# li199603/easy_gaussian_splatting

Hardware: AMD Instinct MI355X
Metric: train iters/sec + forward render fps, 1M Gaussians @ 1080p (higher is better)
Workload: dtype f32

## Files before the change

### easy_gaussian_splatting_amd/csrc/gs_binning.hip

```cpp

#include "gs_common.h"

namespace gs {

#define GS_BIN_PER_GROUP 4096
#define GS_BIN_MAX_GROUPS 256
constexpr int kBinThreads = 1024;
constexpr int kCoopTiles = 32;

BinLayout bin_layout(int C, int64_t N, int tiles) {
    BinLayout L;
    int64_t g = (N + GS_BIN_PER_GROUP - 1) / GS_BIN_PER_GROUP;
    if (g < 1) g = 1;
    if (g > GS_BIN_MAX_GROUPS) g = GS_BIN_MAX_GROUPS;
    L.groups = (int)g;
    L.per_group = (N + g - 1) / g;
    auto align = [](size_t x) { return (x + 255) & ~(size_t)255; };
    size_t off = 0;
    L.hist_off = off; off = align(off + sizeof(uint32_t) * (size_t)C * L.groups * tiles);
    L.tile_cnt_off = off; off = align(off + sizeof(uint32_t) * (size_t)C * tiles);
    L.grp_tot_off = off; off = align(off + sizeof(uint32_t) * (size_t)C * L.groups);
    L.grp_base_off = off; off = align(off + sizeof(uint32_t) * (size_t)C * L.groups);
    L.items_off = off; off = align(off + sizeof(int32_t) * (64 + (size_t)10 * (size_t)C * tiles));
    L.total = off;
// ... 45 lines not shown
        }
    }
    __syncthreads();
    uint32_t* out = hist_mat + ((size_t)c * G + grp) * tiles;
    for (int t = threadIdx.x; t < tiles; t += blockDim.x) out[t] = hist[t];
    uint32_t wsum = wave_reduce_add(local);
    if (lane_id() == 0) scratch[threadIdx.x >> 6] = wsum;
    __syncthreads();
    if (threadIdx.x == 0) {
        uint32_t s = 0;
        for (int i = 0; i < (int)(blockDim.x >> 6); ++i) s += scratch[i];
        grp_tot[c * G + grp] = s;
    }
}

constexpr int kColTiles = GS_BIN_MAX_GROUPS > 256 ? 32 : 64, kColChunks = GS_BIN_MAX_GROUPS > 256 ? 32 : 16;
__global__ __launch_bounds__(kColTiles * kColChunks) void bin_colscan_kernel(int C, int G, int tiles, uint32_t* __restrict__ hist_mat,
                                                                              uint32_t* __restrict__ tile_cnt) {
    __shared__ uint32_t part[kColChunks][kColTiles + 1];
    const int tl = threadIdx.x % kColTiles, ch = threadIdx.x / kColTiles;
    const int64_t i = (int64_t)blockIdx.x * kColTiles + tl;
    const bool in = i < (int64_t)C * tiles;
    const int c = in ? (int)(i / tiles) : 0, t = in ? (int)(i % tiles) : 0;
    const int per = (G + kColChunks - 1) / kColChunks;
    const int g0 = ch * per, g1 = min(G, g0 + per);
    uint32_t* col = hist_mat + (size_t)c * G * tiles + t;
    constexpr int kMax = 16;
    uint32_t v[kMax];
    uint32_t sum = 0;
#pragma unroll
    for (int k = 0; k < kMax; ++k) {
        v[k] = (in && g0 + k < g1) ? col[(size_t)(g0 + k) * tiles] : 0u;
        sum += v[k];
    }
    uint32_t extra = 0;
    for (int g = g0 + kMax; in && g < g1; ++g) extra += col[(size_t)g * tiles];
    part[ch][tl] = sum + extra;
    __syncthreads();
    uint32_t run = 0, total = 0;
#pragma unroll
    for (int k = 0; k < kColChunks; ++k) {
        const uint32_t p = part[k][tl];
        run += k < ch ? p : 0u;
        total += p;
    }
    if (in) {
#pragma unroll
        for (int k = 0; k < kMax; ++k) {
            if (g0 + k < g1) col[(size_t)(g0 + k) * tiles] = run;
            run += v[k];
        }
        for (int g = g0 + kMax; g < g1; ++g) { const uint32_t x = col[(size_t)g * tiles]; col[(size_t)g * tiles] = run; run += x; }
        if (ch == 0) tile_cnt[i] = total;
    }
}

constexpr int kScanItems = 16;
__global__ __launch_bounds__(kBinThreads) void bin_tilescan_kernel(
    int n_tiles_total, int n_groups_total, const uint32_t* __restrict__ tile_cnt,
    const uint32_t* __restrict__ grp_tot, int32_t* __restrict__ isect_offsets,
    int32_t* __restrict__ bucket_offsets, uint32_t* __restrict__ grp_base,
    int64_t* __restrict__ info, int32_t* __restrict__ tile_order, int64_t cap_isects, int64_t cap_tile,
    int64_t keep_mask, int32_t* __restrict__ sort_counts, int64_t* __restrict__ info_mirror, int per_call,
    int64_t* __restrict__ rblk, int phase) {
    __shared__ unsigned long long scratch[17];
    const int chunk = kBinThreads * kScanItems;
    if (round_idle(rblk, phase)) return;
    if (blockIdx.x == 2) {
        if (sort_counts && threadIdx.x < 64) sort_counts[threadIdx.x] = 0;
        unsigned long long gcarry = 0;
        for (int base = 0; base < n_groups_total; base += kBinThreads) {
            const int i = base + threadIdx.x;
            unsigned long long v = i < n_groups_total ? grp_tot[i] : 0ull, total;
            unsigned long long ex = block_excl_scan_add(v, scratch, &total);
            if (i < n_groups_total) grp_base[i] = (uint32_t)(gcarry + ex);
            gcarry += total;
        }
        return;
    }
    if (blockIdx.x == 1) {
        if (!tile_order) return;
        if (n_tiles_total > chunk) {
            for (int i = threadIdx.x; i < n_tiles_total; i += kBinThreads) tile_order[i] = i;
            return;
        }
        constexpr int kW = kBinThreads / 64;
        __shared__ uint32_t cls_cnt[64][kW + 1];
        auto cls_of = [](uint32_t x) -> int {
            if (x < 2u) return 0;
            const int lg = 31 - __clz((int)x);
            return min(63, (lg << 2) | (int)((x << (31 - lg)) >> 29 & 3u));
        };
        const int wv = threadIdx.x >> 6;
        const int first = threadIdx.x * kScanItems;
        uint32_t v[kScanItems];
#pragma unroll
        for (int k = 0; k < kScanItems; ++k) v[k] = (first + k < n_tiles_total) ? tile_cnt[first + k] : 0u;
        for (int i = threadIdx.x; i < 64 * (kW + 1); i += kBinThreads) (&cls_cnt[0][0])[i] = 0u;
        __syncthreads();
#pragma unroll
        for (int k = 0; k < kScanItems; ++k)
            if (first + k < n_tiles_total) atomicAdd(&cls_cnt[cls_of(v[k])][wv], 1u);
        __syncthreads();
        if (threadIdx.x < 64) {
            const int c = 63 - (int)threadIdx.x;
            uint32_t n = 0, cw[kW];
#pragma unroll
            for (int w = 0; w < kW; ++w) { cw[w] = cls_cnt[c][w]; n += cw[w]; }
            uint32_t run = wave_incl_scan_add(n) - n;
#pragma unroll
            for (int w = 0; w < kW; ++w) { cls_cnt[c][w] = run; run += cw[w]; }
        }
        __syncthreads();
#pragma unroll
        for (int k = 0; k < kScanItems; ++k)
            if (first + k < n_tiles_total) tile_order[atomicAdd(&cls_cnt[cls_of(v[k])][wv], 1u)] = first + k;
        return;
    }
    unsigned long long carry_i = phase == 2 ? (unsigned long long)rblk[GS_ROUND_BASE] : 0ull, carry_b = 0;
    uint32_t max_cnt = 0;
    for (int base = 0; base < n_tiles_total; base += chunk) {
        const int first = base + threadIdx.x * kScanItems;
        uint32_t v[kScanItems];
        unsigned long long si = 0, sb = 0;
#pragma unroll
        for (int k = 0; k < kScanItems; ++k) {
            v[k] = (first + k < n_tiles_total) ? tile_cnt[first + k] : 0u;
            si += v[k];
            sb += (v[k] + GS_BUCKET - 1) / GS_BUCKET;
// ... 116 lines not shown
            for (int i = lane_id(); i < bcnt; i += 64) {
                const int yy = div_by_width(i, binv);
                const uint32_t pos = atomicAdd(&cursor[(by0 + yy) * tw + bx0 + (i - yy * bw)], 1u);
                keys[pos] = ((unsigned long long)bd << 32) | (slot_gid ? bslot + i : (uint32_t)bf);
                if (slot_gid) slot_gid[bslot + i] = bf;
            }
        }
    }
}

template <typename KeyPtr>
__device__ __forceinline__ void bitonic_sort_keys(KeyPtr key, int n, int P) {
    for (int k = 2; k <= P; k <<= 1) {
        const int half = k >> 1;
        for (int idx = threadIdx.x; idx < (P >> 1); idx += blockDim.x) {
            const int blk = idx / half, off = idx - blk * half;
            const int a = blk * k + off, b = blk * k + k - 1 - off;
            if (b < n) {
                const unsigned long long ka = key[a], kb = key[b];
                if (ka > kb) { key[a] = kb; key[b] = ka; }
            }
        }
        __syncthreads();
        for (int j = half >> 1; j > 0; j >>= 1) {
            for (int idx = threadIdx.x; idx < (P >> 1); idx += blockDim.x) {
                const int a = ((idx & ~(j - 1)) << 1) | (idx & (j - 1)), b = a + j;
                if (b < n) {
                    const unsigned long long ka = key[a], kb = key[b];
                    if (ka > kb) { key[a] = kb; key[b] = ka; }
                }
            }
            __syncthreads();
        }
    }
}

struct SortArgs {
    int tiles, tile_bits, lo_excl, hi_incl;
    const int32_t* isect_offsets;
    unsigned long long* keys;
    const int32_t* slot_gid;
    int64_t* isect_ids;
    int32_t* flatten_ids;
    int32_t* slots;
    const int64_t* guard;
    int coarse;
    int seg;
    unsigned long long* merged;
    const int64_t* rblk;
    int phase;
};
__device__ __forceinline__ bool sort_off(const SortArgs& a) { return guard_tripped(a.guard) || round_idle(a.rblk, a.phase); }

constexpr int kSegLen = 8192;
constexpr int kSegMax = 8;

template <bool IN_LDS>
__global__ void tile_sort_kernel(const SortArgs a) {
    extern __shared__ __attribute__((aligned(16))) unsigned long long skeys[];
    const int t = blockIdx.x;
    if (sort_off(a)) return;
    const int lo = a.isect_offsets[t], hi = a.isect_offsets[t + 1];
    const int n = hi - lo;
    if (n <= a.lo_excl || n > a.hi_incl) return;
    int P = 1;
    while (P < n) P <<= 1;
    unsigned long long* gk = a.keys + lo;
    if (IN_LDS) {
        for (int i = threadIdx.x; i < n; i += blockDim.x) skeys[i] = gk[i];
        __syncthreads();
        bitonic_sort_keys(skeys, n, P);
    } else {
        bitonic_sort_keys(gk, n, P);
    }
    if (a.coarse) {
        if (IN_LDS) for (int i = threadIdx.x; i < n; i += blockDim.x) gk[i] = skeys[i];
        return;
    }
    const int cam = t / a.tiles, tid = t - cam * a.tiles;
    const long long hi_bits = ((long long)cam << (32 + a.tile_bits)) | ((long long)tid << 32);
    for (int i = threadIdx.x; i < n; i += blockDim.x) {
        const unsigned long long k = IN_LDS ? skeys[i] : gk[i];
        const uint32_t slot = (uint32_t)k;
        if (a.slot_gid) { a.slots[lo + i] = (int32_t)slot; a.flatten_ids[lo + i] = a.slot_gid[slot]; }
        else a.flatten_ids[lo + i] = (int32_t)slot;
        if (a.isect_ids) a.isect_ids[lo + i] = hi_bits | (long long)(k >> 32);
    }
}

template <int T>
__device__ __forceinline__ void radix_sort_list(const SortArgs& a, const int vblock) {
    extern __shared__ __attribute__((aligned(16))) unsigned long long skeys[];
    constexpr int W = T / 64;
    const int tile = a.seg ? vblock / kSegMax : vblock;
    int lo = a.isect_offsets[tile], n = a.isect_offsets[tile + 1] - lo;
    if (n <= a.lo_excl || n > a.hi_incl) return;
    if (a.seg) {
        const int sg = vblock - tile * kSegMax;
        lo += sg * kSegLen;
        n = min(kSegLen, n - sg * kSegLen);
        if (n <= 0) return;
    }
    const int cap = a.seg ? kSegLen : a.hi_incl;
    unsigned long long* src = skeys;
    unsigned long long* dst = skeys + cap;
    uint32_t* cnt = reinterpret_cast<uint32_t*>(skeys + 2 * cap);
    uint32_t* nxt = cnt + W * 256;
    __shared__ int s_flag;
    const int tid = threadIdx.x, lane = tid & 63, wave = tid >> 6;
// ... 69 lines not shown
        uint32_t* tc = cnt; cnt = nxt; nxt = tc;
    }
    __syncthreads();
    if (tid == 0) s_flag = 0;
    __syncthreads();
    bool bad = false;
    for (int i = tid + 1; i < n; i += T) bad |= src[i] < src[i - 1];
    if (bad) s_flag = 1;
    __syncthreads();
    if (s_flag) {
        int P = 1;
        while (P < n) P <<= 1;
        bitonic_sort_keys(src, n, P);
    }
    if (a.coarse || a.seg) {
        unsigned long long* out = a.keys + lo;
        for (int i = tid; i < n; i += T) out[i] = src[i];
        return;
    }
    const int cam = tile / a.tiles, tix = tile - cam * a.tiles;
    const long long hi_bits = ((long long)cam << (32 + a.tile_bits)) | ((long long)tix << 32);
    for (int i = tid; i < n; i += T) {
        const unsigned long long k = src[i];
        const uint32_t slot = (uint32_t)k;
        if (a.slot_gid) { a.slots[lo + i] = (int32_t)slot; a.flatten_ids[lo + i] = a.slot_gid[slot]; }
        else a.flatten_ids[lo + i] = (int32_t)slot;
        if (a.isect_ids) a.isect_ids[lo + i] = hi_bits | (long long)(k >> 32);
    }
}

template <int T>
__global__ __launch_bounds__(T) void tile_radix_sort_kernel(const SortArgs a) {
    if (sort_off(a)) return;
    radix_sort_list<T>(a, blockIdx.x);
}

template <int T>
__global__ __launch_bounds__(T) void tile_radix_sort_items_kernel(const SortArgs a, const int32_t* __restrict__ items,
                                                                  const int32_t* __restrict__ n_items) {
    if (sort_off(a)) return;
    const int n = *n_items;
    for (int it = blockIdx.x; it < n; it += gridDim.x) {
        radix_sort_list<T>(a, items[it]);
        __syncthreads();
    }
}

__global__ __launch_bounds__(256) void class_items_kernel(int n_lists, const int32_t* __restrict__ offsets,
                                                          int32_t* __restrict__ items, int32_t* __restrict__ counts,
                                                          const int64_t* __restrict__ guard, const int64_t* __restrict__ rblk, int phase) {
    if (guard_tripped(guard) || round_idle(rblk, phase)) return;
    const int i = blockIdx.x * blockDim.x + threadIdx.x;
    if (i >= n_lists) return;
    const int n = offsets[i + 1] - offsets[i];
    if (n > 1024 && n <= 4096) items[atomicAdd(&counts[0], 1)] = i;
    else if (n > 4096 && n <= kSegLen) items[n_lists + atomicAdd(&counts[1], 1)] = i;
    else if (n > kSegLen && n <= kSegLen * kSegMax) {
        const int ns = (n + kSegLen - 1) / kSegLen;
        const int p = atomicAdd(&counts[2], ns);
        for (int sg = 0; sg < ns; ++sg) items[2 * n_lists + p + sg] = i * kSegMax + sg;
    }
}

static size_t sort_items_bytes(int64_t n_lists) {
    return sizeof(int32_t) * (64 + (size_t)(2 + kSegMax) * (size_t)n_lists);
}


struct BinsLayout {
    int groups, shift, bw, bh, nbins;
    int64_t per_group;
    size_t hist_off;
    size_t bin_cnt_off;
    size_t grp_tot_off;
    size_t grp_base_off;
    size_t coff_off;
    size_t choff_off;
    size_t tile_cnt_off;
    size_t chunk_bin_off;
    int chunk_shift;
    size_t rec_off;
    size_t staged_off;
    size_t cnt_ct_off;
    size_t items_off;
    int64_t max_chunks;
    size_t total;
};

static BinsLayout bins_layout(int C, int64_t N, int tw, int th, int bin_shift, int64_t coarse_cap) {
    BinsLayout L;
    int64_t g = (N + GS_BIN_PER_GROUP - 1) / GS_BIN_PER_GROUP;
    if (g < 1) g = 1;
    if (g > GS_BIN_MAX_GROUPS) g = GS_BIN_MAX_GROUPS;
    L.groups = (int)g;
    L.per_group = (N + g - 1) / g;
    const int64_t nb2 = (int64_t)((tw + 3) / 4) * ((th + 3) / 4);
    L.shift = bin_shift ? bin_shift : ((N / nb2 > 2500) ? 1 : 2);
    const int B = 1 << L.shift;
    L.bw = (tw + B - 1) / B; L.bh = (th + B - 1) / B; L.nbins = L.bw * L.bh;
    auto align = [](size_t x) { return (x + 255) & ~(size_t)255; };
    size_t off = 0;
    L.hist_off = off; off = align(off + sizeof(uint32_t) * (size_t)C * L.groups * L.nbins);
    L.bin_cnt_off = off; off = align(off + sizeof(uint32_t) * (size_t)C * L.nbins);
    L.grp_tot_off = off; off = align(off + sizeof(uint32_t) * (size_t)C * L.groups);
    L.grp_base_off = off; off = align(off + sizeof(uint32_t) * (size_t)C * L.groups);
    L.coff_off = off; off = align(off + sizeof(int32_t) * ((size_t)C * L.nbins + 1));
    L.choff_off = off; off = align(off + sizeof(int32_t) * ((size_t)C * L.nbins + 1));
    L.tile_cnt_off = off; off = align(off + sizeof(uint32_t) * (size_t)C * tw * th);
    L.chunk_shift = 10 + (L.shift - 1);
    L.max_chunks = (coarse_cap >> L.chunk_shift) + (int64_t)C * L.nbins;
    L.chunk_bin_off = off; off = align(off + sizeof(int4) * (size_t)L.max_chunks);
    L.rec_off = off; off = align(off + sizeof(uint4) * (size_t)C * (size_t)N);
    L.staged_off = off; off = align(off + sizeof(uint4) * (size_t)coarse_cap);
    L.cnt_ct_off = off; off = align(off + sizeof(uint32_t) * (size_t)L.max_chunks * B * B);
// ... 377 lines not shown
            int l = 0, r = min(kSegLen, n - o * kSegLen);
            while (l < r) {
                const int mid = (l + r) >> 1;
                if (seg[mid] < k) l = mid + 1; else r = mid;
            }
            pos += l;
        }
        if (a.coarse) {
            a.merged[lo + pos] = k;
        } else {
            const uint32_t slot = (uint32_t)k;
            if (a.slot_gid) { a.slots[lo + pos] = (int32_t)slot; a.flatten_ids[lo + pos] = a.slot_gid[slot]; }
            else a.flatten_ids[lo + pos] = (int32_t)slot;
            if (a.isect_ids) a.isect_ids[lo + pos] = hi_bits | (long long)(k >> 32);
        }
    }
    }
}

__global__ __launch_bounds__(1024) void seg_copy_kernel(const SortArgs a, const int32_t* __restrict__ items,
                                                        const int32_t* __restrict__ n_items) {
    if (sort_off(a)) return;
    const int n_it = *n_items;
    for (int it = blockIdx.x; it < n_it; it += gridDim.x) {
        const int vblock = items[it];
        const int list = vblock / kSegMax, sg = vblock - list * kSegMax;
        const int lo = a.isect_offsets[list], n = a.isect_offsets[list + 1] - lo;
        const int s_lo = sg * kSegLen, s_n = min(kSegLen, n - s_lo);
        for (int i = threadIdx.x; i < s_n; i += blockDim.x) a.keys[lo + s_lo + i] = a.merged[lo + s_lo + i];
    }
}

constexpr int kSortLarge = kSegLen * kSegMax;

}

using namespace gs;

extern "C" int gs_bin_groups(int64_t N) { return bin_layout(1, N, 1).groups; }

static int list_round(int64_t*& rblk) {
    const Rounds R = current_rounds();
    const int phase = (R.phase == 1 || R.phase == 4) ? 1 : (R.phase == 2 ? 2 : 0);
    rblk = phase ? R.blk : nullptr;
    return phase;
}

extern "C" size_t gs_bin_workspace_bytes(int C, int64_t N, int tile_w, int tile_h) {
    return bin_layout(C, N, tile_w * tile_h).total;
}

#define GS_SORT1K_THREADS 256
#define GS_SORT4K_THREADS 256
static int launch_list_sorts(hipStream_t st, SortArgs& a, unsigned grid, int64_t max_tile_count, int32_t* items_ws) {
    int lo_excl = 0;
    int32_t* counts = items_ws;
    int32_t* items = items_ws + 64;
    const size_t radix_lds = 2 * sizeof(uint32_t) * 256;
    a.lo_excl = 0; a.hi_incl = 1024;
    if (max_tile_count > 0) {
        const size_t lds_k = 2 * sizeof(uint64_t) * 1024 + radix_lds * (GS_SORT1K_THREADS / 64);
        hipLaunchKernelGGL(tile_radix_sort_kernel<GS_SORT1K_THREADS>, dim3(grid), dim3(GS_SORT1K_THREADS), lds_k, st, a);
        GS_LAUNCH_CHECK("tile_radix_sort_kernel");
    }
    if (max_tile_count <= 1024) return GS_OK;
    hipLaunchKernelGGL(class_items_kernel, dim3((grid + 255) / 256), dim3(256), 0, st, (int)grid, a.isect_offsets, items, counts, a.guard, a.rblk, a.phase);
    GS_LAUNCH_CHECK("class_items_kernel");
    {
        a.lo_excl = 1024; a.hi_incl = 4096;
        const size_t lds_k = 2 * sizeof(uint64_t) * 4096 + radix_lds * (GS_SORT4K_THREADS / 64);
        if (int rc = ensure_lds((const void*)tile_radix_sort_items_kernel<GS_SORT4K_THREADS>, lds_k)) return rc;
        hipLaunchKernelGGL(tile_radix_sort_items_kernel<GS_SORT4K_THREADS>, dim3(grid < 512u ? grid : 512u), dim3(GS_SORT4K_THREADS), lds_k, st, a,
                           (const int32_t*)items, (const int32_t*)counts);
        GS_LAUNCH_CHECK("tile_radix_sort_items_kernel<4096>");
    }
    if (max_tile_count > 4096) {
        a.lo_excl = 4096; a.hi_incl = kSegLen;
        const size_t lds_k = 2 * sizeof(uint64_t) * (size_t)kSegLen + radix_lds * (768 / 64);
        if (int rc = ensure_lds((const void*)tile_radix_sort_items_kernel<768>, lds_k)) return rc;
        hipLaunchKernelGGL(tile_radix_sort_items_kernel<768>, dim3(grid < 256u ? grid : 256u), dim3(768), lds_k, st, a,
                           (const int32_t*)(items + grid), (const int32_t*)(counts + 1));
        GS_LAUNCH_CHECK("tile_radix_sort_items_kernel<8192>");
    }
    if (max_tile_count > kSegLen) {
        a.lo_excl = kSegLen; a.hi_incl = kSortLarge; a.seg = 1;
        const size_t lds_k = 2 * sizeof(uint64_t) * (size_t)kSegLen + radix_lds * (768 / 64);
        if (int rc = ensure_lds((const void*)tile_radix_sort_items_kernel<768>, lds_k)) return rc;
        const int32_t* it = items + 2 * (size_t)grid;
        const int32_t* nit = counts + 2;
        hipLaunchKernelGGL(tile_radix_sort_items_kernel<768>, dim3(256), dim3(768), lds_k, st, a, it, nit);
        GS_LAUNCH_CHECK("tile_radix_sort_items_kernel<segments>");
        hipLaunchKernelGGL(seg_merge_kernel, dim3(512), dim3(1024), 0, st, a, it, nit);
        GS_LAUNCH_CHECK("seg_merge_kernel");
        if (a.coarse) {
            hipLaunchKernelGGL(seg_copy_kernel, dim3(512), dim3(1024), 0, st, a, it, nit);
            GS_LAUNCH_CHECK("seg_copy_kernel");
        }
        a.seg = 0;
    }
    if (max_tile_count > kSortLarge) {
        a.lo_excl = kSortLarge; a.hi_incl = 0x7fffffff;
        hipLaunchKernelGGL(tile_sort_kernel<false>, dim3(grid), dim3(1024), 0, st, a);
        GS_LAUNCH_CHECK("tile_sort_kernel<global>");
    }
    (void)lo_excl;
    return GS_OK;
}

extern "C" int gs_bin_count(void* stream, int C, int64_t N, int tile_w, int tile_h, const uint32_t* bbox,
                            void* workspace, size_t workspace_bytes, int32_t* isect_offsets,
                            int32_t* bucket_offsets, int32_t* tile_order, int64_t* info_dev, int64_t* info_host) {
    GS_REQUIRE(C >= 1 && N >= 0 && tile_w > 0 && tile_h > 0, "C>=1, N>=0, positive tile grid");
    const int tiles = tile_w * tile_h;
    GS_REQUIRE((size_t)tiles * 4 + 128 <= 160 * 1024, "tile grid too large for the LDS histogram (max 40928 tiles per camera)");
    GS_REQUIRE((int64_t)C * tiles < (1ll << 31), "too many tiles");
    const BinLayout L = bin_layout(C, N, tiles);
    GS_REQUIRE(workspace && workspace_bytes >= L.total, "workspace too small (see gs_bin_workspace_bytes)");
    GS_REQUIRE(isect_offsets && bucket_offsets && info_dev, "null output pointer");
    GS_REQUIRE(N == 0 || bbox, "null bbox");
    int64_t* rblk;
// ... 15 lines not shown
                       tiles, hist, tile_cnt);
    GS_LAUNCH_CHECK("bin_colscan_kernel");
    const Guard gd = current_guard();
    GS_REQUIRE(gd.info == nullptr || gd.info == info_dev, "the guard set by gs_guard_set must be this call's info_dev");
    hipLaunchKernelGGL(bin_tilescan_kernel, dim3(3), dim3(kBinThreads), 0, st, (int)ct, C * L.groups, tile_cnt,
                       grp_tot, isect_offsets, bucket_offsets, grp_base, info_dev, tile_order, gd.cap_isects, gd.cap_tile,
                       (int64_t)0, (int32_t*)(ws + L.items_off), current_info_mirror(), gd.per_call, rblk, phase);
    GS_LAUNCH_CHECK("bin_tilescan_kernel");
    if (info_host) {
        GS_HIP_CHECK(hipMemcpyAsync(info_host, info_dev, 4 * sizeof(int64_t), hipMemcpyDeviceToHost, st));
        GS_HIP_CHECK(hipStreamSynchronize(st));
    }
    return GS_OK;
}

extern "C" int gs_bin_emit_sort(void* stream, int C, int64_t N, int tile_w, int tile_h, const uint32_t* bbox,
                                const float* depths, void* workspace, size_t workspace_bytes,
                                const int32_t* isect_offsets, int64_t n_isects, int64_t max_tile_count,
                                uint64_t* keys_tmp, int32_t* slot_gid, int32_t* cum_tiles,
                                int64_t* isect_ids, int32_t* flatten_ids, int32_t* slots) {
    GS_REQUIRE(C >= 1 && N >= 0 && tile_w > 0 && tile_h > 0, "C>=1, N>=0, positive tile grid");
    const int tiles = tile_w * tile_h;
    const BinLayout L = bin_layout(C, N, tiles);
    GS_REQUIRE(workspace && workspace_bytes >= L.total, "workspace too small (see gs_bin_workspace_bytes)");
    GS_REQUIRE(n_isects >= 0 && n_isects < (1ll << 31), "intersection count must fit int32");
    if (N == 0) return GS_OK;
    GS_REQUIRE(bbox && depths && isect_offsets && cum_tiles, "null pointer");
    GS_REQUIRE(n_isects == 0 || (keys_tmp && flatten_ids), "null intersection buffer");
    GS_REQUIRE((slot_gid == nullptr) == (slots == nullptr), "slot_gid and slots: both (training lists) or neither (inference lists)");
    int64_t* rblk;
    const int phase = list_round(rblk);
    GS_REQUIRE(phase == 0 || C == 1, "depth rounds: one camera per call");
    hipStream_t st = (hipStream_t)stream;
    char* ws = (char*)workspace;
    const uint32_t* hist = (const uint32_t*)(ws + L.hist_off);
    const uint32_t* grp_base = (const uint32_t*)(ws + L.grp_base_off);
    const size_t lds = sizeof(uint32_t) * ((size_t)tiles + 32);
    if (int rc = ensure_lds((const void*)bin_emit_kernel, lds)) return rc;
    hipLaunchKernelGGL(bin_emit_kernel, dim3(L.groups, C), dim3(kBinThreads), lds, st, N, tile_w, tiles,
                       L.per_group, (const uint4*)bbox, depths, hist, isect_offsets, grp_base,
                       (unsigned long long*)keys_tmp, slot_gid, cum_tiles, current_guard().info, (const int64_t*)rblk, phase);
    GS_LAUNCH_CHECK("bin_emit_kernel");
    if (n_isects == 0) return GS_OK;
    SortArgs a;
    a.tiles = tiles;
    int tb = 0;
    for (int v = tiles; v > 0; v >>= 1) ++tb;
    a.tile_bits = tb;
    a.isect_offsets = isect_offsets; a.keys = (unsigned long long*)keys_tmp; a.slot_gid = slot_gid;
    a.isect_ids = isect_ids; a.flatten_ids = flatten_ids; a.slots = slots;
    a.guard = current_guard().info;
    a.coarse = 0; a.seg = 0; a.merged = nullptr; a.rblk = rblk; a.phase = phase;
    static_assert(2 + kSegMax == 10, "bin_layout sizes the work lists for kSegMax == 8");
    return launch_list_sorts(st, a, (unsigned)(C * tiles), max_tile_count, (int32_t*)(ws + L.items_off));
}

extern "C" size_t gs_bins_workspace_bytes(int C, int64_t N, int tile_w, int tile_h, int bin_shift, int64_t coarse_cap) {
    if (bin_shift < 0 || bin_shift > 2 || coarse_cap < 0) return 0;
    return bins_layout(C, N, tile_w, tile_h, bin_shift, coarse_cap).total;
}

template <bool WRITE>
static int launch_refine(hipStream_t st, const BinsLayout& L, const RefineArgs& a) {
    const unsigned grid = (unsigned)L.max_chunks;
    if (L.shift == 2) hipLaunchKernelGGL((bins_refine_kernel<WRITE, 2>), dim3(grid), dim3(1024), 0, st, a);
    else hipLaunchKernelGGL((bins_refine_kernel<WRITE, 1>), dim3(grid), dim3(256), 0, st, a);
    GS_LAUNCH_CHECK("bins_refine_kernel");
    return GS_OK;
}

static void fill_refine_args(RefineArgs& r, const BinsLayout& L, int C, int tile_w, int tile_h, char* ws, const uint64_t* coarse_keys,
                             const uint32_t* bbox, const int64_t* info_dev) {
    r.tw = tile_w; r.th = tile_h; r.tiles = tile_w * tile_h; r.n_bins_total = C * L.nbins;
    r.choff = (const int32_t*)(ws + L.choff_off);
    r.chunk_desc = (const int4*)(ws + L.chunk_bin_off);
    r.cnt_ct = (uint32_t*)(ws + L.cnt_ct_off);
    int tb = 0;
    for (int v = r.tiles; v > 0; v >>= 1) ++tb;
    r.tile_bits = tb; r.bw = L.bw; r.nbins = L.nbins;
    r.coff = (const int32_t*)(ws + L.coff_off);
    r.keys = (const unsigned long long*)coarse_keys;
    r.rec = (const uint4*)(ws + L.rec_off);
    r.staged = (uint4*)(ws + L.staged_off);
    r.tile_cnt = (uint32_t*)(ws + L.tile_cnt_off);
    r.isect_offsets = nullptr; r.isect_ids = nullptr; r.flatten_ids = nullptr; r.slots = nullptr;
    r.info = info_dev;
    int64_t* rblk;
    r.phase = list_round(rblk);
    r.rblk = rblk;
}

extern "C" int gs_bins_count(void* stream, int C, int64_t N, int tile_w, int tile_h, int bin_shift, const uint32_t* bbox,
                             const float* depths, void* workspace, size_t workspace_bytes, uint64_t* coarse_keys,
                             int64_t coarse_cap, int64_t coarse_list_cap,
                             int32_t* cum_tiles, int32_t* isect_offsets, int32_t* bucket_offsets, int32_t* tile_order,
                             int64_t* info_dev, int64_t* info_host) {
    GS_REQUIRE(C >= 1 && N >= 0 && tile_w > 0 && tile_h > 0, "C>=1, N>=0, positive tile grid");
    const int tiles = tile_w * tile_h;
    GS_REQUIRE((int64_t)C * tiles < (1ll << 31) && (int64_t)C * N < (1ll << 31), "too many tiles or flatten ids");
    GS_REQUIRE(bin_shift >= 0 && bin_shift <= 2, "bin_shift: 0 (library default), 1 (2x2 tiles) or 2 (4x4 tiles)");
    GS_REQUIRE(coarse_cap >= 0 && coarse_cap < (1ll << 31) && (coarse_cap == 0 || coarse_keys), "coarse key buffer");
    const BinsLayout L = bins_layout(C, N, tile_w, tile_h, bin_shift, coarse_cap);
    GS_REQUIRE((size_t)L.nbins * 4 + 128 <= 160 * 1024, "tile grid too large for the LDS bin histogram");
    GS_REQUIRE(workspace && workspace_bytes >= L.total, "workspace too small (see gs_bins_workspace_bytes)");
    GS_REQUIRE(isect_offsets && bucket_offsets && info_dev, "null output pointer");
    GS_REQUIRE(N == 0 || (bbox && depths && cum_tiles), "null bbox / depths / cum_tiles");
    hipStream_t st = (hipStream_t)stream;
    char* ws = (char*)workspace;
    uint32_t* hist = (uint32_t*)(ws + L.hist_off);
    uint32_t* bin_cnt = (uint32_t*)(ws + L.bin_cnt_off);
    uint32_t* grp_tot = (uint32_t*)(ws + L.grp_tot_off);
    uint32_t* grp_base = (uint32_t*)(ws + L.grp_base_off);
    int32_t* coff = (int32_t*)(ws + L.coff_off);
    uint32_t* tile_cnt = (uint32_t*)(ws + L.tile_cnt_off);
    const Guard gd = current_guard();
    GS_REQUIRE(gd.info == nullptr || gd.info == info_dev, "the guard set by gs_guard_set must be this call's info_dev");
    int64_t* rblk;
    const int phase = list_round(rblk);
    GS_REQUIRE(phase == 0 || C == 1, "depth rounds: one camera per call");
    int64_t list_cap = 0x7fffffff;
    if (coarse_list_cap > 0) list_cap = coarse_list_cap <= 1024 ? 1024 : coarse_list_cap <= 4096 ? 4096 : coarse_list_cap <= kSegLen ? kSegLen
                                        : coarse_list_cap <= kSortLarge ? kSortLarge : 0x7fffffff;
    const size_t lds = sizeof(uint32_t) * ((size_t)L.nbins + 32);
    if (int rc = ensure_lds((const void*)bins_hist_kernel, lds)) return rc;
    hipLaunchKernelGGL(bins_hist_kernel, dim3(L.groups, C), dim3(kBinThreads), lds, st, N, L.shift, L.bw, L.nbins, L.per_group,
                       (const uint4*)bbox, hist, grp_tot, (const int64_t*)rblk, phase);
    GS_LAUNCH_CHECK("bins_hist_kernel");
    const int64_t cb = (int64_t)C * L.nbins;
    hipLaunchKernelGGL(bins_colscan_kernel, dim3((unsigned)((cb + 3) / 4)), dim3(256), 0, st, C, L.groups, L.nbins, hist, bin_cnt);
    GS_LAUNCH_CHECK("bins_colscan_kernel");
    hipLaunchKernelGGL(bins_scan_kernel, dim3(2), dim3(kBinThreads), 0, st, (int)cb, C * L.groups, bin_cnt, grp_tot, coff,
                       (int32_t*)(ws + L.choff_off), (int4*)(ws + L.chunk_bin_off), L.max_chunks, L.chunk_shift, grp_base,
                       info_dev, coarse_cap, list_cap,
                       (gd.info != nullptr && !gd.per_call) ? 1 : 0, (int32_t*)(ws + L.items_off), (const int64_t*)rblk, phase);
    GS_LAUNCH_CHECK("bins_scan_kernel");
    if (N > 0) {
        if (int rc = ensure_lds((const void*)bins_emit_kernel, lds)) return rc;
        hipLaunchKernelGGL(bins_emit_kernel, dim3(L.groups, C), dim3(kBinThreads), lds, st, N, L.shift, L.bw, L.nbins, L.per_group,
                           (const uint4*)bbox, depths, hist, coff, grp_base, (unsigned long long*)coarse_keys, cum_tiles,
                           (uint4*)(ws + L.rec_off), (const int64_t*)info_dev, (const int64_t*)rblk, phase);
        GS_LAUNCH_CHECK("bins_emit_kernel");
        SortArgs a;
        a.tiles = L.nbins; a.tile_bits = 0;
        a.isect_offsets = coff; a.keys = (unsigned long long*)coarse_keys; a.slot_gid = nullptr;
        a.isect_ids = nullptr; a.flatten_ids = nullptr; a.slots = nullptr;
        a.guard = info_dev; a.coarse = 1; a.seg = 0; a.rblk = rblk; a.phase = phase;
        a.merged = (unsigned long long*)(ws + L.staged_off);
        if (int rc = launch_list_sorts(st, a, (unsigned)cb, list_cap < coarse_cap ? list_cap : coarse_cap, (int32_t*)(ws + L.items_off))) return rc;
    }
    RefineArgs r;
    fill_refine_args(r, L, C, tile_w, tile_h, ws, coarse_keys, bbox, info_dev);
    if (int rc = launch_refine<false>(st, L, r)) return rc;
    {
        const unsigned g = (unsigned)(((int64_t)C * tiles + 255) / 256);
        if (L.shift == 2) hipLaunchKernelGGL(bins_chunkscan_kernel<2>, dim3(g), dim3(256), 0, st, r, C);
        else hipLaunchKernelGGL(bins_chunkscan_kernel<1>, dim3(g), dim3(256), 0, st, r, C);
        GS_LAUNCH_CHECK("bins_chunkscan_kernel");
    }
    hipLaunchKernelGGL(bin_tilescan_kernel, dim3(2), dim3(kBinThreads), 0, st, C * tiles, 0, tile_cnt, (const uint32_t*)nullptr,
                       isect_offsets, bucket_offsets, (uint32_t*)nullptr, info_dev, tile_order, gd.cap_isects,
                       (int64_t)0x7fffffffffffffffll, (int64_t)12, (int32_t*)nullptr, current_info_mirror(), gd.per_call, rblk, phase);
    GS_LAUNCH_CHECK("bin_tilescan_kernel");
    if (info_host) {
        GS_HIP_CHECK(hipMemcpyAsync(info_host, info_dev, 8 * sizeof(int64_t), hipMemcpyDeviceToHost, st));
        GS_HIP_CHECK(hipStreamSynchronize(st));
    }
    return GS_OK;
}

extern "C" int gs_bins_lists(void* stream, int C, int64_t N, int tile_w, int tile_h, int bin_shift, const uint32_t* bbox, void* workspace,
                             size_t workspace_bytes, const uint64_t* coarse_keys, int64_t coarse_cap, const int32_t* cum_tiles,
                             const int32_t* isect_offsets, int64_t* isect_ids, int32_t* flatten_ids, int32_t* slots,
                             const int64_t* info_dev) {
    GS_REQUIRE(C >= 1 && N >= 0 && tile_w > 0 && tile_h > 0, "C>=1, N>=0, positive tile grid");
    GS_REQUIRE(bin_shift >= 0 && bin_shift <= 2 && coarse_cap >= 0, "bin_shift: 0, 1 or 2; coarse_cap as given to gs_bins_count");
    const BinsLayout L = bins_layout(C, N, tile_w, tile_h, bin_shift, coarse_cap);
    GS_REQUIRE(workspace && workspace_bytes >= L.total, "workspace too small (see gs_bins_workspace_bytes)");
    GS_REQUIRE(info_dev && isect_offsets, "null pointer");
    if (N == 0) return GS_OK;
    GS_REQUIRE(cum_tiles && bbox && flatten_ids, "null list buffer");
    RefineArgs r;
    fill_refine_args(r, L, C, tile_w, tile_h, (char*)workspace, coarse_keys, bbox, info_dev);
    r.isect_offsets = isect_offsets; r.isect_ids = isect_ids; r.flatten_ids = flatten_ids; r.slots = slots;
    return launch_refine<true>((hipStream_t)stream, L, r);
}
```

### easy_gaussian_splatting_amd/csrc/gs_blend.hip

```cpp
#include <algorithm>

#include "gs_common.h"
#include "gs_math.h"

namespace gs {

#ifdef GS_BWD_CHECK
struct BwdCheck {
    float* fwd_T;
    int32_t* fwd_cnt;
    float2* unit_out;
    int2* unit_hdr;
};
static BwdCheck g_bwd_check = {nullptr, nullptr, nullptr, nullptr};
#define GS_IF_CHECK(...) __VA_ARGS__
#else
#define GS_IF_CHECK(...)
#endif

constexpr int kUnit = GS_UNIT;
constexpr int kChunk = 8;
constexpr int kUnitLog = 128;
constexpr int kWalkUnits = GS_WALK_UNITS, kWalkStorage = GS_WALK_STORAGE, kWalkRows = GS_WALK_ROWS,
              kWalkFlags = GS_WALK_FLAGS, kWalkSkip = GS_WALK_SKIP;
constexpr int kScanThreads = 256, kScanPerThread = 32, kScanChunk = kScanThreads * kScanPerThread;

struct BlendFwdArgs {
    const int32_t* tile_order;
    int C, W, H, tw, tiles;
    const float4* rec;
    const float* bg;
    const int32_t *isect_offsets, *flatten_ids, *slots;
    float *out_colors, *out_alphas;
    float4* ckpt;
    int2* qlist;
    int32_t* qcnt;
    uint8_t* qmask;
    int4* unit_desc;
    int32_t* walk;
    int cap_units;
    unsigned long long* flags;
    const int64_t* guard;
    int64_t* rblk;
    uint8_t* live;
    float4* tstate;
    int4* trec;
    int solo;
    GS_IF_CHECK(BwdCheck chk;)
};

#ifdef GS_CLOCK_PROBE
__device__ unsigned long long gs_clk_acc[4];
struct ClockProbe {
    long long c0, w0; int slot;
    __device__ ClockProbe(int s) : c0(clock64()), w0(wall_clock64()), slot(s) {}
    __device__ ~ClockProbe() {
        if ((threadIdx.x & 63) == 0) {
            atomicAdd(&gs_clk_acc[slot], (unsigned long long)(clock64() - c0));
            atomicAdd(&gs_clk_acc[slot + 1], (unsigned long long)(wall_clock64() - w0));
        }
    }
};
#define GS_CLOCK_PROBE_SCOPE(slot) ClockProbe clock_probe_(slot)
#else
#define GS_CLOCK_PROBE_SCOPE(slot)
#endif

#ifdef GS_EXACT_MATH
__device__ __forceinline__ float fast_exp2(float x) { return (float)exp2((double)x); }
__device__ __forceinline__ float fast_rcp(float x) { return (float)(1.0 / (double)x); }
#else
__device__ __forceinline__ float fast_exp2(float x) { return __builtin_amdgcn_exp2f(x); }
__device__ __forceinline__ float fast_rcp(float x) { return __builtin_amdgcn_rcpf(x); }
#endif

constexpr float kDoneScale = 18446744073709551616.f;
constexpr float kDoneInv = 5.421010862427522e-20f;
// ... 258 lines not shown
        }
        if (lv && !a.solo) {
#pragma unroll
            for (int k = 0; k < 4; ++k) a.tstate[((size_t)t * 4 + k) * 64 + lane] = make_float4(T[k], cr[k], cg[k], cb[k]);
            if (CKPT && lane == 0) {
                a.trec[2 * (size_t)t] = make_int4(cnt[0], cnt[1], cnt[2], cnt[3]);
                int ru[4];
#pragma unroll
                for (int k = 0; k < 4; ++k) ru[k] = cnt[k] > 0 ? uring[4 * k + (((cnt[k] - 1) / kUnit) & 3)] : 0;
                a.trec[2 * (size_t)t + 1] = make_int4(ru[0], ru[1], ru[2], ru[3]);
            }
        }
    }
    float bgr = 0.f, bgg = 0.f, bgb = 0.f, bga = 0.f;
    if (a.bg) {
        bgr = a.bg[NC * cam];
        if (NC > 1) bgg = a.bg[NC * cam + 1];
        if (NC > 2) bgb = a.bg[NC * cam + 2];
        if (NC > 3) bga = a.bg[NC * cam + 3];
    }
#pragma unroll
    for (int k = 0; k < 4; ++k) {
        const int px = px0 + 8 * (k & 1), py = py0 + 8 * (k >> 1);
        if (px < a.W && py < a.H) {
            const size_t o = ((size_t)cam * a.H + py) * a.W + px;
            const float Tf = px_final_T(T[k]);
            a.out_colors[NC * o] = cr[k] + Tf * bgr;
            if (NC > 1) a.out_colors[NC * o + 1] = cg[k] + Tf * bgg;
            if (NC > 2) a.out_colors[NC * o + 2] = cb[k] + Tf * bgb;
            if (NC > 3) a.out_colors[NC * o + 3] = ca[k] + Tf * bga;
            a.out_alphas[o] = 1.f - Tf;
            GS_IF_CHECK(if (CKPT && a.chk.fwd_T) { a.chk.fwd_T[o] = Tf; a.chk.fwd_cnt[o] = taken[k]; })
        }
    }
}

template <bool CKPT, int WAVES, int ROUND>
__global__ __launch_bounds__(64 * WAVES) GS_FWD_ATTR void blend_fwd_kernel(const BlendFwdArgs a) {
    blend_fwd_body<CKPT, WAVES, ROUND, 3>(a, nullptr);
}
template <bool CKPT, int WAVES, int NC>
__global__ __launch_bounds__(64 * WAVES) __attribute__((amdgpu_waves_per_eu(CKPT ? (NC == 4 ? 4 : 5) : 1, 8))) void chan_fwd_kernel(const BlendFwdArgs a, float* ckpt_ext) {
    blend_fwd_body<CKPT, WAVES, 0, NC>(a, ckpt_ext);
}

struct RowScanArgs {
    const uint8_t* qmask;
    int32_t* row_base;
    int32_t* walk;
    int64_t n_cap, cap_rows;
    unsigned long long* flags;
    const int64_t* guard;
    volatile int64_t* mirror;
};

__device__ __forceinline__ int32_t row_counts32(const uint8_t* __restrict__ qmask, int64_t i0, int64_t n, uint32_t (&w)[8]) {
#pragma unroll
    for (int j = 0; j < 8; ++j) w[j] = 0u;
    if (i0 + kScanPerThread <= n) {
        const uint4 x = reinterpret_cast<const uint4*>(qmask + i0)[0], y = reinterpret_cast<const uint4*>(qmask + i0)[1];
        w[0] = x.x; w[1] = x.y; w[2] = x.z; w[3] = x.w; w[4] = y.x; w[5] = y.y; w[6] = y.z; w[7] = y.w;
    } else {
        for (int j = 0; j < kScanPerThread; ++j)
            if (i0 + j < n) w[j >> 2] |= (uint32_t)qmask[i0 + j] << (8 * (j & 3));
    }
    int32_t tot = 0;
#pragma unroll
    for (int j = 0; j < 8; ++j) {
        uint32_t v = w[j] & 0x0f0f0f0fu;
        v = v - ((v >> 1) & 0x55555555u);
        v = (v & 0x33333333u) + ((v >> 2) & 0x33333333u);
        w[j] = v;
        tot += (int32_t)((v * 0x01010101u) >> 24);
    }
    return tot;
}

__global__ __launch_bounds__(kScanThreads) void row_count_kernel(const RowScanArgs a) {
    __shared__ int32_t scratch[20];
    if (a.walk[kWalkSkip] != 0) return;
    const int64_t n = slots_in_use(a.n_cap, a.guard);
    const int64_t c0 = (int64_t)blockIdx.x * kScanChunk;
    if (c0 > n) return;
    uint32_t w[8];
    const int32_t tot = row_counts32(a.qmask, c0 + (int64_t)threadIdx.x * kScanPerThread, n, w);
    int32_t block_tot;
    block_excl_scan_add<int32_t>(tot, scratch, &block_tot);
    if (threadIdx.x == 0) a.walk[GS_WALK_WORDS + blockIdx.x] = block_tot;
}

__global__ __launch_bounds__(1024) void row_chunk_scan_kernel(const RowScanArgs a) {
    __shared__ int32_t scratch[20];
    if (a.walk[kWalkSkip] != 0) return;
    const int64_t n = slots_in_use(a.n_cap, a.guard);
    const int nb = (int)(n / kScanChunk) + 1;
    int32_t* part = a.walk + GS_WALK_WORDS;
    const int per = (nb + 1023) / 1024;
    const int j0 = (int)threadIdx.x * per, j1 = min(nb, j0 + per);
    int32_t mine = 0;
    for (int j = j0; j < j1; ++j) mine += part[j];
    int32_t total;
    int32_t run = block_excl_scan_add<int32_t>(mine, scratch, &total);
    for (int j = j0; j < j1; ++j) { const int32_t c = part[j]; part[j] = run; run += c; }
    if (threadIdx.x == 0) {
        int32_t fullest = 0;
        for (int r = 0; r < GS_WALK_RANGES; ++r) fullest = max(fullest, a.walk[GS_WALK_RANGE0 + 32 * r]);
        a.walk[kWalkStorage] = GS_WALK_RANGES * fullest;
        a.walk[kWalkRows] = total;
        int fl = a.walk[kWalkFlags];
        if (a.flags && (fl & GS_FLAG_UNITS)) atomicOr(a.flags, (unsigned long long)GS_FLAG_UNITS);
        if ((int64_t)total > a.cap_rows) {
            fl |= GS_FLAG_ROWS;
            a.walk[kWalkFlags] = fl;
            if (a.flags) atomicOr(a.flags, (unsigned long long)GS_FLAG_ROWS);
        }
        if (a.mirror) {
            a.mirror[0] = a.walk[kWalkUnits]; a.mirror[1] = a.walk[kWalkStorage]; a.mirror[2] = total; a.mirror[3] = fl;
            __threadfence_system();
        }
    }
}

__global__ __launch_bounds__(kScanThreads) void row_base_kernel(const RowScanArgs a) {
    __shared__ int32_t scratch[20];
    if (a.walk[kWalkSkip] != 0) return;
    const int64_t n = slots_in_use(a.n_cap, a.guard);
    const int64_t c0 = (int64_t)blockIdx.x * kScanChunk;
    if (c0 > n) return;
    const int64_t i0 = c0 + (int64_t)threadIdx.x * kScanPerThread;
    uint32_t w[8];
    const int32_t tot = row_counts32(a.qmask, i0, n, w);
    int32_t block_tot;
    const int32_t run = block_excl_scan_add<int32_t>(tot, scratch, &block_tot) + a.walk[GS_WALK_WORDS + blockIdx.x];
    int32_t first16 = 0;
#pragma unroll
    for (int j = 0; j < 4; ++j) first16 += (int32_t)((w[j] * 0x01010101u) >> 24);
    if (i0 <= n) a.row_base[i0 >> 4] = run;
    if (i0 + 16 <= n) a.row_base[(i0 >> 4) + 1] = run + first16;
}

struct BlendBwdArgs {
    int C, W, H, tw, tiles;
    const float4* rec;
    const int32_t* walk;
    const int2* qlist;
    const int32_t* qcnt;
    const int4* unit_desc;
    const float4* ckpt;
    const uint8_t* qmask;
    const int32_t* row_base;
    int cap_units;
    const int32_t* cls_hdr;
    const int4* cls_desc;
    int cls_cap;
    const float *out_colors, *out_alphas, *v_colors, *v_alphas;
    float4* rows;
    const int64_t* guard;
    GS_IF_CHECK(BwdCheck chk;)
};

constexpr int kBwdWaves = 4;
constexpr int kPipeLanes = 8;
constexpr int kPerLane = kUnit / kPipeLanes;
static_assert(kPerLane == 4, "bwd_wave is instantiated for 1 .. 4 entries per lane");
constexpr int kUnitsPerWave = 64 / kPipeLanes;
constexpr int kUnitPixels = 64;
constexpr int kBwdSteps = kUnitPixels + kPipeLanes - 1;

__device__ __forceinline__ float dpp_row_shr1(float v) {
    return __builtin_bit_cast(float, __builtin_amdgcn_update_dpp(__builtin_bit_cast(int, v), __builtin_bit_cast(int, v), 0x111, 0xf, 0xf, false));
}


// ... 169 lines not shown
        row[i] += __popc((unsigned)m & ((1u << q) - 1u));
    }
#pragma unroll
    for (int i = 0; i < E; ++i) {
        if (e[i].has) {
            float4* rp = a.rows + (GS_ROW_FLOATS / 4) * (size_t)row[i];
            const float v_op = e[i].op > 0.f ? (float)(-e[i].s_vs / (acc_t)e[i].op) : 0.f;
            rp[0] = make_float4((float)e[i].s_mx, (float)e[i].s_my, (float)e[i].s_ax, (float)e[i].s_ay);
            rp[1] = make_float4((float)((acc_t)0.5f * e[i].s_A), (float)e[i].s_B, (float)((acc_t)0.5f * e[i].s_C), v_op);
            rp[2] = make_float4((float)e[i].s_r, (float)e[i].s_g, (float)e[i].s_b, NC == 4 ? (float)e[i].s_3 : 0.f);
        }
    }
}

constexpr int kClsHdrInts = 16, kClsThreads = 1024;
__global__ __launch_bounds__(64) void unit_classes_clear_kernel(int32_t* __restrict__ hdr) {
    if (threadIdx.x < kClsHdrInts) hdr[threadIdx.x] = 0;
}
__global__ __launch_bounds__(kClsThreads) void unit_classes_kernel(const int32_t* __restrict__ walk, const int4* __restrict__ unit_desc,
                                                                   const int32_t* __restrict__ qcnt, int cap_units, int cls_cap,
                                                                   int32_t* __restrict__ hdr, int4* __restrict__ cls, const int64_t* __restrict__ guard) {
    __shared__ int s_cnt[kClsThreads / 64][4], s_base[kClsThreads / 64][4];
    if (guard_tripped(guard)) return;
    const int n_units = min(walk[kWalkUnits], cap_units);
    if ((int)blockIdx.x * kClsThreads >= n_units) return;
    const int u = (int)blockIdx.x * kClsThreads + (int)threadIdx.x, wave = threadIdx.x >> 6, lane = threadIdx.x & 63;
    int c = 0;
    int4 ud = make_int4(0, 0, 0, 0);
    if (u < n_units) {
        ud = unit_desc[u];
        const int n_in = min(kUnit, qcnt[ud.x] - ud.y * kUnit);
        c = min(max((n_in + kPipeLanes - 1) / kPipeLanes, 1), 4);
        ud.w = u;
    }
    unsigned long long m[4];
#pragma unroll
    for (int k = 0; k < 4; ++k) m[k] = __ballot(c == k + 1);
    if (lane < 4) s_cnt[wave][lane] = (int)__popcll(lane == 0 ? m[0] : (lane == 1 ? m[1] : (lane == 2 ? m[2] : m[3])));
    __syncthreads();
    if (threadIdx.x < 4) {
        int tot = 0;
        for (int w = 0; w < kClsThreads / 64; ++w) { s_base[w][threadIdx.x] = tot; tot += s_cnt[w][threadIdx.x]; }
        const int base = tot ? atomicAdd(hdr + 1 + threadIdx.x, tot) : 0;
        for (int w = 0; w < kClsThreads / 64; ++w) s_base[w][threadIdx.x] += base;
    }
    __syncthreads();
    if (c) {
        const unsigned long long mine = c == 1 ? m[0] : (c == 2 ? m[1] : (c == 3 ? m[2] : m[3]));
        const int i = s_base[wave][c - 1] + (int)__popcll(mine & ((1ull << lane) - 1ull));
        if (i < (c == 4 ? cap_units : cls_cap)) cls[(c == 4 ? 0 : cap_units + (3 - c) * cls_cap) + i] = ud;
    }
}

template <int NC>
__device__ __forceinline__ void blend_bwd_body(const BlendBwdArgs& a, const float* __restrict__ ckpt_ext) {
    __shared__ float4 sd0_all[kBwdWaves][kUnitsPerWave][64];
    __shared__ float2 sck_all[kBwdWaves][kUnitsPerWave][64];
    const int wave = threadIdx.x >> 6, lane = threadIdx.x & 63;
    const int pipe = lane / kPipeLanes, r = lane & (kPipeLanes - 1);
    if (guard_tripped(a.guard)) return;
    constexpr int kPerBlock = kBwdWaves * kUnitsPerWave;
    int cls = 4, blk = (int)blockIdx.x, n_units, first = 0;
    if (a.cls_hdr == nullptr) {
        n_units = min(a.walk[kWalkUnits], a.cap_units);
    } else {
        const int b4 = (a.cap_units + kPerBlock - 1) / kPerBlock, bt = (a.cls_cap + kPerBlock - 1) / kPerBlock;
        if (blk >= b4) {
            const int k = (blk - b4) / bt;
            cls = 3 - k; blk -= b4 + k * bt; first = a.cap_units + k * a.cls_cap;
        }
        n_units = min(a.cls_hdr[cls], cls == 4 ? a.cap_units : a.cls_cap);
    }
    const int in_class = (blk * kBwdWaves + wave) * kUnitsPerWave + pipe;
    if ((blk * kBwdWaves + wave) * kUnitsPerWave >= n_units) return;
    GS_CLOCK_PROBE_SCOPE(2);
    const bool valid = in_class < n_units;
    float4* sd0 = sd0_all[wave][pipe];
    float2* sck = sck_all[wave][pipe];
    float* sd1 = nullptr;
    if constexpr (NC == 4) {
        __shared__ float sd1_all[kBwdWaves][kUnitsPerWave][64];
        sd1 = sd1_all[wave][pipe];
    }

    int4 ud = make_int4(0, 0, 0, 0);
    if (valid) ud = a.cls_hdr ? a.cls_desc[first + in_class] : a.unit_desc[in_class];
    const int unit = a.cls_hdr ? ud.w : in_class;
    if (cls == 4) bwd_wave<4, NC>(a, ud, valid, unit, sd0, sd1, sck, r, ckpt_ext);
    else if (cls == 3) bwd_wave<3, NC>(a, ud, valid, unit, sd0, sd1, sck, r, ckpt_ext);
    else if (cls == 2) bwd_wave<2, NC>(a, ud, valid, unit, sd0, sd1, sck, r, ckpt_ext);
    else bwd_wave<1, NC>(a, ud, valid, unit, sd0, sd1, sck, r, ckpt_ext);
}

__global__ __launch_bounds__(kBwdWaves * 64) void blend_bwd_kernel(const BlendBwdArgs a) {
    blend_bwd_body<3>(a, nullptr);
}
template <int NC>
__global__ __launch_bounds__(kBwdWaves * 64) void chan_bwd_kernel(const BlendBwdArgs a, const float* ckpt_ext) {
    blend_bwd_body<NC>(a, ckpt_ext);
}

}

using namespace gs;

#ifdef GS_BWD_CHECK
extern "C" int gs_debug_bwd_check_set(float* fwd_T, int32_t* fwd_cnt, float* unit_out, int32_t* unit_hdr) {
    g_bwd_check.fwd_T = fwd_T; g_bwd_check.fwd_cnt = fwd_cnt;
    g_bwd_check.unit_out = reinterpret_cast<float2*>(unit_out); g_bwd_check.unit_hdr = reinterpret_cast<int2*>(unit_hdr);
    return GS_OK;
}
#endif

#ifdef GS_CLOCK_PROBE
extern "C" int gs_debug_clock_probe(int64_t* out4, int reset) {
    unsigned long long h[4] = {0, 0, 0, 0};
    if (out4) { GS_HIP_CHECK(hipMemcpyFromSymbol(h, HIP_SYMBOL(gs_clk_acc), sizeof(h))); for (int i = 0; i < 4; ++i) out4[i] = (int64_t)h[i]; }
    if (reset) { unsigned long long z[4] = {0, 0, 0, 0}; GS_HIP_CHECK(hipMemcpyToSymbol(HIP_SYMBOL(gs_clk_acc), z, sizeof(z))); }
    return GS_OK;
}
#endif

extern "C" size_t gs_walk_state_ints(int64_t n_isects) {
    if (n_isects < 0) return 0;
    return (size_t)GS_WALK_WORDS + (size_t)(n_isects / kScanChunk + 1);
}

template <int NC>
static int blend_fwd_launch(void* stream, int C, int width, int height, const float* rec,
                            const float* backgrounds, const int32_t* isect_offsets, const int32_t* tile_order,
                            const int32_t* flatten_ids, const int32_t* slots, int64_t n_isects, float* render_colors,
                            float* render_alphas, float* ckpt, int32_t* qlist, int32_t* qcnt, uint8_t* qmask,
                            int32_t* unit_desc, int64_t cap_units, int32_t* row_base, int64_t cap_rows, int32_t* walk_state,
                            float* ckpt_ext) {
    GS_REQUIRE(C >= 1 && width > 0 && height > 0 && n_isects >= 0, "C>=1, positive image size, n_isects>=0");
    GS_REQUIRE(isect_offsets && render_colors && render_alphas, "null pointer");
    const bool train = ckpt != nullptr;
    GS_REQUIRE(!train || (qlist && qcnt && qmask && unit_desc && row_base && walk_state && slots), "training mode needs every list output");
    GS_REQUIRE(!train || (cap_units >= kChunk * GS_WALK_RANGES && cap_units < (1ll << 26) && cap_rows >= 0 && cap_rows < (1ll << 31)),
               "training mode: 256 <= cap_units < 2^26 work units, cap_rows < 2^31 gradient rows");
    GS_REQUIRE(!train || n_isects < (1ll << 31) - kScanChunk, "training mode: the slots of a call are indexed by int32");
    static_assert(kScanPerThread == 32, "row_base_kernel writes two groups of 16 slots per thread");
    GS_REQUIRE(!train || (((uintptr_t)qmask & 15) == 0 && ((uintptr_t)row_base & 15) == 0 && ((uintptr_t)walk_state & 7) == 0),
               "training mode: qmask / row_base 16-byte aligned, walk_state 8-byte aligned");
    BlendFwdArgs a;
    a.C = C; a.W = width; a.H = height;
    a.tw = (width + GS_TILE - 1) / GS_TILE;
    a.tiles = a.tw * ((height + GS_TILE - 1) / GS_TILE);
    a.rec = reinterpret_cast<const float4*>(rec); a.bg = backgrounds; a.isect_offsets = isect_offsets;
    a.flatten_ids = flatten_ids; a.slots = slots;
    a.out_colors = render_colors; a.out_alphas = render_alphas;
    a.ckpt = reinterpret_cast<float4*>(ckpt); a.qlist = reinterpret_cast<int2*>(qlist); a.qcnt = qcnt; a.qmask = qmask;
    a.unit_desc = reinterpret_cast<int4*>(unit_desc); a.walk = walk_state; a.cap_units = (int)cap_units;
    a.tile_order = tile_order;
    a.guard = current_guard().info;
    a.flags = a.guard ? reinterpret_cast<unsigned long long*>(const_cast<int64_t*>(a.guard) + 3) : nullptr;
    const Rounds R = current_rounds();
    const int phase = (R.phase == 1 || R.phase == 4) ? 1 : (R.phase == 2 ? 2 : 0);
    a.solo = R.phase == 4 ? 1 : 0;
    GS_REQUIRE(R.phase != 4 || a.flags != nullptr, "depth rounds, front round alone: needs a step guard (gs_guard_set)");
    GS_REQUIRE(phase == 0 || C == 1, "depth rounds: one camera per call");
    GS_REQUIRE(phase == 0 || !train || R.tile_rec, "depth rounds, training mode: gs_rounds_set needs tile_rec");
    GS_REQUIRE(NC == 3 || phase == 0, "depth rounds render 3 channels only (tile_state holds T, r, g, b): clear gs_rounds_set");
    GS_REQUIRE(NC != 4 || !train || ckpt_ext, "channels = 4, training mode: ckpt_ext (cap_units * 64 floats) is required");
    a.rblk = R.blk; a.live = R.live; a.tstate = R.state; a.trec = reinterpret_cast<int4*>(R.tile_rec);
    GS_IF_CHECK(a.chk = g_bwd_check;)
    const unsigned n_tiles = (unsigned)(C * a.tiles);
    hipStream_t st = (hipStream_t)stream;
    constexpr int kFwdWaves = 4;
    const dim3 grid((n_tiles + kFwdWaves - 1) / kFwdWaves), block(64 * kFwdWaves);
    if (train) {
        const int walk_ints = (int)gs_walk_state_ints(n_isects);
        const unsigned cg = (unsigned)std::min<int64_t>(1024, std::max<int64_t>(1, (n_isects / 16 + 255) / 256));
        hipLaunchKernelGGL(qmask_clear_kernel, dim3(cg), dim3(256), 0, st, qmask, n_isects, walk_state, walk_ints, a.guard,
                           (const int64_t*)R.blk, phase);
        GS_LAUNCH_CHECK("qmask_clear_kernel");
        if constexpr (NC != 3) hipLaunchKernelGGL((chan_fwd_kernel<true, kFwdWaves, NC>), grid, block, 0, st, a, ckpt_ext);
        else if (phase == 1) hipLaunchKernelGGL((blend_fwd_kernel<true, kFwdWaves, 1>), grid, block, 0, st, a);
        else if (phase == 2) hipLaunchKernelGGL((blend_fwd_kernel<true, kFwdWaves, 2>), grid, block, 0, st, a);
        else hipLaunchKernelGGL((blend_fwd_kernel<true, kFwdWaves, 0>), grid, block, 0, st, a);
        GS_LAUNCH_CHECK("blend_fwd_kernel");
        if (phase == 1 && !a.solo) return GS_OK;
        RowScanArgs s;
        s.qmask = qmask; s.row_base = row_base; s.walk = walk_state; s.n_cap = n_isects; s.cap_rows = cap_rows;
        s.flags = a.flags; s.guard = a.guard; s.mirror = current_walk_mirror();
        const unsigned chunks = (unsigned)(n_isects / kScanChunk + 1);
        hipLaunchKernelGGL(row_count_kernel, dim3(chunks), dim3(kScanThreads), 0, st, s);
        hipLaunchKernelGGL(row_chunk_scan_kernel, dim3(1), dim3(1024), 0, st, s);
        hipLaunchKernelGGL(row_base_kernel, dim3(chunks), dim3(kScanThreads), 0, st, s);
        GS_LAUNCH_CHECK("row_base_kernel");
    } else {
        if constexpr (NC != 3) hipLaunchKernelGGL((chan_fwd_kernel<false, kFwdWaves, NC>), grid, block, 0, st, a, nullptr);
        else if (phase == 1) hipLaunchKernelGGL((blend_fwd_kernel<false, kFwdWaves, 1>), grid, block, 0, st, a);
        else if (phase == 2) hipLaunchKernelGGL((blend_fwd_kernel<false, kFwdWaves, 2>), grid, block, 0, st, a);
        else hipLaunchKernelGGL((blend_fwd_kernel<false, kFwdWaves, 0>), grid, block, 0, st, a);
        GS_LAUNCH_CHECK("blend_fwd_kernel");
    }
    return GS_OK;
}

extern "C" int gs_blend_fwd(void* stream, int C, int width, int height, const float* rec,
                            const float* backgrounds, const int32_t* isect_offsets, const int32_t* tile_order,
                            const int32_t* flatten_ids, const int32_t* slots, int64_t n_isects, float* render_colors,
                            float* render_alphas, float* ckpt, int32_t* qlist, int32_t* qcnt, uint8_t* qmask,
                            int32_t* unit_desc, int64_t cap_units, int32_t* row_base, int64_t cap_rows, int32_t* walk_state) {
    return blend_fwd_launch<3>(stream, C, width, height, rec, backgrounds, isect_offsets, tile_order, flatten_ids, slots, n_isects,
                               render_colors, render_alphas, ckpt, qlist, qcnt, qmask, unit_desc, cap_units, row_base, cap_rows,
                               walk_state, nullptr);
}

extern "C" int gs_blend_fwd_ch(void* stream, int C, int width, int height, int channels, const float* rec,
                               const float* backgrounds, const int32_t* isect_offsets, const int32_t* tile_order,
                               const int32_t* flatten_ids, const int32_t* slots, int64_t n_isects, float* render_colors,
                               float* render_alphas, float* ckpt, int32_t* qlist, int32_t* qcnt, uint8_t* qmask,
                               int32_t* unit_desc, int64_t cap_units, int32_t* row_base, int64_t cap_rows, int32_t* walk_state,
                               float* ckpt_ext) {
    GS_REQUIRE(channels >= 1 && channels <= 4, "channels must be 1, 2, 3 or 4");
#define GS_FWD_CH(NC) blend_fwd_launch<NC>(stream, C, width, height, rec, backgrounds, isect_offsets, tile_order, flatten_ids, slots, \
                                           n_isects, render_colors, render_alphas, ckpt, qlist, qcnt, qmask, unit_desc, cap_units,   \
                                           row_base, cap_rows, walk_state, ckpt_ext)
    switch (channels) {
        case 1: return GS_FWD_CH(1);
        case 2: return GS_FWD_CH(2);
        case 3: return GS_FWD_CH(3);
        default: return GS_FWD_CH(4);
    }
#undef GS_FWD_CH
}

static int64_t cls_region(int C, int width, int height) {
    const int64_t tiles = (int64_t)((width + GS_TILE - 1) / GS_TILE) * ((height + GS_TILE - 1) / GS_TILE);
    const int64_t per_block = kBwdWaves * kUnitsPerWave;
    return (4 * (int64_t)C * tiles + per_block - 1) / per_block * per_block;
}

extern "C" size_t gs_unit_classes_ints(int64_t cap_units, int C, int width, int height) {
    if (cap_units < 0 || C < 1 || width <= 0 || height <= 0) return 0;
    return (size_t)kClsHdrInts + 4 * ((size_t)cap_units + 3 * (size_t)cls_region(C, width, height));
}

template <int NC>
static int blend_bwd_launch(void* stream, int C, int width, int height, const float* rec,
                            const int32_t* qlist, const int32_t* qcnt, const int32_t* unit_desc, int64_t cap_units,
                            const float* ckpt, const uint8_t* qmask, const int32_t* row_base, const int32_t* walk_state,
                            const float* render_colors, const float* render_alphas, const float* v_render_colors,
                            const float* v_render_alphas, float* rows, int32_t* unit_classes, const float* ckpt_ext) {
    GS_REQUIRE(C >= 1 && width > 0 && height > 0 && cap_units >= 0 && cap_units < (1ll << 26), "C>=1, positive image size, 0 <= cap_units < 2^26");
    if (cap_units == 0) return GS_OK;
    GS_REQUIRE(rec && qlist && qcnt && unit_desc && ckpt && qmask && row_base && walk_state, "null list pointer");
    GS_REQUIRE(render_colors && render_alphas && v_render_colors && rows, "null image pointer");
    GS_REQUIRE(NC != 4 || ckpt_ext, "channels = 4: ckpt_ext (gs_blend_fwd_ch's fourth-channel checkpoints) is required");
    BlendBwdArgs a;
    a.C = C; a.W = width; a.H = height;
    a.tw = (width + GS_TILE - 1) / GS_TILE;
    a.tiles = a.tw * ((height + GS_TILE - 1) / GS_TILE);
    a.rec = reinterpret_cast<const float4*>(rec);
    a.qlist = reinterpret_cast<const int2*>(qlist); a.qcnt = qcnt; a.walk = walk_state;
    a.unit_desc = reinterpret_cast<const int4*>(unit_desc); a.cap_units = (int)cap_units;
    a.ckpt = reinterpret_cast<const float4*>(ckpt); a.qmask = qmask; a.row_base = row_base;
    a.out_colors = render_colors;
    a.out_alphas = render_alphas; a.v_colors = v_render_colors; a.v_alphas = v_render_alphas;
    a.rows = reinterpret_cast<float4*>(rows);
    a.guard = current_guard().info;
    GS_IF_CHECK(a.chk = g_bwd_check;)
    unsigned grid = (unsigned)((cap_units + kUnitsPerWave * kBwdWaves - 1) / (kUnitsPerWave * kBwdWaves));
    a.cls_hdr = nullptr; a.cls_desc = nullptr; a.cls_cap = 0;
    if (unit_classes) {
        GS_REQUIRE(((uintptr_t)unit_classes & 15) == 0, "unit_classes must be 16-byte aligned");
        a.cls_hdr = unit_classes; a.cls_desc = reinterpret_cast<const int4*>(unit_classes + kClsHdrInts);
        a.cls_cap = (int)cls_region(C, width, height);
        hipLaunchKernelGGL(unit_classes_clear_kernel, dim3(1), dim3(64), 0, (hipStream_t)stream, unit_classes);
        hipLaunchKernelGGL(unit_classes_kernel, dim3((unsigned)((cap_units + kClsThreads - 1) / kClsThreads)), dim3(kClsThreads), 0, (hipStream_t)stream,
                           walk_state, a.unit_desc, qcnt, (int)cap_units, a.cls_cap, unit_classes, reinterpret_cast<int4*>(unit_classes + kClsHdrInts),
                           a.guard);
        GS_LAUNCH_CHECK("unit_classes_kernel");
        grid += 3u * (unsigned)(a.cls_cap / (kUnitsPerWave * kBwdWaves));
    }
    if constexpr (NC == 3) hipLaunchKernelGGL(blend_bwd_kernel, dim3(grid), dim3(kBwdWaves * 64), 0, (hipStream_t)stream, a);
    else hipLaunchKernelGGL((chan_bwd_kernel<NC>), dim3(grid), dim3(kBwdWaves * 64), 0, (hipStream_t)stream, a, ckpt_ext);
    GS_LAUNCH_CHECK("blend_bwd_kernel");
    return GS_OK;
}

extern "C" int gs_blend_bwd(void* stream, int C, int width, int height, const float* rec,
                            const int32_t* qlist, const int32_t* qcnt, const int32_t* unit_desc, int64_t cap_units,
                            const float* ckpt, const uint8_t* qmask, const int32_t* row_base, const int32_t* walk_state,
                            const float* render_colors, const float* render_alphas, const float* v_render_colors,
                            const float* v_render_alphas, float* rows, int32_t* unit_classes) {
    return blend_bwd_launch<3>(stream, C, width, height, rec, qlist, qcnt, unit_desc, cap_units, ckpt, qmask, row_base, walk_state,
                               render_colors, render_alphas, v_render_colors, v_render_alphas, rows, unit_classes, nullptr);
}

extern "C" int gs_blend_bwd_ch(void* stream, int C, int width, int height, int channels, const float* rec,
                               const int32_t* qlist, const int32_t* qcnt, const int32_t* unit_desc, int64_t cap_units,
                               const float* ckpt, const uint8_t* qmask, const int32_t* row_base, const int32_t* walk_state,
                               const float* render_colors, const float* render_alphas, const float* v_render_colors,
                               const float* v_render_alphas, float* rows, int32_t* unit_classes, const float* ckpt_ext) {
    GS_REQUIRE(channels >= 1 && channels <= 4, "channels must be 1, 2, 3 or 4");
#define GS_BWD_CH(NC) blend_bwd_launch<NC>(stream, C, width, height, rec, qlist, qcnt, unit_desc, cap_units, ckpt, qmask, row_base, \
                                           walk_state, render_colors, render_alphas, v_render_colors, v_render_alphas, rows,         \
                                           unit_classes, ckpt_ext)
    switch (channels) {
        case 1: return GS_BWD_CH(1);
        case 2: return GS_BWD_CH(2);
        case 3: return GS_BWD_CH(3);
        default: return GS_BWD_CH(4);
    }
#undef GS_BWD_CH
}
```

### easy_gaussian_splatting_amd/csrc/gs_capi.hip

```cpp
#include <stdarg.h>

#include "gs_common.h"

namespace gs {
static thread_local char g_err[512] = "";
void set_error(const char* fmt, ...) {
    va_list ap;
    va_start(ap, fmt);
    vsnprintf(g_err, sizeof(g_err), fmt, ap);
    va_end(ap);
}
static thread_local Guard g_guard = {nullptr, 0, 0, 0};
Guard current_guard() { return g_guard; }
static thread_local int64_t* g_info_mirror = nullptr;
int64_t* current_info_mirror() { return g_info_mirror; }
static thread_local int64_t* g_walk_mirror = nullptr;
int64_t* current_walk_mirror() { return g_walk_mirror; }
static thread_local Rounds g_rounds = {nullptr, nullptr, nullptr, nullptr, 0};
Rounds current_rounds() { return g_rounds; }
}

extern "C" int gs_rounds_set(int64_t* rounds_dev, uint8_t* tile_live, float* tile_state, int32_t* tile_rec, int phase) {
    if (phase < 0 || phase > 4 || (phase != 0 && !rounds_dev) || ((phase == 1 || phase == 2 || phase == 4) && (!tile_live || !tile_state))) {
        gs::set_error("invalid argument: phase 0 (off), 1 (front round), 2 (back round), 3 (behind both) or 4 (front round alone); a round needs its buffers");
        return GS_ERR_ARG;
    }
    if ((((uintptr_t)tile_state) & 15) != 0 || (((uintptr_t)tile_rec) & 15) != 0) {
        gs::set_error("invalid argument: tile_state / tile_rec 16-byte aligned");
        return GS_ERR_ARG;
    }
    gs::g_rounds.blk = phase ? rounds_dev : nullptr;
    gs::g_rounds.live = phase ? tile_live : nullptr;
    gs::g_rounds.state = phase ? reinterpret_cast<float4*>(tile_state) : nullptr;
    gs::g_rounds.tile_rec = phase ? tile_rec : nullptr;
    gs::g_rounds.phase = phase;
    return GS_OK;
}

extern "C" int gs_info_mirror_set(int64_t* info_host_mapped) {
    gs::g_info_mirror = info_host_mapped;
    return GS_OK;
}

extern "C" int gs_walk_mirror_set(int64_t* walk_host_mapped) {
    gs::g_walk_mirror = walk_host_mapped;
    return GS_OK;
}

extern "C" int gs_guard_set(const int64_t* info_dev, int64_t cap_isects, int64_t cap_tile) {
    if (info_dev != nullptr && (cap_isects <= 0 || cap_tile <= 0)) {
        gs::set_error("invalid argument: a guard needs positive capacities");
        return GS_ERR_ARG;
    }
    gs::g_guard.info = info_dev;
    gs::g_guard.cap_isects = info_dev ? cap_isects : 0;
    gs::g_guard.cap_tile = info_dev ? cap_tile : 0;
    gs::g_guard.per_call = 0;
    return GS_OK;
}

extern "C" int gs_guard_set_call(const int64_t* info_dev, int64_t cap_isects, int64_t cap_tile) {
    if (int rc = gs_guard_set(info_dev, cap_isects, cap_tile)) return rc;
    gs::g_guard.per_call = info_dev != nullptr;
    return GS_OK;
}

namespace gs {
__global__ void step_status_kernel(const int64_t* __restrict__ info, const int64_t* __restrict__ applied,
                                   volatile int64_t* __restrict__ status, const float* __restrict__ loss3,
                                   float* __restrict__ loss_ring, int ring_len, const int32_t* __restrict__ walk,
                                   const int64_t* __restrict__ rblk) {
    if (threadIdx.x < 4) status[threadIdx.x] = info[threadIdx.x];
    if (threadIdx.x == 7) status[7] = rblk ? rblk[GS_ROUND_LIVE] : -1;
    if (threadIdx.x == 4) status[4] = applied ? applied[0] : 0;
    if (threadIdx.x == 5) status[5] = walk ? walk[GS_WALK_STORAGE] : 0;
    if (threadIdx.x == 6) status[6] = walk ? walk[GS_WALK_ROWS] : 0;
    if (loss_ring != nullptr && applied != nullptr && info[3] == 0 && threadIdx.x < 3 && applied[0] > 0)
        loss_ring[3 * ((applied[0] - 1) % ring_len) + threadIdx.x] = loss3[threadIdx.x];
    __threadfence_system();
}
}

extern "C" int gs_step_status(void* stream, const int64_t* info_dev, const int64_t* applied_dev, int64_t* status,
                              const float* loss3_dev, float* loss_ring_dev, int ring_len, const int32_t* walk_state) {
    if (!info_dev || !status || (loss_ring_dev && (!loss3_dev || ring_len <= 0))) {
        gs::set_error("invalid argument: null pointer / empty ring");
        return GS_ERR_ARG;
    }
    const gs::Rounds R = gs::current_rounds();
    hipLaunchKernelGGL(gs::step_status_kernel, dim3(1), dim3(64), 0, (hipStream_t)stream, info_dev, applied_dev, status, loss3_dev,
                       loss_ring_dev, ring_len, walk_state, (const int64_t*)(R.phase == 3 ? R.blk : nullptr));
    GS_LAUNCH_CHECK("step_status_kernel");
    return GS_OK;
}

namespace gs {
__global__ void guard_flag_out_kernel(const int64_t* __restrict__ info, float* __restrict__ dst0, float* __restrict__ dst1) {
    const float f = info[3] != 0 ? 1.f : 0.f;
// ... 42 lines not shown
```

### easy_gaussian_splatting_amd/csrc/gs_common.h

```cpp
#pragma once
#include <hip/hip_runtime.h>
#include <stdint.h>
#include <stdio.h>
#include <string.h>

#include <map>
#include <mutex>
#include <utility>

#include "../../include/gs_raster.h"

namespace gs {

void set_error(const char* fmt, ...);

#define GS_HIP_CHECK(expr)                                                                   \
    do {                                                                                     \
        hipError_t _e = (expr);                                                              \
        if (_e != hipSuccess) {                                                              \
            gs::set_error("%s failed: %s (%s:%d)", #expr, hipGetErrorString(_e), __FILE__,   \
                          __LINE__);                                                         \
            return GS_ERR_HIP;                                                               \
        }                                                                                    \
    } while (0)

#define GS_LAUNCH_CHECK(name)                                                                \
    do {                                                                                     \
        hipError_t _e = hipGetLastError();                                                   \
        if (_e != hipSuccess) {                                                              \
            gs::set_error("launch of %s failed: %s", name, hipGetErrorString(_e));           \
            return GS_ERR_HIP;                                                               \
        }                                                                                    \
    } while (0)

inline int ensure_lds(const void* fn, size_t bytes) {
    if (bytes > 64 * 1024) {
        static std::mutex mu;
        static std::map<std::pair<int, const void*>, size_t> done;
        int dev = 0;
        GS_HIP_CHECK(hipGetDevice(&dev));
        std::lock_guard<std::mutex> lock(mu);
        size_t& have = done[{dev, fn}];
        if (have < bytes) {
            GS_HIP_CHECK(hipFuncSetAttribute(fn, hipFuncAttributeMaxDynamicSharedMemorySize, (int)bytes));
            have = bytes;
        }
    }
    return GS_OK;
}

#define GS_REQUIRE(cond, msg)                                                                \
    do {                                                                                     \
        if (!(cond)) {                                                                       \
            gs::set_error("invalid argument: %s (%s)", msg, #cond);                          \
            return GS_ERR_ARG;                                                               \
        }                                                                                    \
    } while (0)

constexpr int kWave = 64;

struct Guard {
    const int64_t* info;
    int64_t cap_isects;
    int64_t cap_tile;
    int per_call;
};
Guard current_guard();
int64_t* current_info_mirror();
int64_t* current_walk_mirror();
__device__ __forceinline__ bool guard_tripped(const int64_t* info) { return info != nullptr && info[3] != 0; }

struct Rounds {
    int64_t* blk;
    uint8_t* live;
    float4* state;
    int32_t* tile_rec;
    int phase;
};
Rounds current_rounds();
__device__ __forceinline__ bool round_idle(const int64_t* blk, int phase) { return phase == 2 && blk[GS_ROUND_LIVE] == 0; }

__device__ __forceinline__ int rows_before(const int32_t* __restrict__ row_base16, const uint8_t* __restrict__ qmask, int s, int* slot_mask = nullptr) {
    const int g = s >> 4, k = s & 15;
    const uint4 q = reinterpret_cast<const uint4*>(qmask)[g];
    const uint32_t w[4] = {q.x, q.y, q.z, q.w};
    int n = row_base16[g];
#pragma unroll
    for (int j = 0; j < 4; ++j) {
        const int b = min(max(k - 4 * j, 0), 4);
        const uint32_t m = b >= 4 ? 0xffffffffu : ((1u << (8 * b)) - 1u);
        n += __popc(w[j] & m & 0x0f0f0f0fu);
    }
    if (slot_mask) *slot_mask = (int)((w[k >> 2] >> (8 * (k & 3))) & 0xfu);
    return n;
}

struct BinLayout {
    int groups;
    int64_t per_group;
    size_t hist_off;
    size_t tile_cnt_off;
    size_t grp_tot_off;
    size_t grp_base_off;
    size_t items_off;
    size_t total;
};
BinLayout bin_layout(int C, int64_t N, int tiles);

__device__ __forceinline__ int div_by_width(int i, float inv_w) { return (int)(((float)i + 0.5f) * inv_w); }

__device__ __forceinline__ int lane_id() { return threadIdx.x & 63; }

template <typename T>
__device__ __forceinline__ T wave_incl_scan_add(T v) {
#pragma unroll
    for (int d = 1; d < 64; d <<= 1) {
        T o = __shfl_up(v, d, 64);
        if (lane_id() >= d) v += o;
    }
    return v;
}

// ... 144 lines not shown
```

### easy_gaussian_splatting_amd/csrc/gs_loss.hip

```cpp
#include "gs_loss_tile.h"

namespace gs {

constexpr float kC1 = 0.01f * 0.01f, kC2 = 0.03f * 0.03f;

struct LossArgs {
    int H, W;
    int clamp_input;
    float lambda_ssim;
    const float *render, *gt, *mask;
    const float* const* slots;
    float* maps;
    float* partial;
    const float* gout;
    float* v_render;
};

__device__ __forceinline__ void st_off(float* base, unsigned byte_off, float v) {
    *reinterpret_cast<float*>(reinterpret_cast<char*>(base) + byte_off) = v;
}

__device__ __forceinline__ void st3_off(float* base, unsigned byte_off, float x, float y, float z) {
    *reinterpret_cast<F3*>(reinterpret_cast<char*>(base) + byte_off) = F3{x, y, z};
}

__device__ __forceinline__ bool loss_tile_channel(const LossArgs& a, int& x0, int& y0, int& ch) {
    const int ntx = (a.W + kLT - 1) / kLT, nt = ntx * ((a.H + kLT - 1) / kLT), per = (nt + 7) >> 3;
    const int id = blockIdx.x, k = id >> 3, local = k / 3, t = (id & 7) * per + local;
    ch = k - 3 * local;
    if (t >= nt) return false;
    const int ty = t / ntx;
    x0 = (t - ty * ntx) * kLT; y0 = ty * kLT;
    return true;
}

template <bool MASK>
__global__ __launch_bounds__(256) void l1_ssim_fwd_kernel(const LossArgs a) {
    constexpr float kWin[11] = GS_WIN_TAPS;
    extern __shared__ __attribute__((aligned(16))) float lds[];
    float* sx = lds;
    float* sy = sx + kLR * kLRP;
    float* hp = sy + kLR * kLRP;
    __shared__ float red[2][4];
    int x0, y0;
    if (!loss_tile(a, x0, y0)) {
        if (threadIdx.x == 0) { a.partial[2 * blockIdx.x] = 0.f; a.partial[2 * blockIdx.x + 1] = 0.f; }
        return;
    }
    const int tid = threadIdx.x;
    const unsigned row_bytes = 12u * (unsigned)a.W;
    const float* gt_img = a.slots ? a.slots[0] : a.gt;
    const float* mask_img = a.slots ? a.slots[1] : a.mask;
    constexpr int kPer = kLR / 6;
    float rv[kPer][3], gv[kPer][3], mv[MASK ? kPer : 1];
    if (tid < kLR * 6) {
        const int rg = tid / kLR, col = tid - rg * kLR;
        const int cx = clampi(x0 - kHalo + col, 0, a.W - 1), ytop = y0 - kHalo + rg;
#pragma unroll
        for (int i = 0; i < kPer; ++i) {
            const unsigned cy = (unsigned)clampi(ytop + 6 * i, 0, a.H - 1);
            const unsigned o = __umul24(cy, row_bytes) + 12u * (unsigned)cx;
            const F3 g3 = ld3_off(gt_img, o), r3 = ld3_off(a.render, o);
            gv[i][0] = g3.x; gv[i][1] = g3.y; gv[i][2] = g3.z;
            rv[i][0] = r3.x; rv[i][1] = r3.y; rv[i][2] = r3.z;
            if (MASK) mv[i] = ld_off(mask_img, __umul24(cy, 4u * (unsigned)a.W) + 4u * (unsigned)cx);
        }
    }
    float l1 = 0.f, ssim_sum = 0.f;
#pragma unroll 1
    for (int ch = 0; ch < 3; ++ch) {
        int t = tid;
        asm volatile("" : "+v"(t));
        const bool st_on = t < kLR * 6;
        const int rg = t / kLR, col = t - rg * kLR;
        if (st_on) {
            const int gx = x0 - kHalo + col;
            const bool col_own = col >= kHalo && col < kHalo + kLT && gx < a.W;
            float* dx = sx + rg * kLRP + col;
            float* dy = sy + rg * kLRP + col;
#pragma unroll
            for (int i = 0; i < kPer; ++i) {
                const int row = rg + 6 * i, gy = y0 - kHalo + row;
                const float g = gv[i][0];
                float r = rv[i][0];
                if (a.clamp_input) r = fminf(fmaxf(r, 0.f), 1.f);
                if (MASK) r = mv[i] * g + (1.f - mv[i]) * r;
                dx[6 * i * kLRP] = r;
                dy[6 * i * kLRP] = g;
                if (col_own && row >= kHalo && row < kHalo + kLT && gy < a.H) l1 += fabsf(r - g);
                gv[i][0] = gv[i][1]; gv[i][1] = gv[i][2];
                rv[i][0] = rv[i][1]; rv[i][1] = rv[i][2];
            }
        }
        __syncthreads();
        float* maps_c = a.maps + (size_t)ch * a.H * a.W * 3;
        {
            const bool h_on = st_on;
            const int row = col, c0 = min(kHOut * rg, kLT - kHOut);
            if (h_on) {
// ... 14 lines not shown
                }
            }
        }
        __syncthreads();
        {
            const int q = t / kLT, vcol = t - q * kLT, r0 = 4 * q;
            float mom[4][4];
#pragma unroll
            for (int mi = 0; mi < 4; ++mi) {
                float hv[14];
#pragma unroll
                for (int i = 0; i < 14; ++i) hv[i] = hp[mi * kLR * kHP + (r0 + i) * kHP + vcol];
#pragma unroll
                for (int j = 0; j < 4; ++j) {
                    float acc = kWin[0] * hv[j];
#pragma unroll
                    for (int kk = 1; kk < 11; ++kk) acc = fmaf(kWin[kk], hv[j + kk], acc);
                    mom[mi][j] = acc;
                }
            }
            const int gx = x0 + vcol;
#pragma unroll
            for (int j = 0; j < 4; ++j) {
                const int gy = y0 + r0 + j;
                const float mu_x = mom[0][j], mu_y = mom[1][j], ess = mom[2][j], exy = mom[3][j];
                const bool interior = gy >= kHalo && gy < a.H - kHalo && gx >= kHalo && gx < a.W - kHalo;
                if (gy < a.H && gx < a.W) {
                    float dmu = 0.f, dxx = 0.f, dxy = 0.f;
                    if (interior) {
                        const float mm = mu_x * mu_x + mu_y * mu_y, sxy = exy - mu_x * mu_y;
                        const float n1 = 2.f * mu_x * mu_y + kC1, n2 = 2.f * sxy + kC2;
                        const float d1 = mm + kC1, d2 = (ess - mm) + kC2;
                        const float i1 = __builtin_amdgcn_rcpf(d1), i2 = __builtin_amdgcn_rcpf(d2), inv = i1 * i2;
                        const float sv = n1 * n2 * inv;
                        ssim_sum += sv;
                        dxx = -sv * i2;
                        dxy = 2.f * n1 * inv;
                        dmu = 2.f * mu_y * (n2 - n1) * inv + 2.f * mu_x * sv * (i2 - i1);
                    }
                    st3_off(maps_c, __umul24((unsigned)gy, row_bytes) + 12u * (unsigned)gx, dmu, dxx, dxy);
                }
            }
        }
        if (ch < 2) __syncthreads();
    }
    l1 = wave_reduce_add(l1);
    ssim_sum = wave_reduce_add(ssim_sum);
    if (lane_id() == 0) { red[0][tid >> 6] = l1; red[1][tid >> 6] = ssim_sum; }
    __syncthreads();
    if (tid == 0) {
        a.partial[2 * blockIdx.x] = red[0][0] + red[0][1] + red[0][2] + red[0][3];
        a.partial[2 * blockIdx.x + 1] = red[1][0] + red[1][1] + red[1][2] + red[1][3];
    }
}

__global__ __launch_bounds__(256) void loss_reduce_kernel(int nblocks, const float* __restrict__ partial, int H, int W,
                                                          float lambda_ssim, float* __restrict__ out) {
    __shared__ double red[2][4];
    double s0 = 0.0, s1 = 0.0;
    for (int i = threadIdx.x; i < nblocks; i += 256) { s0 += partial[2 * i]; s1 += partial[2 * i + 1]; }
#pragma unroll
    for (int d = 32; d > 0; d >>= 1) { s0 += __shfl_xor(s0, d, 64); s1 += __shfl_xor(s1, d, 64); }
    if (lane_id() == 0) { red[0][threadIdx.x >> 6] = s0; red[1][threadIdx.x >> 6] = s1; }
    __syncthreads();
    if (threadIdx.x == 0) {
        const double l1 = (red[0][0] + red[0][1] + red[0][2] + red[0][3]) / ((double)H * W * 3.0);
        const double cnt = (double)(H - 2 * kHalo) * (double)(W - 2 * kHalo) * 3.0;
        const double ssim = (red[1][0] + red[1][1] + red[1][2] + red[1][3]) / cnt;
        out[0] = (float)l1; out[1] = (float)(1.0 - ssim);
        out[2] = (float)((1.0 - lambda_ssim) * l1 + lambda_ssim * (1.0 - ssim));
    }
}

__global__ __launch_bounds__(256) void l1_ssim_bwd_kernel(const LossArgs a) {
    constexpr float kWin[11] = GS_WIN_TAPS;
    extern __shared__ __attribute__((aligned(16))) float lds[];
    float* sm = lds;
    float* hp = lds;
    int x0, y0, ch;
    if (!loss_tile_channel(a, x0, y0, ch)) return;
    const int tid = threadIdx.x;
    const size_t plane = (size_t)a.H * a.W;
    const float g = a.gout[0];
    const float cnt = (float)(a.H - 2 * kHalo) * (float)(a.W - 2 * kHalo) * 3.f;
    const float k_ssim = -g * a.lambda_ssim / cnt;
    const float k_l1 = g * (1.f - a.lambda_ssim) / ((float)a.H * (float)a.W * 3.f);
    const unsigned row_bytes = 12u * (unsigned)a.W;
    const int q = tid / kLT, ocol = tid - q * kLT, r0 = 4 * q, ogx = x0 + ocol;
    const bool col_in = ogx < a.W;
    const unsigned o0 = __umul24((unsigned)min(y0 + r0, a.H - 1), row_bytes) + 12u * (unsigned)min(ogx, a.W - 1);
    const float* mask_img = a.slots ? a.slots[1] : a.mask;
    const float* gt_c = (a.slots ? a.slots[0] : a.gt) + ch;
    const float* render_c = a.render + ch;
    float gtv[4], rr[4], mk[4];
#pragma unroll
    for (int j = 0; j < 4; ++j) {
        const unsigned o = o0 + (y0 + r0 + j < a.H ? j * row_bytes : 0u);
        gtv[j] = ld_off(gt_c, o); rr[j] = ld_off(render_c, o);
        if (mask_img) mk[j] = ld_off(mask_img, o / 3u);
    }
    {
        constexpr int kRowsPer = kLR / 2;
        const int half = __builtin_amdgcn_readfirstlane(tid >> 7), jj = tid & 127;
        const int scol = jj / 3, smi = jj - scol * 3;
        const int sgx = x0 - kHalo + scol;
        const float* maps_c = a.maps + (size_t)ch * plane * 3;
        if (jj < kLR * 3) {
            const bool col_ok = sgx >= 0 && sgx < a.W;
            const unsigned lane_off = 4u * (unsigned)(clampi(sgx, 0, a.W - 1) * 3 + smi);
            float v[kRowsPer];
            const int gy0 = y0 - kHalo + half;
            const char* rowp = reinterpret_cast<const char*>(maps_c) + (int64_t)gy0 * row_bytes;
#pragma unroll
            for (int i = 0; i < kRowsPer; ++i) {
                const int gy = gy0 + 2 * i;
                v[i] = 0.f;
                if (gy >= 0 && gy < a.H) v[i] = ld_off(reinterpret_cast<const float*>(rowp), lane_off);
                rowp += 2 * row_bytes;
            }
            float* d = sm + (smi * kLR + half) * kLRP + scol;
#pragma unroll
            for (int i = 0; i < kRowsPer; ++i) d[2 * i * kLRP] = col_ok ? v[i] : 0.f;
        }
    }
// ... 48 lines not shown
            float r = rr[j], keep = 1.f;
            if (a.clamp_input) { keep = (r >= 0.f && r <= 1.f) ? 1.f : 0.f; r = fminf(fmaxf(r, 0.f), 1.f); }
            if (mask_img) { r = mk[j] * gtv[j] + (1.f - mk[j]) * r; keep *= 1.f - mk[j]; }
            const float d = r - gtv[j];
            const float sgn = d > 0.f ? 1.f : (d < 0.f ? -1.f : 0.f);
            st_off(out_c, o0 + j * row_bytes, keep * (k_ssim * (c[0][j] + 2.f * r * c[1][j] + gtv[j] * c[2][j]) + k_l1 * sgn));
        }
    }
}

__global__ __launch_bounds__(256) void clamp01_kernel(int64_t n4, int64_t n, const float* __restrict__ x,
                                                      const float* __restrict__ v_out, float* __restrict__ out) {
    const int64_t i = (int64_t)blockIdx.x * blockDim.x + threadIdx.x;
    if (i < n4) {
        const float4 a = reinterpret_cast<const float4*>(x)[i];
        float4 r;
        if (v_out) {
            const float4 g = reinterpret_cast<const float4*>(v_out)[i];
            r.x = (a.x >= 0.f && a.x <= 1.f) ? g.x : 0.f; r.y = (a.y >= 0.f && a.y <= 1.f) ? g.y : 0.f;
            r.z = (a.z >= 0.f && a.z <= 1.f) ? g.z : 0.f; r.w = (a.w >= 0.f && a.w <= 1.f) ? g.w : 0.f;
        } else {
            r.x = fminf(fmaxf(a.x, 0.f), 1.f); r.y = fminf(fmaxf(a.y, 0.f), 1.f);
            r.z = fminf(fmaxf(a.z, 0.f), 1.f); r.w = fminf(fmaxf(a.w, 0.f), 1.f);
        }
        reinterpret_cast<float4*>(out)[i] = r;
    }
    if (i == 0)
        for (int64_t k = n4 * 4; k < n; ++k) {
            const float a = x[k];
            out[k] = v_out ? ((a >= 0.f && a <= 1.f) ? v_out[k] : 0.f) : fminf(fmaxf(a, 0.f), 1.f);
        }
}

}

using namespace gs;

extern "C" int gs_clamp01(void* stream, int64_t n, const float* x, const float* v_out, float* out) {
    GS_REQUIRE(n >= 0, "n >= 0");
    if (n == 0) return GS_OK;
    GS_REQUIRE(x && out, "null pointer");
    GS_REQUIRE((((uintptr_t)x | (uintptr_t)out | (uintptr_t)v_out) & 15) == 0, "buffers must be 16-byte aligned");
    const int64_t n4 = n >> 2, blocks = (n4 + 255) / 256;
    hipLaunchKernelGGL(clamp01_kernel, dim3((unsigned)(blocks > 0 ? blocks : 1)), dim3(256), 0, (hipStream_t)stream, n4, n, x, v_out, out);
    GS_LAUNCH_CHECK("clamp01_kernel");
    return GS_OK;
}

extern "C" size_t gs_loss_workspace_floats(int height, int width) {
    const size_t nb = (size_t)((width + kLT - 1) / kLT) * ((height + kLT - 1) / kLT);
    return 9 * (size_t)height * width + 2 * (nb + 8);
}

static int loss_fwd_launch(void* stream, int height, int width, float lambda_ssim, const float* render, const float* gt,
                           const float* mask, const float* const* slots, bool has_mask, int clamp_input, float* workspace, float* out3) {
    GS_REQUIRE(height > 2 * kHalo && width > 2 * kHalo, "image must be larger than the 11x11 window");
    GS_REQUIRE((int64_t)height * width <= kLossMaxPixels && width <= kLossMaxWidth && height <= (1 << 24),
               "image too large for the loss kernels' 32-bit byte offsets (H * W <= 2^28, W <= 2^20, H <= 2^24: row indices go through 24-bit multiplies)");
    GS_REQUIRE(render && (gt || slots) && workspace && out3, "null pointer");
    LossArgs a;
    a.H = height; a.W = width; a.lambda_ssim = lambda_ssim; a.render = render; a.gt = gt; a.mask = mask; a.slots = slots;
    a.clamp_input = clamp_input != 0;
    a.maps = workspace; a.partial = workspace + 9 * (size_t)height * width; a.gout = nullptr; a.v_render = nullptr;
    const int blocks = (int)loss_grid(loss_tile_count(height, width)).x;
    const size_t lds = sizeof(float) * (2 * kLR * kLRP + 4 * kLR * kHP);
    hipStream_t st = (hipStream_t)stream;
    if (has_mask) hipLaunchKernelGGL(l1_ssim_fwd_kernel<true>, dim3((unsigned)blocks), dim3(256), lds, st, a);
    else hipLaunchKernelGGL(l1_ssim_fwd_kernel<false>, dim3((unsigned)blocks), dim3(256), lds, st, a);
    GS_LAUNCH_CHECK("l1_ssim_fwd_kernel");
    hipLaunchKernelGGL(loss_reduce_kernel, dim3(1), dim3(256), 0, st, blocks, a.partial, height, width, lambda_ssim, out3);
    GS_LAUNCH_CHECK("loss_reduce_kernel");
    return GS_OK;
}

static int loss_bwd_launch(void* stream, int height, int width, float lambda_ssim, const float* render, const float* gt,
                           const float* mask, const float* const* slots, int clamp_input, const float* workspace,
                           const float* v_total, float* v_render) {
    GS_REQUIRE(height > 2 * kHalo && width > 2 * kHalo, "image must be larger than the 11x11 window");
    GS_REQUIRE((int64_t)height * width <= kLossMaxPixels && width <= kLossMaxWidth && height <= (1 << 24),
               "image too large for the loss kernels' 32-bit byte offsets (H * W <= 2^28, W <= 2^20, H <= 2^24: row indices go through 24-bit multiplies)");
    GS_REQUIRE(render && (gt || slots) && workspace && v_total && v_render, "null pointer");
    LossArgs a;
    a.H = height; a.W = width; a.lambda_ssim = lambda_ssim; a.render = render; a.gt = gt; a.mask = mask; a.slots = slots;
    a.clamp_input = clamp_input != 0;
    a.maps = const_cast<float*>(workspace); a.partial = nullptr; a.gout = v_total; a.v_render = v_render;
    const size_t lds = sizeof(float) * (3 * kLR * kLRP);
    hipLaunchKernelGGL(l1_ssim_bwd_kernel, dim3(3 * loss_grid(loss_tile_count(height, width)).x), dim3(256), lds, (hipStream_t)stream, a);
    GS_LAUNCH_CHECK("l1_ssim_bwd_kernel");
    return GS_OK;
}

extern "C" int gs_l1_ssim_fwd(void* stream, int height, int width, float lambda_ssim, const float* render,
                              const float* gt, const float* mask, int clamp_input, float* workspace, float* out3) {
    return loss_fwd_launch(stream, height, width, lambda_ssim, render, gt, mask, nullptr, mask != nullptr, clamp_input, workspace, out3);
}

extern "C" int gs_l1_ssim_bwd(void* stream, int height, int width, float lambda_ssim, const float* render,
                              const float* gt, const float* mask, int clamp_input, const float* workspace,
                              const float* v_total, float* v_render) {
    return loss_bwd_launch(stream, height, width, lambda_ssim, render, gt, mask, nullptr, clamp_input, workspace, v_total, v_render);
}

extern "C" int gs_l1_ssim_fwd_slots(void* stream, int height, int width, float lambda_ssim, const float* render,
                                    const float* const* slots_dev, int has_mask, int clamp_input, float* workspace, float* out3) {
    GS_REQUIRE(slots_dev != nullptr, "slots_dev is required");
    return loss_fwd_launch(stream, height, width, lambda_ssim, render, nullptr, nullptr, slots_dev, has_mask != 0, clamp_input, workspace, out3);
}

extern "C" int gs_l1_ssim_bwd_slots(void* stream, int height, int width, float lambda_ssim, const float* render,
                                    const float* const* slots_dev, int clamp_input, const float* workspace,
                                    const float* v_total, float* v_render) {
    GS_REQUIRE(slots_dev != nullptr, "slots_dev is required");
    return loss_bwd_launch(stream, height, width, lambda_ssim, render, nullptr, nullptr, slots_dev, clamp_input, workspace, v_total, v_render);
}
```

### easy_gaussian_splatting_amd/rendering.py

```python
from __future__ import annotations

import ctypes as _ct
import math
import os
import threading
import time
import weakref
from typing import Dict, Optional, Tuple

import torch
from torch import Tensor

from . import _native as nat
from . import workspace as WS

_TILE = nat.GS_TILE
_BWD_CLASSES = os.environ.get("GS_BWD_CLASSES", "1") != "0"


def _ptr(t: Optional[Tensor]) -> Optional[int]:
    return None if t is None else t.data_ptr()


def _stream(device: torch.device) -> int:
# ... 91 lines not shown

ROUNDS_MIN_LISTED = 4_000_000
ROUNDS_MAX_LIVE = 0.05
ROUND_FRACTION = float(os.environ.get("GS_ROUND_FRACTION", "0.125"))
_round_bufs: Dict[tuple, dict] = {}


def rounds_mode() -> str:
    mode = os.environ.get("GS_ROUNDS", "auto")
    if mode not in ("auto", "on", "off"):
        raise ValueError(f"GS_ROUNDS must be 'auto', 'on' or 'off', got {mode!r}")
    return mode


def _round_buffers(dev: torch.device, st: int, N: int, tiles: int) -> dict:
    key = (dev.index if dev.index is not None else torch.cuda.current_device(), st)
    with _state_lock:
        b = _round_bufs.get(key)
    if b is None or b["N"] != N or b["tiles"] != tiles:
        b = {"N": N, "tiles": tiles,
             "blk": torch.zeros((nat.GS_ROUND_WORDS,), dtype=torch.int64, device=dev),
             "hist": torch.zeros((4096,), dtype=torch.int32, device=dev),
             "live": torch.zeros((tiles,), dtype=torch.uint8, device=dev),
             "state": torch.empty((tiles, 4, 64, 4), dtype=torch.float32, device=dev),
             "bbox": torch.empty((N, 4), dtype=torch.int32, device=dev),
             "tpg": torch.empty((N,), dtype=torch.int32, device=dev),
             "host": torch.zeros((nat.GS_ROUND_WORDS,), dtype=torch.int64, pin_memory=True)}
        with _state_lock:
            _round_bufs[key] = b
    return b


def _quantize_up(x: int) -> int:
    g = 1 << max(12, int(x).bit_length() - 5)
    return (int(x) + g - 1) // g * g


_INFO_RING = 8


def _pinned_info(device: torch.device) -> Tensor:
    cache = getattr(_tls, "pinned", None)
    if cache is None:
        cache = _tls.pinned = {}
    key = device.index if device.index is not None else torch.cuda.current_device()
    ring = cache.get(key)
    if ring is None:
        ring = cache[key] = [torch.empty((_INFO_RING, nat.GS_INFO_WORDS), dtype=torch.int64, pin_memory=True), 0]
    ring[1] = (ring[1] + 1) % _INFO_RING
    return ring[0][ring[1]]


class _WalkRecord:
    __slots__ = ("host", "event", "_pool")

    def __init__(self):
        pool = getattr(_tls, "walk_pool", None)
        if pool is None:
            pool = _tls.walk_pool = []
        self._pool = pool
        self.host = pool.pop() if pool else torch.zeros((4,), dtype=torch.int64, pin_memory=True)
        self.host.fill_(-1)
        self.event = None

    def __del__(self):
        try:
            self._pool.append(self.host)
        except Exception:
            pass


def _pending_checks() -> list:
    q = getattr(_tls, "pending_checks", None)
    if q is None:
        q = _tls.pending_checks = []
    return q


def flush_size_checks() -> int:
    q = _pending_checks()
    late = 0
    while q:
        late += int(q.pop(0).resolve())
    return late


class _PendingCheck:

    def __init__(self, resolve_fn):
        self._fn, self.done, self.late = resolve_fn, False, False
        self._lock = threading.Lock()

    def resolve(self) -> bool:
        with self._lock:
            if not self.done:
                self.late = bool(self._fn())
                self.done = True
                self._fn = None
                self.lease_ref = None
        return self.late


class _LazyMeta(dict):
    PENDING = object()

    class Lazy:
        __slots__ = ("fn",)

        def __init__(self, fn):
            self.fn = fn

    _lease = None

    def _isect_ids(self) -> Tensor:
        C, tiles = self["n_cameras"], self["tile_width"] * self["tile_height"]
        fid = self["flatten_ids"]
# ... 224 lines not shown
    flags = (WS.F_TRAIN if need_grad else 0) | (WS.F_TWO_LEVEL if two_level else 0) | (WS.F_ISECT_IDS if eager_ids else 0)
    cap = max(int(hint.get("cap", 0)), 2 * C * N + 4096 if not hint else 0, 4096)
    cap_tile = int(hint.get("cap_tile", 1024)) if not two_level else (1 << 30)
    coarse_cap = max(int(hint.get("entries", 0)), 2 * C * N + 1024) if two_level else 0
    coarse_list_cap = int(hint.get("longest", 0)) if two_level else 0
    cap, coarse_cap = _quantize_up(cap), (_quantize_up(coarse_cap) if two_level else 0)
    cap_units = cap_rows = 0
    if need_grad:
        cap_units = _quantize_up(max(int(hint.get("cap_units", 0)), (cap // 16 + 12 * C * tiles) if "cap_units" not in hint else 0, 256))
        cap_rows = _quantize_up(max(int(hint.get("cap_rows", 0)), cap if "cap_rows" not in hint else 0, 4096))
    walk = _WalkRecord() if need_grad else None

    lease = WS.pool.acquire(dev, st)
    lease.bind(WS.Layout(C, N, W, H, cap, coarse_cap, shift, flags, max(cap_units, 256), cap_rows), st)
    P = lease.ptr
    info_dev = lease.view(WS.INFO, nat.GS_INFO_WORDS)
    info_host = _pinned_info(dev)
    bin_bytes = lambda: int(L.gs_bins_workspace_bytes(C, N, tw, th, shift, coarse_cap) if two_level else L.gs_bin_workspace_bytes(C, N, tw, th))

    use_jac = bool(need_grad and _SH_JAC and deg >= 1)

    def project(stage: int, tag: str):
        _stage(tag, dev, lambda: nat.check(L.gs_project_fwd(
            st, C, N, K, deg, _ptr(means), _ptr(quats), _ptr(scales), _ptr(opacities), _ptr(colors), _ptr(colors_rest),
            per_cam, _ptr(viewmats), _ptr(Ks), W, H, cfg["eps2d"], cfg["near_plane"], cfg["far_plane"],
            cfg["radius_clip"], cfg["tile_culling"], stage, cfg.get("activations", 0), _ptr(radii), _ptr(means2d), _ptr(depths), _ptr(conics),
            P(WS.COLORS_POST), P(WS.REC), P(WS.BBOX), P(WS.TILES_PER_GAUSS), _ptr(rect_ref),
            P(WS.SH_JAC) if use_jac else None), "gs_project_fwd"))

    def bbox_ptr():
        return rb["bbox"].data_ptr() if rounds else P(WS.BBOX)

    def count():
        if two_level:
            nat.check(L.gs_bins_count(st, C, N, tw, th, shift, bbox_ptr(), _ptr(depths), P(WS.BIN), bin_bytes(),
                                      P(WS.COARSE_KEYS), coarse_cap, coarse_list_cap, P(WS.CUM_TILES), P(WS.ISECT_OFFSETS),
                                      P(WS.BUCKET_OFFSETS), P(WS.TILE_ORDER), P(WS.INFO), None), "gs_bins_count")
        else:
            nat.check(L.gs_bin_count(st, C, N, tw, th, bbox_ptr(), P(WS.BIN), bin_bytes(), P(WS.ISECT_OFFSETS),
                                     P(WS.BUCKET_OFFSETS), P(WS.TILE_ORDER), P(WS.INFO), None), "gs_bin_count")

    def lists_and_blend():
        if two_level:
            _stage("gs_bin_emit_sort", dev, lambda: nat.check(L.gs_bins_lists(
                st, C, N, tw, th, shift, bbox_ptr(), P(WS.BIN), bin_bytes(), P(WS.COARSE_KEYS), coarse_cap,
                P(WS.CUM_TILES), P(WS.ISECT_OFFSETS), P(WS.ISECT_IDS), P(WS.FLATTEN_IDS), P(WS.SLOTS), P(WS.INFO)), "gs_bins_lists"))
        else:
            _stage("gs_bin_emit_sort", dev, lambda: nat.check(L.gs_bin_emit_sort(
                st, C, N, tw, th, bbox_ptr(), _ptr(depths), P(WS.BIN), bin_bytes(), P(WS.ISECT_OFFSETS), cap,
                min(cap_tile, cap), P(WS.KEYS_TMP), P(WS.SLOT_GID), P(WS.CUM_TILES), P(WS.ISECT_IDS), P(WS.FLATTEN_IDS),
                P(WS.SLOTS)), "gs_bin_emit_sort"))
        if walk is not None:
            nat.check(L.gs_walk_mirror_set(walk.host.data_ptr()), "gs_walk_mirror_set")
        try:
            if ch == 3:
                _stage("gs_blend_fwd", dev, lambda: nat.check(L.gs_blend_fwd(
                    st, C, W, H, P(WS.REC), _ptr(backgrounds), P(WS.ISECT_OFFSETS), P(WS.TILE_ORDER),
                    P(WS.FLATTEN_IDS), P(WS.SLOTS), cap, _ptr(render_colors), _ptr(render_alphas), P(WS.CKPT), P(WS.QLIST), P(WS.QCNT),
                    P(WS.QMASK), P(WS.UNIT_DESC), lease.layout.cap_units, P(WS.ROW_BASE), lease.layout.cap_rows, P(WS.WALK_STATE)),
                    "gs_blend_fwd"))
            else:
                _stage("gs_blend_fwd", dev, lambda: nat.check(L.gs_blend_fwd_ch(
                    st, C, W, H, ch, P(WS.REC), _ptr(backgrounds), P(WS.ISECT_OFFSETS), P(WS.TILE_ORDER),
                    P(WS.FLATTEN_IDS), P(WS.SLOTS), cap, _ptr(render_colors), _ptr(render_alphas), P(WS.CKPT), P(WS.QLIST), P(WS.QCNT),
                    P(WS.QMASK), P(WS.UNIT_DESC), lease.layout.cap_units, P(WS.ROW_BASE), lease.layout.cap_rows, P(WS.WALK_STATE),
                    lease.ckpt_ext() if (need_grad and ch == 4) else None), "gs_blend_fwd_ch"))
        finally:
            if walk is not None:
                L.gs_walk_mirror_set(None)
                walk.event = torch.cuda.Event()
                walk.event.record(tstream)

    if dc == 3:
        project(1 if split_project else 0, "gs_project_fwd")
    else:
        project(1, "gs_project_fwd")
        if dc > 0:
            _stage("gs_rec_colors", dev, lambda: nat.check(L.gs_rec_colors(st, C, N, dc, _ptr(colors), per_cam, _ptr(radii), P(WS.REC)),
                                                           "gs_rec_colors"))
    if dmode:
        _stage("gs_rec_depth", dev, lambda: nat.check(L.gs_rec_depth(st, C, N, dc, _ptr(depths), _ptr(radii), P(WS.REC)), "gs_rec_depth"))
    sizes = {"attempt": 0, "waited": 0, "info": None}
    tstream = torch.cuda.current_stream(dev)

    def enqueue_attempt():
        nat.check(L.gs_guard_set_call(P(WS.INFO), cap, min(cap_tile, cap)), "gs_guard_set_call")
        nat.check(L.gs_info_mirror_set(info_host.data_ptr()), "gs_info_mirror_set")
        try:
            if rounds:
                if sizes["attempt"] == 0 and split_project:
                    project(2, "gs_project_fwd_color")
                nat.check(L.gs_round_split(st, N, _ptr(depths), P(WS.TILES_PER_GAUSS), ROUND_FRACTION, rb["hist"].data_ptr(), rb["blk"].data_ptr()),
                          "gs_round_split")
                ev = None
                for phase in (1, 2):
                    nat.check(L.gs_rounds_set(rb["blk"].data_ptr(), rb["live"].data_ptr(), rb["state"].data_ptr(), None, phase), "gs_rounds_set")
                    nat.check(L.gs_info_mirror_set(info_host.data_ptr()), "gs_info_mirror_set")
                    _stage("gs_round_footprints", dev, lambda: nat.check(L.gs_round_footprints(
                        st, N, tw, th, P(WS.BBOX), _ptr(depths), rb["bbox"].data_ptr(), rb["tpg"].data_ptr()), "gs_round_footprints"))
                    _stage("gs_bin_count", dev, count)
                    nat.check(L.gs_info_mirror_set(None), "gs_info_mirror_set")
                    if phase == 2:
                        ev = torch.cuda.Event()
                        ev.record(tstream)
                    lists_and_blend()
                    if phase == 1 and not deferred:
                        nat.check(L.gs_round_status(st, rb["blk"].data_ptr(), rb["host"].data_ptr()), "gs_round_status")
                        ev = torch.cuda.Event()
                        ev.record(tstream)
                        t_wait = time.perf_counter_ns()
                        ev.synchronize()
                        sizes["waited"] += time.perf_counter_ns() - t_wait
                        if int(info_host[nat.GS_INFO_FLAGS]) != 0 or int(rb["host"][nat.GS_ROUND_LIVE]) == 0:
                            break
                return ev
            _stage("gs_bin_count", dev, count)
            nat.check(L.gs_info_mirror_set(None), "gs_info_mirror_set")
            ev = torch.cuda.Event()
            ev.record(tstream)
            if sizes["attempt"] == 0 and split_project and ch == 3:
                project(2, "gs_project_fwd_color")
            lists_and_blend()
# ... 86 lines not shown
            stats["deferred_calls"] += 1
        n_isects, n_buckets, max_tile = None, n_buckets_bound, None
    else:
        pending = None
        ev, whole = ev0, False
        while not settle(ev, whole):
            ev, whole = enqueue_attempt(), True
        learn()
        n_isects, n_buckets, max_tile = (sizes["info"][w] for w in (nat.GS_INFO_ISECTS, nat.GS_INFO_BUCKETS, nat.GS_INFO_MAX_TILE))

    def isects() -> int:
        if pending is not None:
            pending.resolve()
            return state_late["n_isects"]
        return n_isects

    ref = WS.LeaseRef(lease)
    lazy = _LazyMeta.Lazy
    if lazy_ref:
        ref_lists = _ReferenceLists(rect_ref, depths, C, N, tw, th, eager_ids)
        list_entries = {"tiles_per_gauss": lazy(lambda: ref_lists.get("tiles_per_gauss")),
                        "isect_ids": lazy(lambda: ref_lists.get("isect_ids")) if eager_ids else _LazyMeta.PENDING,
                        "flatten_ids": lazy(lambda: ref_lists.get("flatten_ids")),
                        "isect_offsets": lazy(lambda: ref_lists.get("isect_offsets"))}
    elif rounds:
        one = _OneRoundLists(lease, depths, C, N, tw, th)
        list_entries = {"tiles_per_gauss": lazy(lambda: lease.view(WS.TILES_PER_GAUSS, C * N).clone().view(C, N)),
                        "isect_ids": _LazyMeta.PENDING, "flatten_ids": lazy(lambda: one.get("flatten_ids")),
                        "isect_offsets": lazy(lambda: one.get("isect_offsets"))}
    else:
        list_entries = {
            "tiles_per_gauss": lazy(lambda: (isects(), lease.view(WS.TILES_PER_GAUSS, C * N).clone().view(C, N))[1]),
            "isect_ids": lazy(lambda: lease.view(WS.ISECT_IDS, isects()).clone()) if eager_ids else _LazyMeta.PENDING,
            "flatten_ids": lazy(lambda: lease.view(WS.FLATTEN_IDS, isects()).clone()),
            "isect_offsets": lazy(lambda: (isects(), lease.view(WS.ISECT_OFFSETS, C * tiles).clone().view(C, th, tw))[1])}
    meta = _LazyMeta({
        "camera_ids": None, "gaussian_ids": None,
        "radii": radii, "means2d": means2d, "depths": depths, "conics": conics,
        "opacities": opacities[None, :].expand(C, N),
        "tile_width": tw, "tile_height": th, **list_entries,
        "width": W, "height": H, "tile_size": _TILE, "n_cameras": C,
    })
    if not lazy_ref:
        meta._lease = ref
    state = dict(C=C, N=N, K=K, deg=deg, per_cam=per_cam, ch=ch, dc=dc, dmode=dmode, sh_jac=use_jac, n_isects=n_isects, n_buckets=n_buckets, radii=radii, lease=lease,
                 lease_ref=WS.LeaseRef(lease) if need_grad else None, factorised=factorised, pending=pending, late=state_late,
                 walk=walk, hint_key=hint_key, backgrounds=backgrounds)
    if pending is not None:
        pending.lease_ref = WS.LeaseRef(lease)
    del ref
    return render_colors, render_alphas, meta, state


def _settle_walk(s: dict, cfg: dict, render_colors: Tensor, render_alphas: Tensor) -> int:
    walk, lease = s.get("walk"), s["lease"]
    if walk is None:
        return 0
    L = nat.lib()
    dev = render_colors.device
    walk.event.synchronize()
    units, storage, rows, fl = (int(v) for v in walk.host.tolist())
    if fl < 0:
        raise nat.NativeLibraryError("rasterization: the forward of this call left no walk record (was it skipped by a step guard?)")
    tries = 0
    while fl & (WS.FLAG_UNITS | WS.FLAG_ROWS):
        tries += 1
        if tries > 3:
            raise nat.NativeLibraryError(f"rasterization: the walk capacities did not settle (units {storage}, rows {rows}, flags {fl})")
        lay = lease.layout
        cu = _quantize_up(storage + (storage >> 2) + 512) if fl & WS.FLAG_UNITS else lay.cap_units
        cr = _quantize_up(rows + (rows >> 2) + 4096) if fl & WS.FLAG_ROWS else lay.cap_rows
        C, N, W, H, cap, coarse_cap, shift, flags = lay.key[:8]
        lease.grow_walk(WS.Layout(C, N, W, H, cap, coarse_cap, shift, flags, cu, cr))
        P = lease.ptr
        with _state_lock:
            stats["walk_reruns"] += 1
        with torch.cuda.device(dev):
            st = _stream(dev)
            sc, sa = torch.empty_like(render_colors), torch.empty_like(render_alphas)
            nat.check(L.gs_walk_mirror_set(walk.host.data_ptr()), "gs_walk_mirror_set")
            try:
                if s["ch"] == 3:
                    nat.check(L.gs_blend_fwd(st, C, W, H, P(WS.REC), _ptr(s["backgrounds"]), P(WS.ISECT_OFFSETS), P(WS.TILE_ORDER),
                                             P(WS.FLATTEN_IDS), P(WS.SLOTS), s["n_isects"], _ptr(sc), _ptr(sa), P(WS.CKPT), P(WS.QLIST),
                                             P(WS.QCNT), P(WS.QMASK), P(WS.UNIT_DESC), cu, P(WS.ROW_BASE), cr, P(WS.WALK_STATE)), "gs_blend_fwd")
                else:
                    nat.check(L.gs_blend_fwd_ch(st, C, W, H, s["ch"], P(WS.REC), _ptr(s["backgrounds"]), P(WS.ISECT_OFFSETS),
                                                P(WS.TILE_ORDER), P(WS.FLATTEN_IDS), P(WS.SLOTS), s["n_isects"], _ptr(sc), _ptr(sa), P(WS.CKPT),
                                                P(WS.QLIST), P(WS.QCNT), P(WS.QMASK), P(WS.UNIT_DESC), cu, P(WS.ROW_BASE), cr, P(WS.WALK_STATE),
                                                lease.ckpt_ext() if s["ch"] == 4 else None), "gs_blend_fwd_ch")
            finally:
                L.gs_walk_mirror_set(None)
            torch.cuda.current_stream(dev).synchronize()
        units, storage, rows, fl = (int(v) for v in walk.host.tolist())
    with _state_lock:
        old = _hints.get(s["hint_key"])
        if old is not None:
            old["cap_units"] = max(storage + (storage >> 2) + 512, int(old.get("cap_units", 0) * 0.995))
            old["cap_rows"] = max(rows + (rows >> 2) + 4096, int(old.get("cap_rows", 0) * 0.995))
    return rows


class _Rasterize(torch.autograd.Function):

    @staticmethod
    def forward(ctx, means, quats, scales, opacities, colors, colors_rest, viewmats, Ks, backgrounds, cfg, holder, campos=None):
        ctx.camera_grads = bool(cfg.get("camera_grads")) and ctx.needs_input_grad[6]
        need_grad = bool(cfg.get("grad_enabled", True)) and (any(ctx.needs_input_grad[:6]) or ctx.camera_grads)
        ctx.set_materialize_grads(False)
        render_colors, render_alphas, meta, state = _forward_stages(
            means, quats, scales, opacities, colors, colors_rest, viewmats, Ks, backgrounds, cfg, need_grad)
        holder.meta = meta
        if holder.debug is not None and need_grad:
            lease, tiles = state["lease"], meta["tile_width"] * meta["tile_height"]
            wstate = lease.view(WS.WALK_STATE, 8).clone()
            holder.debug.update(unit_counter=wstate[WS.WALK_UNITS:WS.WALK_UNITS + 1], walk_state=wstate,
                                qcnt=lease.view(WS.QCNT, state["C"] * tiles * 4).clone(), unit_entries=nat.GS_UNIT)
            if state["n_isects"] is not None:
                holder.debug["walked_isects"] = lease.view(WS.QMASK, max(state["n_isects"], 1))[: state["n_isects"]].count_nonzero()
        holder.lease_ref = state.pop("lease_ref")
        out_colors = render_colors
        if cfg.get("expected_depth"):
            out_colors = torch.empty_like(render_colors)
            _stage("gs_expected_depth_fwd", means.device, lambda: nat.check(nat.lib().gs_expected_depth_fwd(
                _stream(means.device), render_alphas.numel(), state["ch"], _ptr(render_colors), _ptr(render_alphas), _ptr(out_colors)),
                "gs_expected_depth_fwd"))
        holder.out_ptrs = (out_colors.data_ptr(), render_alphas.data_ptr())
        ctx.cfg, ctx.holder, ctx.state = cfg, holder, state
        ctx.split = colors_rest is not None
        if need_grad:
            extra = (colors_rest,) if ctx.split else ()
            ctx.save_for_backward(means, quats, scales, colors, viewmats, Ks, render_colors, render_alphas, opacities, *extra)
        return out_colors, render_alphas

    @staticmethod
    def backward(ctx, v_render_colors, v_render_alphas):
        L = nat.lib()
        means, quats, scales, colors, viewmats, Ks, render_colors, render_alphas, opacities = ctx.saved_tensors[:9]
        colors_rest = ctx.saved_tensors[9] if ctx.split else None
        s, cfg, holder = ctx.state, ctx.cfg, ctx.holder
        dev = means.device
        st = _stream(dev)
        C, N, K = s["C"], s["N"], s["K"]
        W, H = cfg["width"], cfg["height"]
        f32 = dict(dtype=torch.float32, device=dev)
        v_rc = torch.zeros_like(render_colors) if v_render_colors is None else v_render_colors.contiguous()
        v_ra = None if v_render_alphas is None else v_render_alphas.contiguous()
        lease, factorised = s["lease"], s["factorised"]
        if s.get("pending") is not None:
            if s["pending"].resolve():
                raise RuntimeError("rasterization(_size_check='deferred'): the forward of this call outgrew its list capacities and was "
                                   "repaired only now -- the loss and the upstream gradient of this backward were computed from unwritten "
                                   "memory.  Re-run the step (the capacities have been raised), or use the default immediate size check.")
            s["n_isects"], s["n_buckets"] = s["late"]["n_isects"], s["late"]["n_buckets"]
        P = lease.ptr
        n_rows = _settle_walk(s, cfg, render_colors, render_alphas)
        ucls = torch.empty((int(L.gs_unit_classes_ints(lease.layout.cap_units, C, W, H)),), dtype=torch.int32, device=dev) if _BWD_CLASSES else None
        ch, dc, dmode = s["ch"], s["dc"], s["dmode"]
        if cfg.get("expected_depth"):
            v_out, v_ra_in = v_rc, v_ra
            v_rc, v_ra = torch.empty_like(render_colors), torch.empty_like(render_alphas)
            _stage("gs_expected_depth_bwd", dev, lambda: nat.check(L.gs_expected_depth_bwd(
                st, render_alphas.numel(), ch, _ptr(render_colors), _ptr(render_alphas), _ptr(v_out), _ptr(v_ra_in), _ptr(v_rc), _ptr(v_ra)),
                "gs_expected_depth_bwd"))
        if ch == 3:
            _stage("gs_blend_bwd", dev, lambda: nat.check(L.gs_blend_bwd(st, C, W, H, P(WS.REC), P(WS.QLIST), P(WS.QCNT),
                                     P(WS.UNIT_DESC), lease.layout.cap_units, P(WS.CKPT), P(WS.QMASK), P(WS.ROW_BASE), P(WS.WALK_STATE),
                                     _ptr(render_colors), _ptr(render_alphas), _ptr(v_rc), _ptr(v_ra), P(WS.ROWS), _ptr(ucls)), "gs_blend_bwd"))
        else:
            _stage("gs_blend_bwd", dev, lambda: nat.check(L.gs_blend_bwd_ch(st, C, W, H, ch, P(WS.REC), P(WS.QLIST), P(WS.QCNT),
                                     P(WS.UNIT_DESC), lease.layout.cap_units, P(WS.CKPT), P(WS.QMASK), P(WS.ROW_BASE), P(WS.WALK_STATE),
                                     _ptr(render_colors), _ptr(render_alphas), _ptr(v_rc), _ptr(v_ra), P(WS.ROWS), _ptr(ucls),
                                     lease.ckpt_ext() if ch == 4 else None), "gs_blend_bwd_ch"))
        go = holder.grad_out or {}
        for k_, shp in (("means", (N, 3)), ("quats", (N, 4)), ("scales", (N, 3)), ("opacities", (N,)), ("grad_norm", (N,)), ("count", (N,))):
            if k_ in go and not (go[k_].shape == shp and go[k_].is_contiguous() and go[k_].dtype == torch.float32 and go[k_].device == dev):
                raise ValueError(f"_grad_out['{k_}'] must be a contiguous float32 tensor of shape {shp} on {dev}")
        if ("grad_norm" in go) != ("count" in go) or ("count" in go and not (factorised and C == 1)):
            raise ValueError("_grad_out['grad_norm'] / ['count'] come together, with _sh_grads='colors_pre' and a single camera")
        v_means = go["means"] if "means" in go else torch.empty((N, 3), **f32)
        v_quats = go["quats"] if "quats" in go else torch.empty((N, 4), **f32)
        v_scales = go["scales"] if "scales" in go else torch.empty((N, 3), **f32)
        v_opac = go["opacities"] if "opacities" in go else torch.empty((N,), **f32)
        v_colors = None if (factorised or dmode == "only") else torch.empty(colors.shape, **f32)
        v_pc, pc_cam = (v_colors, s["per_cam"]) if dc == 3 else (torch.empty((C, N, 3), **f32), 1)
        v_rest = torch.empty(colors_rest.shape, **f32) if (ctx.split and not factorised and dmode != "only") else None
        v_pre = row_sums = None
        if factorised:
            row_sums = torch.empty((C * N, 12), **f32)
            pay = holder.view_payload
            if pay is not None:
                if not (C == 1 and pay.dim() == 1 and pay.numel() >= 4 * N + 16 and pay.is_contiguous() and pay.dtype == torch.float32 and pay.device == dev):
                    raise ValueError(f"_view_payload must be a contiguous 1-D float32 tensor of >= 4 N + 16 elements on {dev} (single camera)")
                v_pre, rad_out, cam_out = pay[:3 * N].view(1, N, 3), pay[3 * N:4 * N], pay[4 * N:4 * N + 16]
            else:
                v_pre, rad_out, cam_out = torch.empty((C, N, 3), **f32), None, None
            _stage("gs_row_sums", dev, lambda: nat.check(L.gs_row_sums(
                st, C, N, _ptr(s["radii"]), P(WS.COLORS_POST), P(WS.TILES_PER_GAUSS), P(WS.CUM_TILES), P(WS.ROWS), P(WS.ROW_BASE), P(WS.QMASK),
                _ptr(row_sums), _ptr(v_pre), _ptr(rad_out), float(max(W, H)), _ptr(viewmats), _ptr(cam_out)), "gs_row_sums"))
            if holder.means2d_ref is not None and holder.means2d_ref() is not None:
                holder.means2d_ref().colors_pre_grad = v_pre
            if holder.on_colors_pre is not None:
                holder.on_colors_pre(v_pre)
        v_abs = torch.empty((C, N, 2), **f32)
        dbg = holder.debug
        v_m2 = v_cn = v_cp = None
        m2_out = holder.means2d_ref() if holder.means2d_ref is not None else None
        if dbg is not None or (m2_out is not None and m2_out.requires_grad):
            v_m2 = torch.empty((C, N, 2), **f32)
        if dbg is not None:
            v_cn = torch.empty((C, N, 3), **f32)
            v_cp = torch.empty((C, N, 3), **f32)
        v_viewmats = v_campos = None
        bwd_args = lambda: (st, C, N, K, s["deg"], _ptr(means), _ptr(quats), _ptr(scales), _ptr(colors),
                            _ptr(colors_rest), pc_cam, _ptr(viewmats), _ptr(Ks), W, H, cfg["eps2d"],
                            cfg["near_plane"], cfg["far_plane"], _ptr(s["radii"]),
                            P(WS.COLORS_POST), P(WS.TILES_PER_GAUSS), P(WS.CUM_TILES),
                            P(WS.ROWS), P(WS.ROW_BASE), P(WS.QMASK), _ptr(v_means), _ptr(v_quats), _ptr(v_scales), _ptr(v_opac),
                            _ptr(v_pc), _ptr(v_rest), _ptr(v_abs), _ptr(v_m2), _ptr(v_cn), _ptr(v_cp), None,
                            _ptr(opacities), cfg.get("activations", 0), P(WS.SH_JAC) if s.get("sh_jac") else None,
                            _ptr(row_sums), _ptr(go.get("grad_norm")), _ptr(go.get("count")))
        if ctx.camera_grads:
            v_m2 = torch.empty((C, N, 2), **f32) if v_m2 is None else v_m2
            v_cn = torch.empty((C, N, 3), **f32) if v_cn is None else v_cn
            v_cp = torch.empty((C, N, 3), **f32) if v_cp is None else v_cp
            partials = torch.empty((int(L.gs_cam_partials_doubles(C, N)),), dtype=torch.float64, device=dev)
# ... 220 lines not shown
```

### easy_gaussian_splatting_amd/train_graph.py

```python
from __future__ import annotations

import ctypes as ct
import math
import time
from collections import deque
from collections.abc import Mapping
from typing import Any, Dict, Optional

import torch
from torch import Tensor

from . import _native as nat
from .optim import FusedAdam
from . import rendering
from .rendering import _SH_JAC


_TILE = nat.GS_TILE
_SORT_CLASSES = (1024, 4096, 8192, 16384)


def _p(t: Optional[Tensor]):
    return None if t is None else t.data_ptr()

# ... 433 lines not shown
                self._alloc_binning()
                with torch.cuda.device(dev), self._on_stream():
                    self._count()
                info = b["info"].tolist()
                if not int(info[nat.GS_INFO_FLAGS]) & (nat.GS_FLAG_COARSE | nat.GS_FLAG_COARSE_LIST):
                    break
                self.cap_coarse = int(int(info[nat.GS_INFO_COARSE]) * self.margin) + 4096
            self.cap_coarse = int(int(info[nat.GS_INFO_COARSE]) * self.margin) + 4096
            self.cap_coarse_list = int(int(info[nat.GS_INFO_MAX_BIN]) * 1.5) + 64
            self.probed_coarse = (int(info[nat.GS_INFO_COARSE]), int(info[nat.GS_INFO_MAX_BIN]))
            n_isects, max_tile = int(info[nat.GS_INFO_ISECTS]), int(info[nat.GS_INFO_MAX_TILE])
        b["info"].zero_()
        return n_isects, max_tile

    def _enqueue_forward(self):
        L, b = nat.lib(), self.buf
        self._project()
        if not self.rounds_on:
            self._lists_and_blend("bbox")
            return
        self._ck(L.gs_round_split(self._st(), self.N, _p(b["depths"]), _p(b["tiles_per_gauss"]), self.round_fraction, _p(b["depth_hist"]),
                                   _p(b["rounds"])), "gs_round_split")
        for phase in ((4,) if self.front_only else (1, 2)):
            self._rounds_phase(phase)
            self._ck(L.gs_round_footprints(self._st(), self.N, self.tw, self.th, _p(b["bbox"]), _p(b["depths"]), _p(b["bbox_round"]),
                                            _p(b["tpg_round"])), "gs_round_footprints")
            self._lists_and_blend("bbox_round")
        self._rounds_phase(3)

    def _lists_and_blend(self, bbox: str):
        L, b = nat.lib(), self.buf
        st = self._st()
        N, W, H = self.N, self.W, self.H
        self._count(bbox)
        if self.binning == "bins":
            self._ck(L.gs_bins_lists(st, 1, N, self.tw, self.th, self.bin_shift, _p(b[bbox]), _p(b["ws"]), self.ws_bytes,
                                      _p(b["coarse_keys"]), self.cap_coarse, _p(b["cum_tiles"]), _p(b["isect_offsets"]),
                                      None, _p(b["flatten_ids"]), _p(b["slots"]), _p(b["info"])), "gs_bins_lists")
        else:
            self._ck(L.gs_bin_emit_sort(st, 1, N, self.tw, self.th, _p(b[bbox]), _p(b["depths"]), _p(b["ws"]), self.ws_bytes,
                                         _p(b["isect_offsets"]), self.cap, self.cap_tile, _p(b["keys_tmp"]), _p(b["slot_gid"]),
                                         _p(b["cum_tiles"]), None, _p(b["flatten_ids"]), _p(b["slots"])), "gs_bin_emit_sort")
        self._ck(L.gs_blend_fwd(st, 1, W, H, _p(b["rec"]), _p(b["bg"]), _p(b["isect_offsets"]),
                                 _p(b["tile_order"]), _p(b["flatten_ids"]), _p(b["slots"]), self.cap, _p(b["render_colors"]),
                                 _p(b["render_alphas"]), _p(b["ckpt"]), _p(b["qlist"]), _p(b["qcnt"]), _p(b["qmask"]),
                                 _p(b["unit_desc"]), self.cap_units, _p(b["row_base"]), self.cap_rows, _p(b["walk_state"])),
                 "gs_blend_fwd")

    def _enqueue_step(self):
        L, b, m, opt = nat.lib(), self.buf, self.model, self.opt
        st = self._st()
        N, W, H = self.N, self.W, self.H
        nat.check(L.gs_guard_set(_p(b["info"]), self.cap, self.cap_tile), "gs_guard_set")
        self._stage_no = 0
        try:
            self._enqueue_forward()
            lam = float(self.lc.lambda_ssim)
            self._ck(L.gs_l1_ssim_fwd_slots(st, H, W, lam, _p(b["render_colors"]), _p(b["img_slots"]), int(self.has_mask), 1, _p(b["loss_ws"]),
                                             _p(b["loss3"])), "gs_l1_ssim_fwd_slots")
            self._ck(L.gs_l1_ssim_bwd_slots(st, H, W, lam, _p(b["render_colors"]), _p(b["img_slots"]), 1, _p(b["loss_ws"]),
                                             _p(b["one"]), _p(b["v_render"])), "gs_l1_ssim_bwd_slots")
            if self.scale_reg and self.fuse_adam:
                self._scale_reg(None)
            self._ck(L.gs_blend_bwd(st, 1, W, H, _p(b["rec"]), _p(b["qlist"]), _p(b["qcnt"]), _p(b["unit_desc"]), self.cap_units,
                                     _p(b["ckpt"]), _p(b["qmask"]), _p(b["row_base"]), _p(b["walk_state"]),
                                     _p(b["render_colors"]), _p(b["render_alphas"]), _p(b["v_render"]), None, _p(b["rows"]), _p(b["unit_cls"])),
                      "gs_blend_bwd")
            b1, b2 = opt.defaults["betas"]
            if self.fuse_adam:
                offs = (ct.c_int64 * 6)(*opt._offs)
                args = (st, N, self.K, int(m.active_sh_degree), _p(opt.flat_param), _p(opt.exp_avg),
                        _p(opt.exp_avg_sq), offs, _p(b["viewmats"]), _p(b["Ks"]), W, H, 0.3, 0.01, 1e10,
                        _p(b["radii"]), _p(b["colors_post"]), self._tpg(), _p(b["cum_tiles"]),
                        _p(b["rows"]), _p(b["row_base"]), _p(b["qmask"]), _p(b["v_abs"]), float(b1), float(b2),
                        float(opt.defaults["eps"]), _p(b["hyper"]), _p(b["applied"]), _p(m.max_radii),
                        _p(m.grad_norm_accum), _p(m.collecting_counts), _p(b["sh_jac"]))
                if self.scale_reg:
                    self._ck(L.gs_project_bwd_adam_reg(*args, self.max_scale_ratio, self.lambda_scale), "gs_project_bwd_adam_reg")
                else:
                    self._ck(L.gs_project_bwd_adam(*args), "gs_project_bwd_adam")
            else:
                g = self.grads
                self._ck(L.gs_project_bwd(st, 1, N, self.K, int(m.active_sh_degree), _p(m.means), _p(m.quats), _p(m.log_scales),
                                          _p(m.sh_0), _p(m.sh_rest) if self.K > 1 else None, 0, _p(b["viewmats"]), _p(b["Ks"]), W, H,
                                          0.3, 0.01, 1e10, _p(b["radii"]), _p(b["colors_post"]), self._tpg(),
                                          _p(b["cum_tiles"]), _p(b["rows"]), _p(b["row_base"]), _p(b["qmask"]), _p(g["means"]), _p(g["quats"]),
                                          _p(g["log_scales"]), _p(g["logit_opacities"]), _p(g["sh_0"]), _p(g["sh_rest"]), _p(b["v_abs"]),
                                          None, None, None, None, _p(m.logit_opacities), 1, _p(b["sh_jac"]), None, None, None), "gs_project_bwd")
                if self.scale_reg:
                    self._scale_reg(g["log_scales"])
                self._ck(L.gs_update_statistics(st, N, float(max(H, W)), _p(b["radii"]), _p(b["v_abs"]), _p(m.max_radii),
                                                _p(m.grad_norm_accum), _p(m.collecting_counts)), "gs_update_statistics")
                ns = len(opt._plist)
                ends = (ct.c_int64 * ns)(*opt._ends)
                lens = (ct.c_int64 * ns)(*opt._lens)
                gptr = (ct.c_void_p * ns)(*[_p(g[grp["name"]]) for grp, _ in opt._plist])
                self._ck(L.gs_adam_step_dev(st, opt.flat_param.numel(), _p(opt.flat_param), _p(opt.exp_avg), _p(opt.exp_avg_sq), ns,
                                            ends, lens, gptr, float(b1), float(b2), float(opt.defaults["eps"]), 1.0, _p(b["hyper"]),
                                            _p(b["applied"])), "gs_adam_step_dev")
            self._ck(L.gs_step_status(st, _p(b["info"]), _p(b["applied"]), self.status.data_ptr(), _p(b["loss3"]), _p(b["loss_ring"]),
                                      self.LOSS_RING, _p(b["walk_state"])), "gs_step_status")
        except TrainStepGraph._Stop:
            pass
        finally:
            L.gs_guard_set(None, 0, 0)
            L.gs_rounds_set(None, None, None, None, 0)

    def _scale_reg(self, v_log_scales: Optional[Any], check=None):
        b, m = self.buf, self.model
        v = v_log_scales if (v_log_scales is None or isinstance(v_log_scales, int)) else v_log_scales.data_ptr()
        (check or self._ck)(nat.lib().gs_scale_reg(self._st(), self.N, _p(m.log_scales), self.max_scale_ratio, self.lambda_scale, _p(b["loss3"]),
                                        _p(b["scale_reg"]), v), "gs_scale_reg")

    def _tail(self, t: int, lrs):
        """What a step enqueues behind its graph (nothing: the single-GPU step is the graph)."""

    def _hyper(self, t: int, lrs):
        L, opt = nat.lib(), self.opt
        ns = len(opt._plist)
        b1, b2 = opt.defaults["betas"]
        nat.check(L.gs_adam_hyper(self._st(), ns, (ct.c_float * ns)(*lrs), float(b1), float(b2), int(t), _p(self.buf["hyper"])),
                  "gs_adam_hyper")

    def _capture(self, warm_up: bool = True):
        opt, m = self.opt, self.model
        names = ("max_radii", "grad_norm_accum", "collecting_counts")
        with torch.cuda.device(self.dev), self._on_stream():
            if warm_up:
                self._warm.add((self.binning, self.cap_tile))
                saved = [opt.flat_param.clone(), opt.exp_avg.clone(), opt.exp_avg_sq.clone()] + [getattr(m, n).clone() for n in names]
                self._hyper(max(opt._step, 0) + 1, [float(grp["lr"]) for grp, _ in opt._plist])
                self._enqueue_step()
                self.stream.synchronize()
                info = self.buf["info"].tolist()
                with torch.no_grad():
                    opt.flat_param.copy_(saved[0]); opt.exp_avg.copy_(saved[1]); opt.exp_avg_sq.copy_(saved[2])
                    for n, s in zip(names, saved[3:]):
                        getattr(m, n).copy_(s)
                self.buf["applied"].zero_()
                if info[nat.GS_INFO_FLAGS] != 0:
                    self.buf["info"].zero_()
                    raise RuntimeError(f"TrainStepGraph: warm-up step overflowed its own capacities {info}")
            self.graph = None
            if self.use_graph:
                g = torch.cuda.CUDAGraph()
                with torch.cuda.graph(g, stream=self.stream):
                    self._enqueue_step()
                self.graph = g
                self.stats["captures"] += 1
            if warm_up:
                self.stream.synchronize()
        self.status.zero_()
        self.confirmed_at_build = self.confirmed

    def _issue(self, entry):
        t, lrs, w2c, K, gt, mask, ready = entry[:7]
        conv = entry[7] if len(entry) > 7 else None
        after = entry[8] if len(entry) > 8 else None
# ... 122 lines not shown
                e[4] = HostFeed.to_target(src["image"], self.dev)
                e[5] = src["mask"].to(self.dev, torch.float32) if (self.has_mask and src.get("mask") is not None) else e[5]
        first = redo[0]
        self._build({"w2c": first[2], "K": first[3]}, first[4], first[5], min_cap=max(n_isects, 1), min_cap_tile=max_tile, min_walk=walk)
        for e in redo:
            self._issue(e)

    def finish(self):
        while self.pending:
            self._poll(block=True)

    LOSS_RING = 4096

    def loss_history(self, last_n: int) -> Tensor:
        applied = int(self.buf["applied"].item())
        n = max(0, min(int(last_n), applied, self.LOSS_RING))
        idx = (torch.arange(applied - n, applied, device=self.dev)) % self.LOSS_RING
        return self.buf["loss_ring"][idx]

    def report(self) -> Dict[str, Any]:
        extra = dict(scale_reg=True, max_scale_ratio=self.max_scale_ratio, lambda_scale=self.lambda_scale) if self.scale_reg else {}
        return dict(self.stats, **extra, binning=self.binning, probed_isects=self.probed[0], probed_longest_list=self.probed[1],
                    probed_coarse_entries=getattr(self, "probed_coarse", (0, 0))[0] if self.binning == "bins" else 0,
                    capacity_isects=self.cap, capacity_tile_list=self.cap_tile, capacity_work_units=self.cap_units,
                    capacity_rows=self.cap_rows, probed_work_units=self.probed_walk[0], probed_rows=self.probed_walk[1],
                    seen_work_units=self.seen_units, seen_rows=self.seen_rows, steps=self.confirmed,
                    graph=self.graph is not None, rounds=bool(self.rounds_on), round_fraction=self.round_fraction if self.rounds_on else None,
                    front_round_alone=bool(self.rounds_on and self.front_only))


class ViewParallelGraphStep(TrainStepGraph):

    def __init__(self, model, optimizer, loss_computer, data, gt_img, mask=None, vp=None, **kw):
        if vp is None or not vp.exchange or not vp.native or not vp.guard_words:
            raise ValueError("ViewParallelGraphStep needs a native ViewParallelStep(..., guard_words=True) with the exchange on")
        if not vp._raw_parameters():
            raise ValueError("ViewParallelGraphStep: the model must pass its raw parameters (fuse_activations)")
        self.vp = vp
        kw["fuse_adam"] = False
        super().__init__(model, optimizer, loss_computer, data, gt_img, mask, **kw)

    def _alloc_lists(self):
        super()._alloc_lists()
        self.buf["row_sums"] = self._take("row_sums", (self.N, 12), torch.float32)
        self.vp._records(); self.vp._bucket()

    def _enqueue_step(self):
        L, b, m, vp = nat.lib(), self.buf, self.model, self.vp
        st = self._st()
        N, W, H = self.N, self.W, self.H
        send, _ = vp._records()
        _, offs, flat = vp._bucket()
        nat.check(L.gs_guard_set(_p(b["info"]), self.cap, self.cap_tile), "gs_guard_set")
        self._stage_no = 0
        try:
            self._enqueue_forward()
            lam = float(self.lc.lambda_ssim)
            self._ck(L.gs_l1_ssim_fwd_slots(st, H, W, lam, _p(b["render_colors"]), _p(b["img_slots"]), int(self.has_mask), 1, _p(b["loss_ws"]),
                                             _p(b["loss3"])), "gs_l1_ssim_fwd_slots")
            self._ck(L.gs_l1_ssim_bwd_slots(st, H, W, lam, _p(b["render_colors"]), _p(b["img_slots"]), 1, _p(b["loss_ws"]),
                                             _p(b["one"]), _p(b["v_render"])), "gs_l1_ssim_bwd_slots")
            self._ck(L.gs_blend_bwd(st, 1, W, H, _p(b["rec"]), _p(b["qlist"]), _p(b["qcnt"]), _p(b["unit_desc"]), self.cap_units,
                                     _p(b["ckpt"]), _p(b["qmask"]), _p(b["row_base"]), _p(b["walk_state"]),
                                     _p(b["render_colors"]), _p(b["render_alphas"]), _p(b["v_render"]), None, _p(b["rows"]), _p(b["unit_cls"])), "gs_blend_bwd")
            sp = send.data_ptr()
            self._ck(L.gs_row_sums(st, 1, N, _p(b["radii"]), _p(b["colors_post"]), self._tpg(), _p(b["cum_tiles"]), _p(b["rows"]),
                                    _p(b["row_base"]), _p(b["qmask"]), _p(b["row_sums"]), sp, sp + 4 * 3 * N, float(max(H, W)), _p(b["viewmats"]),
                                    sp + 4 * 4 * N), "gs_row_sums")
            self._ck(L.gs_guard_flag_out(st, _p(b["info"]), sp + 4 * (4 * N + 16), flat.data_ptr() + 4 * vp._flag_off), "gs_guard_flag_out")
        except TrainStepGraph._Stop:
            pass
        finally:
            L.gs_guard_set(None, 0, 0)
            L.gs_rounds_set(None, None, None, None, 0)

    def _tail(self, t: int, lrs):
        import torch.distributed as dist
        L, b, m, vp, opt = nat.lib(), self.buf, self.model, self.vp, self.opt
        st = self._st()
        N, W, H, world = self.N, self.W, self.H, vp.world
        P = vp.record_len()
        send, recv = vp._records()
        _, offs, flat = vp._bucket()
        seg = lambda i, n: flat.data_ptr() + 4 * offs[i]
        w_gather = dist.all_gather_into_tensor(recv, send, group=vp.group, async_op=True)
        vp.collectives += 1
        nat.check(L.gs_guard_set(_p(b["info"]), self.cap, self.cap_tile), "gs_guard_set")
        try:
            nat.check(L.gs_project_bwd(st, 1, N, self.K, int(m.active_sh_degree), _p(m.means), _p(m.quats), _p(m.log_scales), _p(m.sh_0),
                                       _p(m.sh_rest) if self.K > 1 else None, 0, _p(b["viewmats"]), _p(b["Ks"]), W, H, 0.3, 0.01, 1e10, _p(b["radii"]),
                                       _p(b["colors_post"]), self._tpg(), _p(b["cum_tiles"]), _p(b["rows"]), _p(b["row_base"]), _p(b["qmask"]),
                                       seg(0, 3 * N), seg(2, 4 * N), seg(1, 3 * N), seg(3, N), None, None, _p(b["v_abs"]), None, None, None, None,
                                       _p(m.logit_opacities), 1, _p(b["sh_jac"]), _p(b["row_sums"]), seg(4, N), seg(5, N)), "gs_project_bwd")
            if self.scale_reg:
                self._scale_reg(seg(1, 3 * N), nat.check)
            w_sum = dist.all_reduce(flat, op=dist.ReduceOp.SUM, group=vp.group, async_op=True)
            vp.collectives += 1
            w_gather.wait()
            nat.check(L.gs_guard_merge(st, _p(b["info"]), recv.data_ptr() + 4 * (4 * N + 16), world, P), "gs_guard_merge")
            lr = dict(zip([g["name"] for g, _ in opt._plist], lrs))
            m0, v0 = opt.moments_of(m.sh_0)
            mr, vr = opt.moments_of(m.sh_rest) if self.K > 1 else (None, None)
            b1, b2 = opt.defaults["betas"]
            nat.check(L.gs_sh_adam_views(st, world, N, self.K, int(m.active_sh_degree), _p(m.means), recv.data_ptr(), P, _p(m.sh_0), _p(m0), _p(v0),
                                         _p(m.sh_rest) if self.K > 1 else None, _p(mr), _p(vr), float(lr["sh_0"]), float(lr["sh_rest"]), float(b1),
                                         float(b2), float(opt.defaults["eps"]), int(t), 1.0 / world, _p(m.max_radii)), "gs_sh_adam_views")
            w_sum.wait()
            nat.check(L.gs_guard_merge(st, _p(b["info"]), flat.data_ptr() + 4 * vp._flag_off, 1, 0), "gs_guard_merge")
            ns = len(opt._plist)
            grads = {"means": seg(0, 3 * N), "log_scales": seg(1, 3 * N), "quats": seg(2, 4 * N), "logit_opacities": seg(3, N)}
            gptr = (ct.c_void_p * ns)(*[grads.get(g["name"]) for g, _ in opt._plist])
            nat.check(L.gs_adam_step_stats(st, opt.flat_param.numel(), _p(opt.flat_param), _p(opt.exp_avg), _p(opt.exp_avg_sq), ns,
                                           (ct.c_int64 * ns)(*opt._ends), (ct.c_int64 * ns)(*opt._lens), gptr, (ct.c_float * ns)(*lrs), float(b1),
                                           float(b2), float(opt.defaults["eps"]), int(t), 1.0 / world, N, seg(4, N), seg(5, N),
                                           _p(m.grad_norm_accum), _p(m.collecting_counts)), "gs_adam_step_stats")
            nat.check(L.gs_step_applied(st, _p(b["info"]), _p(b["applied"])), "gs_step_applied")
            nat.check(L.gs_step_status(st, _p(b["info"]), _p(b["applied"]), self.status.data_ptr(), _p(b["loss3"]), _p(b["loss_ring"]),
                                       self.LOSS_RING, _p(b["walk_state"])), "gs_step_status")
        finally:
            L.gs_guard_set(None, 0, 0)
            L.gs_rounds_set(None, None, None, None, 0)

    def _poll(self, block: bool):
        super()._poll(block=True)


# ... 55 lines not shown
```

### include/gs_raster.h

```cpp
#ifndef GS_RASTER_H_
#define GS_RASTER_H_

#include <stddef.h>
#include <stdint.h>

#ifdef __cplusplus
extern "C" {
#endif

#define GS_TILE 16
#define GS_BUCKET 64
#define GS_UNIT 32
#define GS_REC_FLOATS 12
#ifndef GS_ROW_FLOATS
#define GS_ROW_FLOATS 12
#endif

#define GS_WALK_UNITS 0
#define GS_WALK_STORAGE 1
#define GS_WALK_ROWS 3
#define GS_WALK_FLAGS 4
#define GS_WALK_SKIP 5
#define GS_WALK_RANGES 32
#define GS_WALK_RANGE0 32
#define GS_WALK_WORDS (GS_WALK_RANGE0 + 32 * GS_WALK_RANGES)
#define GS_INFO_ISECTS 0
#define GS_INFO_BUCKETS 1
#define GS_INFO_MAX_TILE 2
#define GS_INFO_FLAGS 3
#define GS_INFO_COARSE 4
#define GS_INFO_MAX_BIN 5
#define GS_INFO_LIVE 6
#define GS_INFO_ONE_ROUND 7
#define GS_INFO_WORDS 8
#define GS_FLAG_ISECTS 1
#define GS_FLAG_TILE 2
#define GS_FLAG_COARSE 4
#define GS_FLAG_COARSE_LIST 8
#define GS_FLAG_UNITS 16
#define GS_FLAG_ROWS 32
#define GS_FLAG_BACK 64
#define GS_FLAG_PEER 128

#define GS_OK 0
#define GS_ERR_ARG (-1)
#define GS_ERR_HIP (-2)
#define GS_ERR_UNSUPPORTED (-3)

int gs_version(void);
const char* gs_build_flags(void);
const char* gs_last_error(void);
const char* gs_arch(void);

int gs_guard_set(const int64_t* info_dev, int64_t cap_isects, int64_t cap_tile);
int gs_guard_set_call(const int64_t* info_dev, int64_t cap_isects, int64_t cap_tile);

int gs_info_mirror_set(int64_t* info_host_mapped);
int gs_walk_mirror_set(int64_t* walk_host_mapped);

int gs_guard_flag_out(void* stream, const int64_t* info_dev, float* dst0, float* dst1);
int gs_guard_merge(void* stream, int64_t* info_dev, const float* flags, int n, int64_t stride);
int gs_step_applied(void* stream, const int64_t* info_dev, int64_t* applied_dev);

#define GS_ROUND_BASE 0
#define GS_ROUND_SPLIT 1
#define GS_ROUND_LIVE 2
#define GS_ROUND_FRONT_N 3
#define GS_ROUND_LISTED_ALL 4
#define GS_ROUND_WORDS 8
int gs_rounds_set(int64_t* rounds_dev, uint8_t* tile_live, float* tile_state, int32_t* tile_rec, int phase);
int gs_round_split(void* stream, int64_t N, const float* depths, const int32_t* tiles_per_gauss, float fraction,
                   uint32_t* hist_ws, int64_t* rounds_dev);
int gs_round_footprints(void* stream, int64_t N, int tile_w, int tile_h, const uint32_t* bbox, const float* depths,
                        uint32_t* bbox_round, int32_t* tiles_per_gauss_round);

// ... 33 lines not shown
#define GS_WS_TRAIN 1
#define GS_WS_TWO_LEVEL 2
#define GS_WS_ISECT_IDS 4
int gs_workspace_query(int C, int64_t N, int width, int height, int64_t cap_isects, int64_t coarse_cap, int64_t cap_units,
                       int64_t cap_rows, int bin_shift, int flags, int64_t* offsets, int64_t* arena_bytes);
int gs_workspace_bind(void* stream, void* fixed_base, int64_t fixed_bytes, void* list_base, int64_t list_bytes,
                      void* walk_base, int64_t walk_bytes, const int64_t* offsets, const int64_t* arena_bytes);

int gs_bin_groups(int64_t N);
size_t gs_bin_workspace_bytes(int C, int64_t N, int tile_w, int tile_h);

int gs_project_fwd(void* stream, int C, int64_t N, int K, int sh_degree, const float* means,
                   const float* quats, const float* scales, const float* opacities,
                   const float* colors_in, const float* sh_rest, int colors_per_camera,
                   const float* viewmats, const float* Ks, int width, int height, float eps2d,
                   float near_plane, float far_plane, float radius_clip, int tile_culling, int stage, int activations,
                   int32_t* radii,
                   float* means2d, float* depths, float* conics, float* colors_out, float* rec, uint32_t* bbox,
                   int32_t* tiles_per_gauss, uint32_t* rect_ref, float* sh_jac);

int gs_bin_count(void* stream, int C, int64_t N, int tile_w, int tile_h, const uint32_t* bbox,
                 void* workspace, size_t workspace_bytes, int32_t* isect_offsets,
                 int32_t* bucket_offsets, int32_t* tile_order, int64_t* info_dev, int64_t* info_host);

int gs_bin_emit_sort(void* stream, int C, int64_t N, int tile_w, int tile_h, const uint32_t* bbox,
                     const float* depths, void* workspace, size_t workspace_bytes,
                     const int32_t* isect_offsets, int64_t n_isects, int64_t max_tile_count,
                     uint64_t* keys_tmp, int32_t* slot_gid, int32_t* cum_tiles, int64_t* isect_ids,
                     int32_t* flatten_ids, int32_t* slots);

size_t gs_bins_workspace_bytes(int C, int64_t N, int tile_w, int tile_h, int bin_shift, int64_t coarse_cap);
int gs_bins_count(void* stream, int C, int64_t N, int tile_w, int tile_h, int bin_shift, const uint32_t* bbox,
                  const float* depths, void* workspace, size_t workspace_bytes, uint64_t* coarse_keys,
                  int64_t coarse_cap, int64_t coarse_list_cap, int32_t* cum_tiles, int32_t* isect_offsets,
                  int32_t* bucket_offsets, int32_t* tile_order, int64_t* info_dev, int64_t* info_host);
int gs_bins_lists(void* stream, int C, int64_t N, int tile_w, int tile_h, int bin_shift, const uint32_t* bbox,
                  void* workspace, size_t workspace_bytes, const uint64_t* coarse_keys, int64_t coarse_cap,
                  const int32_t* cum_tiles, const int32_t* isect_offsets, int64_t* isect_ids, int32_t* flatten_ids,
                  int32_t* slots, const int64_t* info_dev);

size_t gs_walk_state_ints(int64_t n_isects);
int gs_blend_fwd(void* stream, int C, int width, int height, const float* rec,
                 const float* backgrounds, const int32_t* isect_offsets, const int32_t* tile_order,
                 const int32_t* flatten_ids, const int32_t* slots, int64_t n_isects, float* render_colors,
                 float* render_alphas, float* ckpt, int32_t* qlist, int32_t* qcnt, uint8_t* qmask,
                 int32_t* unit_desc, int64_t cap_units, int32_t* row_base, int64_t cap_rows, int32_t* walk_state);

size_t gs_unit_classes_ints(int64_t cap_units, int C, int width, int height);
int gs_blend_bwd(void* stream, int C, int width, int height, const float* rec,
                 const int32_t* qlist, const int32_t* qcnt, const int32_t* unit_desc, int64_t cap_units,
                 const float* ckpt, const uint8_t* qmask, const int32_t* row_base, const int32_t* walk_state,
                 const float* render_colors, const float* render_alphas, const float* v_render_colors,
                 const float* v_render_alphas, float* rows, int32_t* unit_classes);

int gs_rec_colors(void* stream, int C, int64_t N, int channels, const float* colors, int colors_per_camera, const int32_t* radii,
                  float* rec);
int gs_blend_fwd_ch(void* stream, int C, int width, int height, int channels, const float* rec,
                    const float* backgrounds, const int32_t* isect_offsets, const int32_t* tile_order,
                    const int32_t* flatten_ids, const int32_t* slots, int64_t n_isects, float* render_colors,
                    float* render_alphas, float* ckpt, int32_t* qlist, int32_t* qcnt, uint8_t* qmask,
                    int32_t* unit_desc, int64_t cap_units, int32_t* row_base, int64_t cap_rows, int32_t* walk_state,
                    float* ckpt_ext);
int gs_blend_bwd_ch(void* stream, int C, int width, int height, int channels, const float* rec,
                    const int32_t* qlist, const int32_t* qcnt, const int32_t* unit_desc, int64_t cap_units,
                    const float* ckpt, const uint8_t* qmask, const int32_t* row_base, const int32_t* walk_state,
                    const float* render_colors, const float* render_alphas, const float* v_render_colors,
                    const float* v_render_alphas, float* rows, int32_t* unit_classes, const float* ckpt_ext);
int gs_channel_grads(void* stream, int C, int64_t N, int channels, int colors_per_camera, const int32_t* radii,
                     const int32_t* tiles_per_gauss, const int32_t* cum_tiles, const float* rows, const int32_t* row_base,
                     const uint8_t* qmask, float* v_colors);

int gs_project_bwd(void* stream, int C, int64_t N, int K, int sh_degree, const float* means,
                   const float* quats, const float* scales, const float* colors_in,
                   const float* sh_rest, int colors_per_camera, const float* viewmats,
                   const float* Ks, int width, int height, float eps2d, float near_plane, float far_plane,
                   const int32_t* radii, const float* colors_post, const int32_t* tiles_per_gauss,
                   const int32_t* cum_tiles, const float* rows, const int32_t* row_base, const uint8_t* qmask,
                   float* v_means, float* v_quats, float* v_scales, float* v_opacities,
                   float* v_colors, float* v_sh_rest, float* v_means2d_abs, float* v_means2d,
                   float* v_conics, float* v_colors_post, float* v_colors_pre,
                   const float* opacities, int activations, const float* sh_jac, const float* row_sums,
                   float* stat_grad_norm, float* stat_count);

size_t gs_cam_partials_doubles(int C, int64_t N);
int gs_project_bwd_cam(void* stream, int C, int64_t N, int K, int sh_degree, const float* means,
                       const float* quats, const float* scales, const float* colors_in,
                       const float* sh_rest, int colors_per_camera, const float* viewmats,
                       const float* Ks, int width, int height, float eps2d, float near_plane, float far_plane,
                       const int32_t* radii, const float* colors_post, const int32_t* tiles_per_gauss,
                       const int32_t* cum_tiles, const float* rows, const int32_t* row_base, const uint8_t* qmask,
                       float* v_means, float* v_quats, float* v_scales, float* v_opacities,
                       float* v_colors, float* v_sh_rest, float* v_means2d_abs, float* v_means2d,
                       float* v_conics, float* v_colors_post, float* v_colors_pre,
                       const float* opacities, int activations, const float* sh_jac, const float* row_sums,
                       float* stat_grad_norm, float* stat_count, double* cam_partials, float* v_viewmats,
                       float* v_campos);

int gs_rec_depth(void* stream, int C, int64_t N, int lane, const float* depths, const int32_t* radii, float* rec);
size_t gs_depth_partials_doubles(int C, int64_t N);
int gs_depth_grads(void* stream, int C, int64_t N, int lane, const float* means, const float* viewmats, const int32_t* radii,
                   const int32_t* tiles_per_gauss, const int32_t* cum_tiles, const float* rows, const int32_t* row_base,
                   const uint8_t* qmask, float* v_means, float* v_depths, double* cam_partials, float* v_viewmats);
int gs_expected_depth_fwd(void* stream, int64_t n_pixels, int channels, const float* acc_colors, const float* alphas,
                          float* out_colors);
int gs_expected_depth_bwd(void* stream, int64_t n_pixels, int channels, const float* acc_colors, const float* alphas,
                          const float* v_out, const float* v_alphas_in, float* v_colors, float* v_alphas);
// ... 113 lines not shown
```

Measured before the change: 742.4.

## Fold list classification, row chunk scan and unit classes into earlier kernels

Tile-list classification for sorting moves into the tilescan kernel, so class_items_kernel is skipped on the tile path. The single-block row_chunk_scan_kernel becomes a last-block-ticket step inside row_count_kernel. Backward unit classification is computed during the forward row count and handed to backward through a new thread-local class buffer, so the clear and classify launches are dropped. This cuts kernel launches and serial single-block stages, at the cost of more global atomics, a ticket protocol that depends on memory fences, and extra host-side state plumbing.

```diff
diff --git a/easy_gaussian_splatting_amd/csrc/gs_binning.hip b/easy_gaussian_splatting_amd/csrc/gs_binning.hip
--- a/easy_gaussian_splatting_amd/csrc/gs_binning.hip
+++ b/easy_gaussian_splatting_amd/csrc/gs_binning.hip
@@ -121,6 +121,19 @@
         }
         for (int g = g0 + kMax; g < g1; ++g) { const uint32_t x = col[(size_t)g * tiles]; col[(size_t)g * tiles] = run; run += x; }
         if (ch == 0) tile_cnt[i] = total;
+    }
+}
+
+constexpr int kSegLen = 8192;
+constexpr int kSegMax = 8;
+
+__device__ __forceinline__ void class_item(int i, int n, int n_lists, int32_t* __restrict__ items, int32_t* __restrict__ counts) {
+    if (n > 1024 && n <= 4096) items[atomicAdd(&counts[0], 1)] = i;
+    else if (n > 4096 && n <= kSegLen) items[n_lists + atomicAdd(&counts[1], 1)] = i;
+    else if (n > kSegLen && n <= kSegLen * kSegMax) {
+        const int ns = (n + kSegLen - 1) / kSegLen;
+        const int p = atomicAdd(&counts[2], ns);
+        for (int sg = 0; sg < ns; ++sg) items[2 * n_lists + p + sg] = i * kSegMax + sg;
     }
 }
 
@@ -144,6 +157,10 @@
             unsigned long long ex = block_excl_scan_add(v, scratch, &total);
             if (i < n_groups_total) grp_base[i] = (uint32_t)(gcarry + ex);
             gcarry += total;
+        }
+        if (sort_counts) {
+            __syncthreads();
+            for (int i = threadIdx.x; i < n_tiles_total; i += kBinThreads) class_item(i, (int)tile_cnt[i], n_tiles_total, sort_counts + 64, sort_counts);
         }
         return;
     }
@@ -366,9 +383,6 @@
 };
 __device__ __forceinline__ bool sort_off(const SortArgs& a) { return guard_tripped(a.guard) || round_idle(a.rblk, a.phase); }
 
-constexpr int kSegLen = 8192;
-constexpr int kSegMax = 8;
-
 template <bool IN_LDS>
 __global__ void tile_sort_kernel(const SortArgs a) {
     extern __shared__ __attribute__((aligned(16))) unsigned long long skeys[];
@@ -544,14 +558,7 @@
     if (guard_tripped(guard) || round_idle(rblk, phase)) return;
     const int i = blockIdx.x * blockDim.x + threadIdx.x;
     if (i >= n_lists) return;
-    const int n = offsets[i + 1] - offsets[i];
-    if (n > 1024 && n <= 4096) items[atomicAdd(&counts[0], 1)] = i;
-    else if (n > 4096 && n <= kSegLen) items[n_lists + atomicAdd(&counts[1], 1)] = i;
-    else if (n > kSegLen && n <= kSegLen * kSegMax) {
-        const int ns = (n + kSegLen - 1) / kSegLen;
-        const int p = atomicAdd(&counts[2], ns);
-        for (int sg = 0; sg < ns; ++sg) items[2 * n_lists + p + sg] = i * kSegMax + sg;
-    }
+    class_item(i, offsets[i + 1] - offsets[i], n_lists, items, counts);
 }
 
 static size_t sort_items_bytes(int64_t n_lists) {
@@ -1035,7 +1042,7 @@
 
 #define GS_SORT1K_THREADS 256
 #define GS_SORT4K_THREADS 256
-static int launch_list_sorts(hipStream_t st, SortArgs& a, unsigned grid, int64_t max_tile_count, int32_t* items_ws) {
+static int launch_list_sorts(hipStream_t st, SortArgs& a, unsigned grid, int64_t max_tile_count, int32_t* items_ws, bool items_ready) {
     int lo_excl = 0;
     int32_t* counts = items_ws;
     int32_t* items = items_ws + 64;
@@ -1047,8 +1054,10 @@
         GS_LAUNCH_CHECK("tile_radix_sort_kernel");
     }
     if (max_tile_count <= 1024) return GS_OK;
-    hipLaunchKernelGGL(class_items_kernel, dim3((grid + 255) / 256), dim3(256), 0, st, (int)grid, a.isect_offsets, items, counts, a.guard, a.rblk, a.phase);
-    GS_LAUNCH_CHECK("class_items_kernel");
+    if (!items_ready) {
+        hipLaunchKernelGGL(class_items_kernel, dim3((grid + 255) / 256), dim3(256), 0, st, (int)grid, a.isect_offsets, items, counts, a.guard, a.rblk, a.phase);
+        GS_LAUNCH_CHECK("class_items_kernel");
+    }
     {
         a.lo_excl = 1024; a.hi_incl = 4096;
         const size_t lds_k = 2 * sizeof(uint64_t) * 4096 + radix_lds * (GS_SORT4K_THREADS / 64);
@@ -1170,7 +1179,7 @@
     a.guard = current_guard().info;
     a.coarse = 0; a.seg = 0; a.merged = nullptr; a.rblk = rblk; a.phase = phase;
     static_assert(2 + kSegMax == 10, "bin_layout sizes the work lists for kSegMax == 8");
-    return launch_list_sorts(st, a, (unsigned)(C * tiles), max_tile_count, (int32_t*)(ws + L.items_off));
+    return launch_list_sorts(st, a, (unsigned)(C * tiles), max_tile_count, (int32_t*)(ws + L.items_off), true);
 }
 
 extern "C" size_t gs_bins_workspace_bytes(int C, int64_t N, int tile_w, int tile_h, int bin_shift, int64_t coarse_cap) {
@@ -1264,7 +1273,7 @@
         a.isect_ids = nullptr; a.flatten_ids = nullptr; a.slots = nullptr;
         a.guard = info_dev; a.coarse = 1; a.seg = 0; a.rblk = rblk; a.phase = phase;
         a.merged = (unsigned long long*)(ws + L.staged_off);
-        if (int rc = launch_list_sorts(st, a, (unsigned)cb, list_cap < coarse_cap ? list_cap : coarse_cap, (int32_t*)(ws + L.items_off))) return rc;
+        if (int rc = launch_list_sorts(st, a, (unsigned)cb, list_cap < coarse_cap ? list_cap : coarse_cap, (int32_t*)(ws + L.items_off), false)) return rc;
     }
     RefineArgs r;
     fill_refine_args(r, L, C, tile_w, tile_h, ws, coarse_keys, bbox, info_dev);
diff --git a/easy_gaussian_splatting_amd/csrc/gs_blend.hip b/easy_gaussian_splatting_amd/csrc/gs_blend.hip
--- a/easy_gaussian_splatting_amd/csrc/gs_blend.hip
+++ b/easy_gaussian_splatting_amd/csrc/gs_blend.hip
@@ -22,7 +22,7 @@
 constexpr int kChunk = 8;
 constexpr int kUnitLog = 128;
 constexpr int kWalkUnits = GS_WALK_UNITS, kWalkStorage = GS_WALK_STORAGE, kWalkRows = GS_WALK_ROWS,
-              kWalkFlags = GS_WALK_FLAGS, kWalkSkip = GS_WALK_SKIP;
+              kWalkFlags = GS_WALK_FLAGS, kWalkSkip = GS_WALK_SKIP, kWalkTicket = GS_WALK_TICKET, kWalkClasses = GS_WALK_CLASSES;
 constexpr int kScanThreads = 256, kScanPerThread = 32, kScanChunk = kScanThreads * kScanPerThread;
 
 struct BlendFwdArgs {
@@ -387,7 +387,12 @@
     unsigned long long* flags;
     const int64_t* guard;
     volatile int64_t* mirror;
+    const int4* unit_desc;
+    const int32_t* qcnt;
+    int4* cls;
+    int cap_units, cls_cap;
 };
+__device__ __forceinline__ void walk_unit_classes(const RowScanArgs& a, int nb);
 
 __device__ __forceinline__ int32_t row_counts32(const uint8_t* __restrict__ qmask, int64_t i0, int64_t n, uint32_t (&w)[8]) {
 #pragma unroll
@@ -411,26 +416,9 @@
     return tot;
 }
 
-__global__ __launch_bounds__(kScanThreads) void row_count_kernel(const RowScanArgs a) {
-    __shared__ int32_t scratch[20];
-    if (a.walk[kWalkSkip] != 0) return;
-    const int64_t n = slots_in_use(a.n_cap, a.guard);
-    const int64_t c0 = (int64_t)blockIdx.x * kScanChunk;
-    if (c0 > n) return;
-    uint32_t w[8];
-    const int32_t tot = row_counts32(a.qmask, c0 + (int64_t)threadIdx.x * kScanPerThread, n, w);
-    int32_t block_tot;
-    block_excl_scan_add<int32_t>(tot, scratch, &block_tot);
-    if (threadIdx.x == 0) a.walk[GS_WALK_WORDS + blockIdx.x] = block_tot;
-}
-
-__global__ __launch_bounds__(1024) void row_chunk_scan_kernel(const RowScanArgs a) {
-    __shared__ int32_t scratch[20];
-    if (a.walk[kWalkSkip] != 0) return;
-    const int64_t n = slots_in_use(a.n_cap, a.guard);
-    const int nb = (int)(n / kScanChunk) + 1;
+__device__ __forceinline__ void row_chunk_scan(const RowScanArgs& a, int nb, int32_t* scratch) {
     int32_t* part = a.walk + GS_WALK_WORDS;
-    const int per = (nb + 1023) / 1024;
+    const int per = (nb + kScanThreads - 1) / kScanThreads;
     const int j0 = (int)threadIdx.x * per, j1 = min(nb, j0 + per);
     int32_t mine = 0;
     for (int j = j0; j < j1; ++j) mine += part[j];
@@ -438,6 +426,7 @@
     int32_t run = block_excl_scan_add<int32_t>(mine, scratch, &total);
     for (int j = j0; j < j1; ++j) { const int32_t c = part[j]; part[j] = run; run += c; }
     if (threadIdx.x == 0) {
+        a.walk[kWalkTicket] = 0;
         int32_t fullest = 0;
         for (int r = 0; r < GS_WALK_RANGES; ++r) fullest = max(fullest, a.walk[GS_WALK_RANGE0 + 32 * r]);
         a.walk[kWalkStorage] = GS_WALK_RANGES * fullest;
@@ -454,6 +443,30 @@
             __threadfence_system();
         }
     }
+}
+
+__global__ __launch_bounds__(kScanThreads) void row_count_kernel(const RowScanArgs a) {
+    __shared__ int32_t scratch[20];
+    __shared__ int s_last;
+    if (a.walk[kWalkSkip] != 0) return;
+    const int64_t n = slots_in_use(a.n_cap, a.guard);
+    const int64_t c0 = (int64_t)blockIdx.x * kScanChunk;
+    if (c0 > n) return;
+    const int nb = (int)(n / kScanChunk) + 1;
+    uint32_t w[8];
+    const int32_t tot = row_counts32(a.qmask, c0 + (int64_t)threadIdx.x * kScanPerThread, n, w);
+    int32_t block_tot;
+    block_excl_scan_add<int32_t>(tot, scratch, &block_tot);
+    if (threadIdx.x == 0) {
+        a.walk[GS_WALK_WORDS + blockIdx.x] = block_tot;
+        __threadfence();
+        s_last = atomicAdd(a.walk + kWalkTicket, 1) == nb - 1 ? 1 : 0;
+    }
+    if (a.cls != nullptr) walk_unit_classes(a, nb);
+    __syncthreads();
+    if (s_last == 0) return;
+    __threadfence();
+    row_chunk_scan(a, nb, scratch);
 }
 
 __global__ __launch_bounds__(kScanThreads) void row_base_kernel(const RowScanArgs a) {
@@ -729,6 +742,47 @@
     }
 }
 
+__device__ __forceinline__ int walk_unit_class(const RowScanArgs& a, int u, int n_units, int4& ud) {
+    if (u >= n_units) return 0;
+    ud = a.unit_desc[u];
+    const int n_in = min(kUnit, a.qcnt[ud.x] - ud.y * kUnit);
+    ud.w = u;
+    return min(max((n_in + kPipeLanes - 1) / kPipeLanes, 1), 4);
+}
+__device__ __forceinline__ void walk_unit_classes(const RowScanArgs& a, int nb) {
+    __shared__ int s_cnt[kScanThreads / 64][4], s_base[kScanThreads / 64][4];
+    const int n_units = min(a.walk[kWalkUnits], a.cap_units);
+    const int wave = threadIdx.x >> 6, lane = threadIdx.x & 63;
+    const int first = (int)blockIdx.x * kScanThreads, stride = nb * kScanThreads;
+    int4 ud = make_int4(0, 0, 0, 0);
+    int n1 = 0, n2 = 0, n3 = 0, n4 = 0;
+    for (int u0 = first; u0 < n_units; u0 += stride) {
+        const int c = walk_unit_class(a, u0 + (int)threadIdx.x, n_units, ud);
+        n1 += (int)__popcll(__ballot(c == 1)); n2 += (int)__popcll(__ballot(c == 2));
+        n3 += (int)__popcll(__ballot(c == 3)); n4 += (int)__popcll(__ballot(c == 4));
+    }
+    if (lane < 4) s_cnt[wave][lane] = lane == 0 ? n1 : (lane == 1 ? n2 : (lane == 2 ? n3 : n4));
+    __syncthreads();
+    if (threadIdx.x < 4) {
+        int tot = 0;
+        for (int w = 0; w < kScanThreads / 64; ++w) { s_base[w][threadIdx.x] = tot; tot += s_cnt[w][threadIdx.x]; }
+        const int base = tot ? atomicAdd(a.walk + kWalkClasses + 1 + threadIdx.x, tot) : 0;
+        for (int w = 0; w < kScanThreads / 64; ++w) s_base[w][threadIdx.x] += base;
+    }
+    __syncthreads();
+    int b1 = s_base[wave][0], b2 = s_base[wave][1], b3 = s_base[wave][2], b4 = s_base[wave][3];
+    for (int u0 = first; u0 < n_units; u0 += stride) {
+        const int c = walk_unit_class(a, u0 + (int)threadIdx.x, n_units, ud);
+        const unsigned long long m1 = __ballot(c == 1), m2 = __ballot(c == 2), m3 = __ballot(c == 3), m4 = __ballot(c == 4);
+        if (c) {
+            const unsigned long long mine = c == 1 ? m1 : (c == 2 ? m2 : (c == 3 ? m3 : m4));
+            const int i = (c == 1 ? b1 : (c == 2 ? b2 : (c == 3 ? b3 : b4))) + (int)__popcll(mine & ((1ull << lane) - 1ull));
+            if (i < (c == 4 ? a.cap_units : a.cls_cap)) a.cls[(c == 4 ? 0 : a.cap_units + (3 - c) * a.cls_cap) + i] = ud;
+        }
+        b1 += (int)__popcll(m1); b2 += (int)__popcll(m2); b3 += (int)__popcll(m3); b4 += (int)__popcll(m4);
+    }
+}
+
 template <int NC>
 __device__ __forceinline__ void blend_bwd_body(const BlendBwdArgs& a, const float* __restrict__ ckpt_ext) {
     __shared__ float4 sd0_all[kBwdWaves][kUnitsPerWave][64];
@@ -801,6 +855,12 @@
 extern "C" size_t gs_walk_state_ints(int64_t n_isects) {
     if (n_isects < 0) return 0;
     return (size_t)GS_WALK_WORDS + (size_t)(n_isects / kScanChunk + 1);
+}
+
+static int64_t cls_region(int C, int width, int height) {
+    const int64_t tiles = (int64_t)((width + GS_TILE - 1) / GS_TILE) * ((height + GS_TILE - 1) / GS_TILE);
+    const int64_t per_block = kBwdWaves * kUnitsPerWave;
+    return (4 * (int64_t)C * tiles + per_block - 1) / per_block * per_block;
 }
 
 template <int NC>
@@ -840,6 +900,8 @@
     GS_REQUIRE(phase == 0 || !train || R.tile_rec, "depth rounds, training mode: gs_rounds_set needs tile_rec");
     GS_REQUIRE(NC == 3 || phase == 0, "depth rounds render 3 channels only (tile_state holds T, r, g, b): clear gs_rounds_set");
     GS_REQUIRE(NC != 4 || !train || ckpt_ext, "channels = 4, training mode: ckpt_ext (cap_units * 64 floats) is required");
+    const WalkClasses wc = train ? current_walk_classes() : WalkClasses{nullptr, 0};
+    GS_REQUIRE(wc.buf == nullptr || wc.cap_units == cap_units, "gs_walk_classes_set: the class buffer was announced for another cap_units");
     a.rblk = R.blk; a.live = R.live; a.tstate = R.state; a.trec = reinterpret_cast<int4*>(R.tile_rec);
     GS_IF_CHECK(a.chk = g_bwd_check;)
     const unsigned n_tiles = (unsigned)(C * a.tiles);
@@ -861,9 +923,13 @@
         RowScanArgs s;
         s.qmask = qmask; s.row_base = row_base; s.walk = walk_state; s.n_cap = n_isects; s.cap_rows = cap_rows;
         s.flags = a.flags; s.guard = a.guard; s.mirror = current_walk_mirror();
+        s.unit_desc = a.unit_desc; s.qcnt = qcnt; s.cls = nullptr; s.cap_units = (int)cap_units; s.cls_cap = 0;
+        if (wc.buf) {
+            s.cls = reinterpret_cast<int4*>(wc.buf + kClsHdrInts);
+            s.cls_cap = (int)cls_region(C, width, height);
+        }
         const unsigned chunks = (unsigned)(n_isects / kScanChunk + 1);
         hipLaunchKernelGGL(row_count_kernel, dim3(chunks), dim3(kScanThreads), 0, st, s);
-        hipLaunchKernelGGL(row_chunk_scan_kernel, dim3(1), dim3(1024), 0, st, s);
         hipLaunchKernelGGL(row_base_kernel, dim3(chunks), dim3(kScanThreads), 0, st, s);
         GS_LAUNCH_CHECK("row_base_kernel");
     } else {
@@ -903,12 +969,6 @@
         default: return GS_FWD_CH(4);
     }
 #undef GS_FWD_CH
-}
-
-static int64_t cls_region(int C, int width, int height) {
-    const int64_t tiles = (int64_t)((width + GS_TILE - 1) / GS_TILE) * ((height + GS_TILE - 1) / GS_TILE);
-    const int64_t per_block = kBwdWaves * kUnitsPerWave;
-    return (4 * (int64_t)C * tiles + per_block - 1) / per_block * per_block;
 }
 
 extern "C" size_t gs_unit_classes_ints(int64_t cap_units, int C, int width, int height) {
@@ -946,11 +1006,16 @@
         GS_REQUIRE(((uintptr_t)unit_classes & 15) == 0, "unit_classes must be 16-byte aligned");
         a.cls_hdr = unit_classes; a.cls_desc = reinterpret_cast<const int4*>(unit_classes + kClsHdrInts);
         a.cls_cap = (int)cls_region(C, width, height);
-        hipLaunchKernelGGL(unit_classes_clear_kernel, dim3(1), dim3(64), 0, (hipStream_t)stream, unit_classes);
-        hipLaunchKernelGGL(unit_classes_kernel, dim3((unsigned)((cap_units + kClsThreads - 1) / kClsThreads)), dim3(kClsThreads), 0, (hipStream_t)stream,
-                           walk_state, a.unit_desc, qcnt, (int)cap_units, a.cls_cap, unit_classes, reinterpret_cast<int4*>(unit_classes + kClsHdrInts),
-                           a.guard);
-        GS_LAUNCH_CHECK("unit_classes_kernel");
+        const WalkClasses wc = current_walk_classes();
+        if (wc.buf == unit_classes && wc.cap_units == cap_units) {
+            a.cls_hdr = walk_state + kWalkClasses;
+        } else {
+            hipLaunchKernelGGL(unit_classes_clear_kernel, dim3(1), dim3(64), 0, (hipStream_t)stream, unit_classes);
+            hipLaunchKernelGGL(unit_classes_kernel, dim3((unsigned)((cap_units + kClsThreads - 1) / kClsThreads)), dim3(kClsThreads), 0, (hipStream_t)stream,
+                               walk_state, a.unit_desc, qcnt, (int)cap_units, a.cls_cap, unit_classes, reinterpret_cast<int4*>(unit_classes + kClsHdrInts),
+                               a.guard);
+            GS_LAUNCH_CHECK("unit_classes_kernel");
+        }
         grid += 3u * (unsigned)(a.cls_cap / (kUnitsPerWave * kBwdWaves));
     }
     if constexpr (NC == 3) hipLaunchKernelGGL(blend_bwd_kernel, dim3(grid), dim3(kBwdWaves * 64), 0, (hipStream_t)stream, a);
diff --git a/easy_gaussian_splatting_amd/csrc/gs_capi.hip b/easy_gaussian_splatting_amd/csrc/gs_capi.hip
--- a/easy_gaussian_splatting_amd/csrc/gs_capi.hip
+++ b/easy_gaussian_splatting_amd/csrc/gs_capi.hip
@@ -16,6 +16,8 @@
 int64_t* current_info_mirror() { return g_info_mirror; }
 static thread_local int64_t* g_walk_mirror = nullptr;
 int64_t* current_walk_mirror() { return g_walk_mirror; }
+static thread_local WalkClasses g_walk_classes = {nullptr, 0};
+WalkClasses current_walk_classes() { return g_walk_classes; }
 static thread_local Rounds g_rounds = {nullptr, nullptr, nullptr, nullptr, 0};
 Rounds current_rounds() { return g_rounds; }
 }
@@ -44,6 +46,16 @@
 
 extern "C" int gs_walk_mirror_set(int64_t* walk_host_mapped) {
     gs::g_walk_mirror = walk_host_mapped;
+    return GS_OK;
+}
+
+extern "C" int gs_walk_classes_set(int32_t* unit_classes, int64_t cap_units) {
+    if (unit_classes != nullptr && (cap_units <= 0 || cap_units >= (1ll << 26) || (((uintptr_t)unit_classes) & 15) != 0)) {
+        gs::set_error("invalid argument: unit_classes 16-byte aligned, 0 < cap_units < 2^26");
+        return GS_ERR_ARG;
+    }
+    gs::g_walk_classes.buf = unit_classes;
+    gs::g_walk_classes.cap_units = unit_classes ? cap_units : 0;
     return GS_OK;
 }
 
diff --git a/easy_gaussian_splatting_amd/csrc/gs_common.h b/easy_gaussian_splatting_amd/csrc/gs_common.h
--- a/easy_gaussian_splatting_amd/csrc/gs_common.h
+++ b/easy_gaussian_splatting_amd/csrc/gs_common.h
@@ -68,6 +68,11 @@
 Guard current_guard();
 int64_t* current_info_mirror();
 int64_t* current_walk_mirror();
+struct WalkClasses {
+    int32_t* buf;
+    int64_t cap_units;
+};
+WalkClasses current_walk_classes();
 __device__ __forceinline__ bool guard_tripped(const int64_t* info) { return info != nullptr && info[3] != 0; }
 
 struct Rounds {
diff --git a/easy_gaussian_splatting_amd/csrc/gs_loss.hip b/easy_gaussian_splatting_amd/csrc/gs_loss.hip
--- a/easy_gaussian_splatting_amd/csrc/gs_loss.hip
+++ b/easy_gaussian_splatting_amd/csrc/gs_loss.hip
@@ -1,3 +1,6 @@
+#include <mutex>
+#include <unordered_map>
+
 #include "gs_loss_tile.h"
 
 namespace gs {
@@ -14,7 +17,12 @@
     float* partial;
     const float* gout;
     float* v_render;
+    float* out3;
+    int ticket;
 };
+
+constexpr int kLossTickets = 1024;
+__device__ unsigned g_loss_tickets[kLossTickets];
 
 __device__ __forceinline__ void st_off(float* base, unsigned byte_off, float v) {
     *reinterpret_cast<float*>(reinterpret_cast<char*>(base) + byte_off) = v;
@@ -32,6 +40,40 @@
     const int ty = t / ntx;
     x0 = (t - ty * ntx) * kLT; y0 = ty * kLT;
     return true;
+}
+
+__device__ __forceinline__ void loss_reduce(int nblocks, const float* partial, int H, int W, float lambda_ssim, float* out) {
+    __shared__ double red[2][4];
+    double s0 = 0.0, s1 = 0.0;
+    for (int i = threadIdx.x; i < nblocks; i += 256) { s0 += partial[2 * i]; s1 += partial[2 * i + 1]; }
+#pragma unroll
+    for (int d = 32; d > 0; d >>= 1) { s0 += __shfl_xor(s0, d, 64); s1 += __shfl_xor(s1, d, 64); }
+    if (lane_id() == 0) { red[0][threadIdx.x >> 6] = s0; red[1][threadIdx.x >> 6] = s1; }
+    __syncthreads();
+    if (threadIdx.x == 0) {
+        const double l1 = (red[0][0] + red[0][1] + red[0][2] + red[0][3]) / ((double)H * W * 3.0);
+        const double cnt = (double)(H - 2 * kHalo) * (double)(W - 2 * kHalo) * 3.0;
+        const double ssim = (red[1][0] + red[1][1] + red[1][2] + red[1][3]) / cnt;
+        out[0] = (float)l1; out[1] = (float)(1.0 - ssim);
+        out[2] = (float)((1.0 - lambda_ssim) * l1 + lambda_ssim * (1.0 - ssim));
+    }
+}
+__global__ __launch_bounds__(256) void loss_reduce_kernel(int nblocks, const float* partial, int H, int W, float lambda_ssim, float* out) {
+    loss_reduce(nblocks, partial, H, W, lambda_ssim, out);
+}
+
+__device__ __forceinline__ void loss_ticket_reduce(const LossArgs& a) {
+    __shared__ int s_last;
+    if (a.ticket < 0) return;
+    if (threadIdx.x == 0) {
+        __threadfence();
+        s_last = atomicAdd(&g_loss_tickets[a.ticket], 1u) == gridDim.x - 1u ? 1 : 0;
+    }
+    __syncthreads();
+    if (s_last == 0) return;
+    __threadfence();
+    if (threadIdx.x == 0) g_loss_tickets[a.ticket] = 0u;
+    loss_reduce((int)gridDim.x, a.partial, a.H, a.W, a.lambda_ssim, a.out3);
 }
 
 template <bool MASK>
@@ -45,6 +87,7 @@
     int x0, y0;
     if (!loss_tile(a, x0, y0)) {
         if (threadIdx.x == 0) { a.partial[2 * blockIdx.x] = 0.f; a.partial[2 * blockIdx.x + 1] = 0.f; }
+        loss_ticket_reduce(a);
         return;
     }
     const int tid = threadIdx.x;
@@ -165,24 +208,7 @@
         a.partial[2 * blockIdx.x] = red[0][0] + red[0][1] + red[0][2] + red[0][3];
         a.partial[2 * blockIdx.x + 1] = red[1][0] + red[1][1] + red[1][2] + red[1][3];
     }
-}
-
-__global__ __launch_bounds__(256) void loss_reduce_kernel(int nblocks, const float* __restrict__ partial, int H, int W,
-                                                          float lambda_ssim, float* __restrict__ out) {
-    __shared__ double red[2][4];
-    double s0 = 0.0, s1 = 0.0;
-    for (int i = threadIdx.x; i < nblocks; i += 256) { s0 += partial[2 * i]; s1 += partial[2 * i + 1]; }
-#pragma unroll
-    for (int d = 32; d > 0; d >>= 1) { s0 += __shfl_xor(s0, d, 64); s1 += __shfl_xor(s1, d, 64); }
-    if (lane_id() == 0) { red[0][threadIdx.x >> 6] = s0; red[1][threadIdx.x >> 6] = s1; }
-    __syncthreads();
-    if (threadIdx.x == 0) {
-        const double l1 = (red[0][0] + red[0][1] + red[0][2] + red[0][3]) / ((double)H * W * 3.0);
-        const double cnt = (double)(H - 2 * kHalo) * (double)(W - 2 * kHalo) * 3.0;
-        const double ssim = (red[1][0] + red[1][1] + red[1][2] + red[1][3]) / cnt;
-        out[0] = (float)l1; out[1] = (float)(1.0 - ssim);
-        out[2] = (float)((1.0 - lambda_ssim) * l1 + lambda_ssim * (1.0 - ssim));
-    }
+    loss_ticket_reduce(a);
 }
 
 __global__ __launch_bounds__(256) void l1_ssim_bwd_kernel(const LossArgs a) {
@@ -337,6 +363,18 @@
     return 9 * (size_t)height * width + 2 * (nb + 8);
 }
 
+static int loss_ticket_slot(const void* workspace) {
+    static std::mutex mu;
+    static std::unordered_map<const void*, int> slots;
+    std::lock_guard<std::mutex> lock(mu);
+    const auto it = slots.find(workspace);
+    if (it != slots.end()) return it->second;
+    if ((int)slots.size() >= kLossTickets) return -1;
+    const int slot = (int)slots.size();
+    slots.emplace(workspace, slot);
+    return slot;
+}
+
 static int loss_fwd_launch(void* stream, int height, int width, float lambda_ssim, const float* render, const float* gt,
                            const float* mask, const float* const* slots, bool has_mask, int clamp_input, float* workspace, float* out3) {
     GS_REQUIRE(height > 2 * kHalo && width > 2 * kHalo, "image must be larger than the 11x11 window");
@@ -347,14 +385,17 @@
     a.H = height; a.W = width; a.lambda_ssim = lambda_ssim; a.render = render; a.gt = gt; a.mask = mask; a.slots = slots;
     a.clamp_input = clamp_input != 0;
     a.maps = workspace; a.partial = workspace + 9 * (size_t)height * width; a.gout = nullptr; a.v_render = nullptr;
+    a.out3 = out3; a.ticket = loss_ticket_slot(workspace);
     const int blocks = (int)loss_grid(loss_tile_count(height, width)).x;
     const size_t lds = sizeof(float) * (2 * kLR * kLRP + 4 * kLR * kHP);
     hipStream_t st = (hipStream_t)stream;
     if (has_mask) hipLaunchKernelGGL(l1_ssim_fwd_kernel<true>, dim3((unsigned)blocks), dim3(256), lds, st, a);
     else hipLaunchKernelGGL(l1_ssim_fwd_kernel<false>, dim3((unsigned)blocks), dim3(256), lds, st, a);
     GS_LAUNCH_CHECK("l1_ssim_fwd_kernel");
-    hipLaunchKernelGGL(loss_reduce_kernel, dim3(1), dim3(256), 0, st, blocks, a.partial, height, width, lambda_ssim, out3);
-    GS_LAUNCH_CHECK("loss_reduce_kernel");
+    if (a.ticket < 0) {
+        hipLaunchKernelGGL(loss_reduce_kernel, dim3(1), dim3(256), 0, st, blocks, a.partial, height, width, lambda_ssim, out3);
+        GS_LAUNCH_CHECK("loss_reduce_kernel");
+    }
     return GS_OK;
 }
 
@@ -369,6 +410,7 @@
     a.H = height; a.W = width; a.lambda_ssim = lambda_ssim; a.render = render; a.gt = gt; a.mask = mask; a.slots = slots;
     a.clamp_input = clamp_input != 0;
     a.maps = const_cast<float*>(workspace); a.partial = nullptr; a.gout = v_total; a.v_render = v_render;
+    a.out3 = nullptr; a.ticket = -1;
     const size_t lds = sizeof(float) * (3 * kLR * kLRP);
     hipLaunchKernelGGL(l1_ssim_bwd_kernel, dim3(3 * loss_grid(loss_tile_count(height, width)).x), dim3(256), lds, (hipStream_t)stream, a);
     GS_LAUNCH_CHECK("l1_ssim_bwd_kernel");
diff --git a/easy_gaussian_splatting_amd/rendering.py b/easy_gaussian_splatting_amd/rendering.py
--- a/easy_gaussian_splatting_amd/rendering.py
+++ b/easy_gaussian_splatting_amd/rendering.py
@@ -167,7 +167,7 @@
 
 
 class _WalkRecord:
-    __slots__ = ("host", "event", "_pool")
+    __slots__ = ("host", "event", "ucls", "_pool")
 
     def __init__(self):
         pool = getattr(_tls, "walk_pool", None)
@@ -177,6 +177,7 @@
         self.host = pool.pop() if pool else torch.zeros((4,), dtype=torch.int64, pin_memory=True)
         self.host.fill_(-1)
         self.event = None
+        self.ucls = None
 
     def __del__(self):
         try:
@@ -507,6 +508,7 @@
                 P(WS.SLOTS)), "gs_bin_emit_sort"))
         if walk is not None:
             nat.check(L.gs_walk_mirror_set(walk.host.data_ptr()), "gs_walk_mirror_set")
+            _announce_classes(walk, lease.layout.cap_units, C, W, H, dev)
         try:
             if ch == 3:
                 _stage("gs_blend_fwd", dev, lambda: nat.check(L.gs_blend_fwd(
@@ -523,6 +525,7 @@
         finally:
             if walk is not None:
                 L.gs_walk_mirror_set(None)
+                L.gs_walk_classes_set(None, 0)
                 walk.event = torch.cuda.Event()
                 walk.event.record(tstream)
 
@@ -715,6 +718,14 @@
     return render_colors, render_alphas, meta, state
 
 
+def _announce_classes(walk: "_WalkRecord", cap_units: int, C: int, W: int, H: int, dev) -> None:
+    if not _BWD_CLASSES:
+        return
+    L = nat.lib()
+    walk.ucls = torch.empty((int(L.gs_unit_classes_ints(cap_units, C, W, H)),), dtype=torch.int32, device=dev)
+    nat.check(L.gs_walk_classes_set(walk.ucls.data_ptr(), cap_units), "gs_walk_classes_set")
+
+
 def _settle_walk(s: dict, cfg: dict, render_colors: Tensor, render_alphas: Tensor) -> int:
     walk, lease = s.get("walk"), s["lease"]
     if walk is None:
@@ -742,6 +753,7 @@
             st = _stream(dev)
             sc, sa = torch.empty_like(render_colors), torch.empty_like(render_alphas)
             nat.check(L.gs_walk_mirror_set(walk.host.data_ptr()), "gs_walk_mirror_set")
+            _announce_classes(walk, cu, C, W, H, dev)
             try:
                 if s["ch"] == 3:
                     nat.check(L.gs_blend_fwd(st, C, W, H, P(WS.REC), _ptr(s["backgrounds"]), P(WS.ISECT_OFFSETS), P(WS.TILE_ORDER),
@@ -754,6 +766,7 @@
                                                 lease.ckpt_ext() if s["ch"] == 4 else None), "gs_blend_fwd_ch")
             finally:
                 L.gs_walk_mirror_set(None)
+                L.gs_walk_classes_set(None, 0)
             torch.cuda.current_stream(dev).synchronize()
         units, storage, rows, fl = (int(v) for v in walk.host.tolist())
     with _state_lock:
@@ -818,7 +831,10 @@
             s["n_isects"], s["n_buckets"] = s["late"]["n_isects"], s["late"]["n_buckets"]
         P = lease.ptr
         n_rows = _settle_walk(s, cfg, render_colors, render_alphas)
-        ucls = torch.empty((int(L.gs_unit_classes_ints(lease.layout.cap_units, C, W, H)),), dtype=torch.int32, device=dev) if _BWD_CLASSES else None
+        walk = s.get("walk")
+        ucls = walk.ucls if walk is not None else None
+        if ucls is not None:
+            nat.check(L.gs_walk_classes_set(ucls.data_ptr(), lease.layout.cap_units), "gs_walk_classes_set")
         ch, dc, dmode = s["ch"], s["dc"], s["dmode"]
         if cfg.get("expected_depth"):
             v_out, v_ra_in = v_rc, v_ra
@@ -826,15 +842,18 @@
             _stage("gs_expected_depth_bwd", dev, lambda: nat.check(L.gs_expected_depth_bwd(
                 st, render_alphas.numel(), ch, _ptr(render_colors), _ptr(render_alphas), _ptr(v_out), _ptr(v_ra_in), _ptr(v_rc), _ptr(v_ra)),
                 "gs_expected_depth_bwd"))
-        if ch == 3:
-            _stage("gs_blend_bwd", dev, lambda: nat.check(L.gs_blend_bwd(st, C, W, H, P(WS.REC), P(WS.QLIST), P(WS.QCNT),
-                                     P(WS.UNIT_DESC), lease.layout.cap_units, P(WS.CKPT), P(WS.QMASK), P(WS.ROW_BASE), P(WS.WALK_STATE),
-                                     _ptr(render_colors), _ptr(render_alphas), _ptr(v_rc), _ptr(v_ra), P(WS.ROWS), _ptr(ucls)), "gs_blend_bwd"))
-        else:
-            _stage("gs_blend_bwd", dev, lambda: nat.check(L.gs_blend_bwd_ch(st, C, W, H, ch, P(WS.REC), P(WS.QLIST), P(WS.QCNT),
-                                     P(WS.UNIT_DESC), lease.layout.cap_units, P(WS.CKPT), P(WS.QMASK), P(WS.ROW_BASE), P(WS.WALK_STATE),
-                                     _ptr(render_colors), _ptr(render_alphas), _ptr(v_rc), _ptr(v_ra), P(WS.ROWS), _ptr(ucls),
-                                     lease.ckpt_ext() if ch == 4 else None), "gs_blend_bwd_ch"))
+        try:
+            if ch == 3:
+                _stage("gs_blend_bwd", dev, lambda: nat.check(L.gs_blend_bwd(st, C, W, H, P(WS.REC), P(WS.QLIST), P(WS.QCNT),
+                                         P(WS.UNIT_DESC), lease.layout.cap_units, P(WS.CKPT), P(WS.QMASK), P(WS.ROW_BASE), P(WS.WALK_STATE),
+                                         _ptr(render_colors), _ptr(render_alphas), _ptr(v_rc), _ptr(v_ra), P(WS.ROWS), _ptr(ucls)), "gs_blend_bwd"))
+            else:
+                _stage("gs_blend_bwd", dev, lambda: nat.check(L.gs_blend_bwd_ch(st, C, W, H, ch, P(WS.REC), P(WS.QLIST), P(WS.QCNT),
+                                         P(WS.UNIT_DESC), lease.layout.cap_units, P(WS.CKPT), P(WS.QMASK), P(WS.ROW_BASE), P(WS.WALK_STATE),
+                                         _ptr(render_colors), _ptr(render_alphas), _ptr(v_rc), _ptr(v_ra), P(WS.ROWS), _ptr(ucls),
+                                         lease.ckpt_ext() if ch == 4 else None), "gs_blend_bwd_ch"))
+        finally:
+            L.gs_walk_classes_set(None, 0)
         go = holder.grad_out or {}
         for k_, shp in (("means", (N, 3)), ("quats", (N, 4)), ("scales", (N, 3)), ("opacities", (N,)), ("grad_norm", (N,)), ("count", (N,))):
             if k_ in go and not (go[k_].shape == shp and go[k_].is_contiguous() and go[k_].dtype == torch.float32 and go[k_].device == dev):
diff --git a/easy_gaussian_splatting_amd/train_graph.py b/easy_gaussian_splatting_amd/train_graph.py
--- a/easy_gaussian_splatting_amd/train_graph.py
+++ b/easy_gaussian_splatting_amd/train_graph.py
@@ -509,6 +509,7 @@
         st = self._st()
         N, W, H = self.N, self.W, self.H
         nat.check(L.gs_guard_set(_p(b["info"]), self.cap, self.cap_tile), "gs_guard_set")
+        nat.check(L.gs_walk_classes_set(_p(b["unit_cls"]), self.cap_units), "gs_walk_classes_set")
         self._stage_no = 0
         try:
             self._enqueue_forward()
@@ -561,6 +562,7 @@
             pass
         finally:
             L.gs_guard_set(None, 0, 0)
+            L.gs_walk_classes_set(None, 0)
             L.gs_rounds_set(None, None, None, None, 0)
 
     def _scale_reg(self, v_log_scales: Optional[Any], check=None):
@@ -789,6 +791,7 @@
         send, _ = vp._records()
         _, offs, flat = vp._bucket()
         nat.check(L.gs_guard_set(_p(b["info"]), self.cap, self.cap_tile), "gs_guard_set")
+        nat.check(L.gs_walk_classes_set(_p(b["unit_cls"]), self.cap_units), "gs_walk_classes_set")
         self._stage_no = 0
         try:
             self._enqueue_forward()
@@ -809,6 +812,7 @@
             pass
         finally:
             L.gs_guard_set(None, 0, 0)
+            L.gs_walk_classes_set(None, 0)
             L.gs_rounds_set(None, None, None, None, 0)
 
     def _tail(self, t: int, lrs):
diff --git a/include/gs_raster.h b/include/gs_raster.h
--- a/include/gs_raster.h
+++ b/include/gs_raster.h
@@ -21,6 +21,8 @@
 #define GS_WALK_ROWS 3
 #define GS_WALK_FLAGS 4
 #define GS_WALK_SKIP 5
+#define GS_WALK_TICKET 6
+#define GS_WALK_CLASSES 8
 #define GS_WALK_RANGES 32
 #define GS_WALK_RANGE0 32
 #define GS_WALK_WORDS (GS_WALK_RANGE0 + 32 * GS_WALK_RANGES)
@@ -160,6 +162,7 @@
                  const float* ckpt, const uint8_t* qmask, const int32_t* row_base, const int32_t* walk_state,
                  const float* render_colors, const float* render_alphas, const float* v_render_colors,
                  const float* v_render_alphas, float* rows, int32_t* unit_classes);
+int gs_walk_classes_set(int32_t* unit_classes, int64_t cap_units);
 
 int gs_rec_colors(void* stream, int C, int64_t N, int channels, const float* colors, int colors_per_camera, const int32_t* radii,
                   float* rec);
```

After: 708.8. 4.5% lower.
